# StanfordASL/pmpc

Hardware: AMD Instinct MI355X
Metric: SCP iterations/sec (M particles x N horizon) (higher is better)
Workload: dtype f64; 1 GPU; quadrotor x12 u4 M=4096 N=50 Nc=1 box-u, full SCP iteration (on-device linearise + c_lqp_solve-equivalent + residual), BASELINE config D; timed window = SCP iterations 6..2477 from the cold start X_prev = x0, U_prev = U_ref (the active-set round count falls as the SCP loop converges, so the rate depends on the window); particles_per_gpu=4096, parallelism=particle-shard x1, scp_loop=library (pmpc_scp_loop_device), ipm_warm_start=True

## Files before the change

include/pmpc_abi.h:

```cpp
#ifndef PMPC_ABI_H
#define PMPC_ABI_H

#include <stddef.h>

#ifdef __cplusplus
extern "C" {
#endif


void c_lqp_solve(double *X_out, double *U_out, size_t xdim, size_t udim, size_t N, size_t M, long long Nc,
                 double *x0, double *f, double *fx, double *fu, double *X_prev, double *U_prev, double *Q,
                 double *R, double *X_ref, double *U_ref, double *lx, double *ux, double *lu, double *uu,
                 double reg_x, double reg_u, double *slew_reg, double *slew_reg0, double *slew_um1,
                 long long verbose);

void c_lcone_solve(double *X_out, double *U_out, size_t xdim, size_t udim, size_t N, size_t M, long long Nc,
                   double *x0, double *f, double *fx, double *fu, double *X_prev, double *U_prev, double *Q,
                   double *R, double *X_ref, double *U_ref, double *lx, double *ux, double *lu, double *uu,
                   double reg_x, double reg_u, double *slew_reg, double *slew_reg0, double *slew_um1,
                   long long verbose, double smooth_alpha, char *solver);

void pmpc_lqp_solve_host(double *X_out, double *U_out, size_t xdim, size_t udim, size_t N, size_t M, long long Nc,
                         double *x0, double *f, double *fx, double *fu, double *X_prev, double *U_prev, double *Q,
                         double *R, double *X_ref, double *U_ref, double *lx, double *ux, double *lu, double *uu,
// ... 24 lines not shown
#define PMPC_CONE_OBJECTIVE 1024u
#define PMPC_F32_MATRICES 512u

typedef struct pmpc_problem {
  size_t xdim, udim, N, M;
  long long Nc;
  unsigned flags;
  double reg_x, reg_u;
  const double *x0, *f, *fx, *fu, *X_prev, *U_prev, *Q, *R, *X_ref, *U_ref;
  const double *lx, *ux, *lu, *uu;
  const double *slew_reg, *slew_reg0, *slew_um1;
  double *X_out, *U_out;
  const double *weights;
  double barrier_mu;
  size_t soc_q;
  const double *soc_W, *soc_w0, *soc_v;
  double soc_v0;
  const double *soc_u_interior;
  size_t cone_count;
  const int *cone_sizes;
  const double *cone_A, *cone_c;
  int cone_per_stage;
  long long cone_k;
  int smooth_cstr;
  double smooth_beta;
} pmpc_problem;

typedef struct pmpc_info {
  int status;
  int ipm_iters;
  int structured_solves;
  int fast_path;
  double mu;
  double slack_res;
  double max_violation;
  int outer_solves;
  int active_set_rounds;
} pmpc_info;

typedef struct pmpc_ctx pmpc_ctx;

int pmpc_create(pmpc_ctx **ctx, int device);
void pmpc_destroy(pmpc_ctx *ctx);
int pmpc_set_option(pmpc_ctx *ctx, const char *key, double value);
int pmpc_get_option(pmpc_ctx *ctx, const char *key, double *value);
void *pmpc_stream(pmpc_ctx *ctx);
void pmpc_sync(pmpc_ctx *ctx);

int pmpc_lqp_solve_device(pmpc_ctx *ctx, const pmpc_problem *prob, pmpc_info *info, int verbose);

int pmpc_lcone_solve_device(pmpc_ctx *ctx, const pmpc_problem *prob, double smooth_alpha, pmpc_info *info, int verbose);

int pmpc_lsoc_solve_device(pmpc_ctx *ctx, const pmpc_problem *prob, pmpc_info *info, int verbose);

int pmpc_particle_costs_device(pmpc_ctx *ctx, const pmpc_problem *prob, const double *X, const double *U, double *J_out);

int pmpc_comm_unique_id(void *unique_id_128);
int pmpc_comm_init(pmpc_ctx *ctx, int rank, int world, const void *unique_id_128);
int pmpc_comm_init_mock(pmpc_ctx *ctx, int rank, int world, int group);
int pmpc_comm_rank(pmpc_ctx *ctx);
int pmpc_comm_world(pmpc_ctx *ctx);

int pmpc_linearize_device(pmpc_ctx *ctx, int model, size_t N, size_t M, const double *x0, const double *X_prev,
                          const double *U_prev, const double *params, double *f, double *fx, double *fu);

int pmpc_linearize_device_f32(pmpc_ctx *ctx, int model, size_t N, size_t M, const double *x0, const double *X_prev,
                              const double *U_prev, const double *params, double *f, float *fx, float *fu);

int pmpc_rollout_device(pmpc_ctx *ctx, int model, size_t N, size_t M, const double *x0, const double *U, const double *params, double *X);

int pmpc_shift_plan_device(pmpc_ctx *ctx, int model, size_t N, size_t M, size_t s, const double *X, const double *U,
                           const double *params, const double *U_tail, double *X_new, double *U_new, double *um1_new);

int pmpc_linearize_compact_device(pmpc_ctx *ctx, int model, size_t N, size_t M, const double *x0, const double *X_prev,
                                  const double *U_prev, const double *params, double *f, double *jc);
int pmpc_expand_jac_device(pmpc_ctx *ctx, int model, size_t N, size_t M, const double *jc, double *fx, double *fu, int orient);
long long pmpc_jac_compact_doubles(int model, size_t N, size_t M);
int pmpc_jac_live_mask(int model, unsigned char *fx_mask, unsigned char *fu_mask);

int pmpc_as_sweep_variant(int sweep, int xdim, int udim, int M, int Nc, unsigned flags, const int *knobs, int *out);

int pmpc_as_sweep_launches(int sweep, unsigned long long *out, int n, int reset);
void pmpc_as_sweep_knobs(int *out);

int pmpc_scp_residual_device(pmpc_ctx *ctx, size_t xdim, size_t udim, size_t N, size_t M, const double *X, const double *X_prev,
                             const double *U, const double *U_prev, double *out);

int pmpc_scp_loop_device(pmpc_ctx *ctx, int model, const double *params, const pmpc_problem *p, double *f2, double *fx2, double *fu2,
                         int steps, int first_cold, double *res, pmpc_info *infos, int *last_in_out);

int pmpc_ref_shift_device(pmpc_ctx *ctx, size_t dim, size_t rows, const double *A, const double *c, const double *ref, double *out);
long long pmpc_ref_shift_bad_pivots(pmpc_ctx *ctx, int reset);

typedef struct pmpc_scp_cost {
  int kind;
  int K, pos_dim;
  int pos_idx[3];
  int per_stage;
  const double *centres, *sigma, *w;
} pmpc_scp_cost;
size_t pmpc_abi_scp_cost_size(void);

int pmpc_obstacle_cost_grad_device(pmpc_ctx *ctx, const pmpc_scp_cost *cost, size_t xdim, size_t N, size_t M, const double *X_prev,
                                   double *cx);
int pmpc_obstacle_ref_shift_device(pmpc_ctx *ctx, const pmpc_scp_cost *cost, size_t xdim, size_t N, size_t M, const double *X_prev,
                                   const double *Q, const double *X_ref, double *out);

int pmpc_scp_loop_device_cost(pmpc_ctx *ctx, int model, const double *params, const pmpc_problem *p, double *f2, double *fx2,
                              double *fu2, int steps, int first_cold, double *res, pmpc_info *infos, int *last_in_out,
                              const pmpc_scp_cost *cost);

typedef struct pmpc_scp_cstr {
  int kind;
  int K, pos_dim;
  int pos_idx[3];
  long long centre_stride_particle, centre_stride_stage;
  const double *centres, *radius;
} pmpc_scp_cstr;
size_t pmpc_abi_scp_cstr_size(void);

int pmpc_keepout_augment_device(pmpc_ctx *ctx, const pmpc_scp_cstr *cstr, size_t xdim, size_t udim, size_t N, size_t M,
                                const double *X_prev, const double *f, const double *fx, const double *fu, const double *X_ref,
                                double *f_aug, double *fx_aug, double *fu_aug, double *X_prev_aug, double *X_ref_aug, double *xu_aug);

void pmpc_profile_enable(pmpc_ctx *ctx, int level);
void pmpc_profile_read(pmpc_ctx *ctx, double *ms4, long long *n4);
void pmpc_profile_read_partial(pmpc_ctx *ctx, double *ms, long long *n);
void pmpc_profile_read_all(pmpc_ctx *ctx, double *ms, long long *launches, int count);

void pmpc_restart_stats(pmpc_ctx *ctx, unsigned long long *out4, int reset);

const char *pmpc_version(void);
void pmpc_abi_struct_sizes(size_t *problem, size_t *info);

#ifdef __cplusplus
}
#endif
#endif
```

pmpc_amd/_lib.py:

```python
from __future__ import annotations

import ctypes
import os
from pathlib import Path

import numpy as np

_HERE = Path(__file__).resolve().parent
LIB_PATH = Path(os.environ["PMPC_HIP_LIB"]) if os.environ.get("PMPC_HIP_LIB") else _HERE / "libpmpc_hip.so"
_lib = None

c_dp = ctypes.POINTER(ctypes.c_double)

HAS_XBOUNDS, HAS_UBOUNDS, HAS_SLEW, HAS_SLEW0, FORCE_GENERIC, SYMMETRIC_COST, COLD_START, STATIC_CONS_BOUNDS, PREV_IS_LAST_SOLUTION, F32_MATRICES, CONE_OBJECTIVE = 1, 2, 4, 8, 16, 32, 64, 128, 256, 512, 1024

ABI_SYMBOLS = [
    "c_lqp_solve", "c_lcone_solve", "pmpc_lqp_solve_host", "pmpc_lcone_solve_host", "pmpc_create", "pmpc_destroy", "pmpc_stream", "pmpc_sync", "pmpc_lqp_solve_device",
    "pmpc_comm_unique_id", "pmpc_comm_init", "pmpc_comm_rank", "pmpc_comm_world", "pmpc_linearize_device",
    "pmpc_profile_enable", "pmpc_profile_read", "pmpc_version", "pmpc_lcone_solve_device", "pmpc_particle_costs_device", "pmpc_lsoc_solve_device", "pmpc_comm_init_mock",
    "pmpc_scp_residual_device", "pmpc_profile_read_partial", "pmpc_profile_read_all", "pmpc_scp_loop_device", "pmpc_linearize_device_f32",
    "pmpc_set_option", "pmpc_get_option", "pmpc_abi_struct_sizes", "pmpc_lcone_solve_host_ex", "pmpc_restart_stats",
    "pmpc_linearize_compact_device", "pmpc_expand_jac_device", "pmpc_jac_compact_doubles", "pmpc_jac_live_mask",
    "pmpc_as_sweep_variant", "pmpc_as_sweep_launches", "pmpc_as_sweep_knobs",
    "pmpc_ref_shift_device", "pmpc_ref_shift_bad_pivots", "pmpc_obstacle_cost_grad_device", "pmpc_obstacle_ref_shift_device",
    "pmpc_scp_loop_device_cost", "pmpc_abi_scp_cost_size",
    "pmpc_rollout_device", "pmpc_shift_plan_device",
    "pmpc_keepout_augment_device", "pmpc_abi_scp_cstr_size",
]


class PmpcProblem(ctypes.Structure):
    _fields_ = (
        [(k, ctypes.c_size_t) for k in ("xdim", "udim", "N", "M")]
        + [("Nc", ctypes.c_longlong), ("flags", ctypes.c_uint), ("reg_x", ctypes.c_double), ("reg_u", ctypes.c_double)]
        + [(k, ctypes.c_void_p) for k in ("x0", "f", "fx", "fu", "X_prev", "U_prev", "Q", "R", "X_ref", "U_ref",
                                          "lx", "ux", "lu", "uu", "slew_reg", "slew_reg0", "slew_um1", "X_out", "U_out", "weights")]
        + [("barrier_mu", ctypes.c_double), ("soc_q", ctypes.c_size_t), ("soc_W", ctypes.c_void_p), ("soc_w0", ctypes.c_void_p),
           ("soc_v", ctypes.c_void_p), ("soc_v0", ctypes.c_double), ("soc_u_interior", ctypes.c_void_p),
           ("cone_count", ctypes.c_size_t), ("cone_sizes", ctypes.POINTER(ctypes.c_int)), ("cone_A", ctypes.c_void_p), ("cone_c", ctypes.c_void_p),
           ("cone_per_stage", ctypes.c_int), ("cone_k", ctypes.c_longlong), ("smooth_cstr", ctypes.c_int), ("smooth_beta", ctypes.c_double)]
    )


class PmpcInfo(ctypes.Structure):
    _fields_ = [("status", ctypes.c_int), ("ipm_iters", ctypes.c_int), ("structured_solves", ctypes.c_int),
                ("fast_path", ctypes.c_int), ("mu", ctypes.c_double), ("slack_res", ctypes.c_double),
                ("max_violation", ctypes.c_double), ("outer_solves", ctypes.c_int), ("active_set_rounds", ctypes.c_int)]


class PmpcScpCost(ctypes.Structure):
    _fields_ = [("kind", ctypes.c_int), ("K", ctypes.c_int), ("pos_dim", ctypes.c_int), ("pos_idx", ctypes.c_int * 3), ("per_stage", ctypes.c_int),
                ("centres", ctypes.c_void_p), ("sigma", ctypes.c_void_p), ("w", ctypes.c_void_p)]


class PmpcScpCstr(ctypes.Structure):
    _fields_ = [("kind", ctypes.c_int), ("K", ctypes.c_int), ("pos_dim", ctypes.c_int), ("pos_idx", ctypes.c_int * 3),
                ("centre_stride_particle", ctypes.c_longlong), ("centre_stride_stage", ctypes.c_longlong),
                ("centres", ctypes.c_void_p), ("radius", ctypes.c_void_p)]


def load():
    global _lib
    if _lib is not None:
        return _lib
    if not LIB_PATH.exists():
        raise ImportError(
            f"{LIB_PATH} is missing: build the HIP extension first (python -c 'import __graft_entry__ as g; g.build()' "
            "or make -C pmpc_amd/csrc). pmpc_amd has no CPU fallback.")
    lib = ctypes.CDLL(str(LIB_PATH), mode=ctypes.RTLD_GLOBAL)
    sz, ll, dbl, vp = ctypes.c_size_t, ctypes.c_longlong, ctypes.c_double, ctypes.c_void_p
    common = [c_dp, c_dp, sz, sz, sz, sz, ll] + [c_dp] * 14 + [dbl, dbl] + [c_dp] * 3 + [ll]
    lib.c_lqp_solve.argtypes = common
    lib.c_lqp_solve.restype = None
    lib.c_lcone_solve.argtypes = common + [dbl, ctypes.c_char_p]
    lib.c_lcone_solve.restype = None
    lib.pmpc_lqp_solve_host.argtypes = common + [ctypes.c_uint]
    lib.pmpc_lqp_solve_host.restype = None
    lib.pmpc_lcone_solve_host.argtypes = common + [dbl, ctypes.c_uint, ll]
    lib.pmpc_lcone_solve_host.restype = None
    lib.pmpc_lcone_solve_host_ex.argtypes = common + [dbl, ctypes.c_uint, ll, ctypes.c_int, dbl]
    lib.pmpc_lcone_solve_host_ex.restype = None
    lib.pmpc_create.argtypes = [ctypes.POINTER(vp), ctypes.c_int]
    lib.pmpc_create.restype = ctypes.c_int
    lib.pmpc_destroy.argtypes = [vp]
    lib.pmpc_destroy.restype = None
    lib.pmpc_set_option.argtypes = [vp, ctypes.c_char_p, ctypes.c_double]
    lib.pmpc_set_option.restype = ctypes.c_int
    lib.pmpc_get_option.argtypes = [vp, ctypes.c_char_p, c_dp]
    lib.pmpc_get_option.restype = ctypes.c_int
    lib.pmpc_stream.argtypes = [vp]
    lib.pmpc_stream.restype = vp
    lib.pmpc_sync.argtypes = [vp]
    lib.pmpc_sync.restype = None
    lib.pmpc_lqp_solve_device.argtypes = [vp, ctypes.POINTER(PmpcProblem), ctypes.POINTER(PmpcInfo), ctypes.c_int]
    lib.pmpc_lqp_solve_device.restype = ctypes.c_int
    lib.pmpc_lcone_solve_device.argtypes = [vp, ctypes.POINTER(PmpcProblem), dbl, ctypes.POINTER(PmpcInfo), ctypes.c_int]
    lib.pmpc_lcone_solve_device.restype = ctypes.c_int
    lib.pmpc_lsoc_solve_device.argtypes = [vp, ctypes.POINTER(PmpcProblem), ctypes.POINTER(PmpcInfo), ctypes.c_int]
    lib.pmpc_lsoc_solve_device.restype = ctypes.c_int
    lib.pmpc_particle_costs_device.argtypes = [vp, ctypes.POINTER(PmpcProblem), vp, vp, vp]
    lib.pmpc_particle_costs_device.restype = ctypes.c_int
    lib.pmpc_comm_unique_id.argtypes = [vp]
    lib.pmpc_comm_unique_id.restype = ctypes.c_int
    lib.pmpc_comm_init.argtypes = [vp, ctypes.c_int, ctypes.c_int, vp]
    lib.pmpc_comm_init.restype = ctypes.c_int
    lib.pmpc_comm_init_mock.argtypes = [vp, ctypes.c_int, ctypes.c_int, ctypes.c_int]
    lib.pmpc_comm_init_mock.restype = ctypes.c_int
    lib.pmpc_comm_rank.argtypes = [vp]
    lib.pmpc_comm_rank.restype = ctypes.c_int
    lib.pmpc_comm_world.argtypes = [vp]
    lib.pmpc_comm_world.restype = ctypes.c_int
    lib.pmpc_linearize_device.argtypes = [vp, ctypes.c_int, sz, sz] + [vp] * 7
    lib.pmpc_linearize_device.restype = ctypes.c_int
    lib.pmpc_linearize_device_f32.argtypes = [vp, ctypes.c_int, sz, sz] + [vp] * 7
    lib.pmpc_linearize_device_f32.restype = ctypes.c_int
    if hasattr(lib, "pmpc_jac_live_mask"):
        lib.pmpc_linearize_compact_device.argtypes = [vp, ctypes.c_int, sz, sz] + [vp] * 6
        lib.pmpc_linearize_compact_device.restype = ctypes.c_int
        lib.pmpc_expand_jac_device.argtypes = [vp, ctypes.c_int, sz, sz, vp, vp, vp, ctypes.c_int]
        lib.pmpc_expand_jac_device.restype = ctypes.c_int
        lib.pmpc_jac_compact_doubles.argtypes = [ctypes.c_int, sz, sz]
        lib.pmpc_jac_compact_doubles.restype = ctypes.c_longlong
        lib.pmpc_jac_live_mask.argtypes = [ctypes.c_int, vp, vp]
        lib.pmpc_jac_live_mask.restype = ctypes.c_int
    if hasattr(lib, "pmpc_as_sweep_variant"):
        lib.pmpc_as_sweep_variant.argtypes = [ctypes.c_int] * 5 + [ctypes.c_uint, ctypes.POINTER(ctypes.c_int), ctypes.POINTER(ctypes.c_int)]
        lib.pmpc_as_sweep_variant.restype = ctypes.c_int
    if hasattr(lib, "pmpc_as_sweep_launches"):
        lib.pmpc_as_sweep_launches.argtypes = [ctypes.c_int, ctypes.POINTER(ctypes.c_ulonglong), ctypes.c_int, ctypes.c_int]
        lib.pmpc_as_sweep_launches.restype = ctypes.c_int
        lib.pmpc_as_sweep_knobs.argtypes = [ctypes.POINTER(ctypes.c_int)]
        lib.pmpc_as_sweep_knobs.restype = None
    lib.pmpc_scp_residual_device.argtypes = [vp, sz, sz, sz, sz] + [vp] * 5
    lib.pmpc_scp_residual_device.restype = ctypes.c_int
    lib.pmpc_profile_enable.argtypes = [vp, ctypes.c_int]
    lib.pmpc_profile_enable.restype = None
    lib.pmpc_profile_read.argtypes = [vp, c_dp, ctypes.POINTER(ctypes.c_longlong)]
    lib.pmpc_profile_read.restype = None
    lib.pmpc_profile_read_partial.argtypes = [vp, ctypes.POINTER(ctypes.c_double), ctypes.POINTER(ctypes.c_longlong)]
    lib.pmpc_profile_read_partial.restype = None
    lib.pmpc_restart_stats.argtypes = [vp, ctypes.POINTER(ctypes.c_ulonglong), ctypes.c_int]
    lib.pmpc_restart_stats.restype = None
    lib.pmpc_profile_read_all.argtypes = [vp, c_dp, ctypes.POINTER(ctypes.c_longlong), ctypes.c_int]
    lib.pmpc_profile_read_all.restype = None
    lib.pmpc_scp_loop_device.argtypes = [vp, ctypes.c_int, vp, ctypes.POINTER(PmpcProblem), vp, vp, vp, ctypes.c_int, ctypes.c_int, vp,
                                         ctypes.POINTER(PmpcInfo), ctypes.POINTER(ctypes.c_int)]
    lib.pmpc_scp_loop_device.restype = ctypes.c_int
    if hasattr(lib, "pmpc_scp_loop_device_cost"):
        lib.pmpc_ref_shift_device.argtypes = [vp, sz, sz, vp, vp, vp, vp]
        lib.pmpc_ref_shift_device.restype = ctypes.c_int
        lib.pmpc_ref_shift_bad_pivots.argtypes = [vp, ctypes.c_int]
        lib.pmpc_ref_shift_bad_pivots.restype = ctypes.c_longlong
        lib.pmpc_obstacle_cost_grad_device.argtypes = [vp, ctypes.POINTER(PmpcScpCost), sz, sz, sz, vp, vp]
        lib.pmpc_obstacle_cost_grad_device.restype = ctypes.c_int
        lib.pmpc_obstacle_ref_shift_device.argtypes = [vp, ctypes.POINTER(PmpcScpCost), sz, sz, sz, vp, vp, vp, vp]
        lib.pmpc_obstacle_ref_shift_device.restype = ctypes.c_int
        lib.pmpc_scp_loop_device_cost.argtypes = lib.pmpc_scp_loop_device.argtypes + [ctypes.POINTER(PmpcScpCost)]
        lib.pmpc_scp_loop_device_cost.restype = ctypes.c_int
        lib.pmpc_abi_scp_cost_size.argtypes = []
        lib.pmpc_abi_scp_cost_size.restype = sz
        if lib.pmpc_abi_scp_cost_size() != ctypes.sizeof(PmpcScpCost):
            raise ImportError(f"{LIB_PATH} and pmpc_amd/_lib.py disagree on pmpc_scp_cost: library {lib.pmpc_abi_scp_cost_size()} bytes, "
                              f"binding {ctypes.sizeof(PmpcScpCost)}: rebuild the library")
    if hasattr(lib, "pmpc_shift_plan_device"):
        lib.pmpc_rollout_device.argtypes = [vp, ctypes.c_int, sz, sz, vp, vp, vp, vp]
        lib.pmpc_rollout_device.restype = ctypes.c_int
        lib.pmpc_shift_plan_device.argtypes = [vp, ctypes.c_int, sz, sz, sz] + [vp] * 7
        lib.pmpc_shift_plan_device.restype = ctypes.c_int
    if hasattr(lib, "pmpc_keepout_augment_device"):
        lib.pmpc_keepout_augment_device.argtypes = [vp, ctypes.POINTER(PmpcScpCstr), sz, sz, sz, sz] + [vp] * 11
        lib.pmpc_keepout_augment_device.restype = ctypes.c_int
        lib.pmpc_abi_scp_cstr_size.argtypes = []
        lib.pmpc_abi_scp_cstr_size.restype = sz
        if lib.pmpc_abi_scp_cstr_size() != ctypes.sizeof(PmpcScpCstr):
            raise ImportError(f"{LIB_PATH} and pmpc_amd/_lib.py disagree on pmpc_scp_cstr: library {lib.pmpc_abi_scp_cstr_size()} bytes, "
                              f"binding {ctypes.sizeof(PmpcScpCstr)}: rebuild the library")
    lib.pmpc_version.argtypes = []
    lib.pmpc_version.restype = ctypes.c_char_p
    if not hasattr(lib, "pmpc_abi_struct_sizes"):
        raise ImportError(f"{LIB_PATH} predates this binding (no pmpc_abi_struct_sizes): rebuild it (make -C pmpc_amd/csrc)")
    lib.pmpc_abi_struct_sizes.argtypes = [ctypes.POINTER(sz), ctypes.POINTER(sz)]
    lib.pmpc_abi_struct_sizes.restype = None
    sp, si = sz(0), sz(0)
    lib.pmpc_abi_struct_sizes(ctypes.byref(sp), ctypes.byref(si))
    if (sp.value, si.value) != (ctypes.sizeof(PmpcProblem), ctypes.sizeof(PmpcInfo)):
        raise ImportError(f"{LIB_PATH} ({lib.pmpc_version().decode()}) and pmpc_amd/_lib.py disagree on the ABI structs: library "
                          f"{sp.value}/{si.value} bytes, binding {ctypes.sizeof(PmpcProblem)}/{ctypes.sizeof(PmpcInfo)}: rebuild the library")
    _lib = lib
    return lib


def jac_live_mask(model: int, x: int, u: int):
    lib = load()
    mx, mu = np.zeros(x * x, dtype=np.uint8), np.zeros(x * u, dtype=np.uint8)
    got = lib.pmpc_jac_live_mask(int(model), mx.ctypes.data, mu.ctypes.data)
    if got < 0:
        raise ValueError(f"model {model} is not a built-in model")
    if got != 100 * x + u:
        raise ValueError(f"model {model}: compact records are for dims {got // 100} x {got % 100}, not {x} x {u}")
    return mx.reshape(x, x).T.astype(bool), mu.reshape(u, x).T.astype(bool)


AS_SWEEP_FLAGS = ("defect", "as_settled_in", "mat32", "cone_H", "xb_D", "as_uraw", "as_T")


def as_sweep_variant(sweep: str, x: int, u: int, M: int, Nc: int, flags: int, knobs=None):
    lib = load()
    out = (ctypes.c_int * 8)()
    kn = (ctypes.c_int * 3)(*knobs) if knobs is not None else None
    got = lib.pmpc_as_sweep_variant({"bwd": 0, "fwd": 1}[sweep], x, u, M, Nc, flags, kn, out)
    if got < 0:
        raise ValueError(f"({x}, {u}) is not a compiled pair of the active-set sweeps")
    return tuple(out[:5]), bool(got), tuple(bool(v) for v in out[5:8])


def as_sweep_code(sweep: str, variant) -> int:
    a, b, c, d, e = (int(v) for v in variant)
    if sweep == "bwd":
        return a + 3 * (b + 2 * (c + 2 * (d + 3 * e)))
    return a + 2 * b + 4 * c + 8 * d + 16 * e


def as_sweep_launches(sweep: str, reset: bool = False):
    lib = load()
    sw = {"bwd": 0, "fwd": 1}[sweep]
    n = lib.pmpc_as_sweep_launches(sw, None, 0, 0)
    out = (ctypes.c_ulonglong * n)()
    lib.pmpc_as_sweep_launches(sw, out, n, int(reset))
    return [int(v) for v in out]


def as_sweep_knobs():
    out = (ctypes.c_int * 3)()
    load().pmpc_as_sweep_knobs(out)
    return tuple(out)


def dptr(a: np.ndarray):
    assert a.dtype == np.float64 and a.flags["C_CONTIGUOUS"]
    return a.ctypes.data_as(c_dp)
```

pmpc_amd/csrc/as_ctl_dev.h:

```cpp
#pragma once
#include "pmpc_dev.h"

namespace {

__device__ inline void as_ctl_block(AsCtl *ctl, const int *cnt_part, int M, const int *fail, int reduce, int decide, int last_of_batch,
                                                 AsCtl *mirror, unsigned long long *mirror_seq, unsigned long long seq, double *tail, const double *viol,
                                                 const int *open_part = nullptr) {
  __shared__ int sh[4][1024];
  __shared__ double shv[1024];
  if (ctl->done) {
    if (threadIdx.x == 0 && decide && last_of_batch && mirror) {
      *mirror = *ctl;
      __threadfence_system();
      *(volatile unsigned long long *)mirror_seq = seq;
    }
    return;
  }
  if (reduce) {
    int r = 0, d = 0, b = 0, op = 0;
    double vw = 0.0;
    for (int i = threadIdx.x; i < M; i += 1024) {
      r += cnt_part[3 * i]; d += cnt_part[3 * i + 1]; b |= cnt_part[3 * i + 2];
      if (viol) vw = fmax(vw, viol[i]);
      if (open_part) op += open_part[i];
    }
    sh[0][threadIdx.x] = r; sh[1][threadIdx.x] = d; sh[2][threadIdx.x] = b; sh[3][threadIdx.x] = op; shv[threadIdx.x] = vw;
    __syncthreads();
    for (int o = 512; o > 0; o >>= 1) {
      if (threadIdx.x < o) {
        sh[0][threadIdx.x] += sh[0][threadIdx.x + o];
        sh[1][threadIdx.x] += sh[1][threadIdx.x + o];
        sh[2][threadIdx.x] |= sh[2][threadIdx.x + o];
        sh[3][threadIdx.x] += sh[3][threadIdx.x + o];
        shv[threadIdx.x] = fmax(shv[threadIdx.x], shv[threadIdx.x + o]);
      }
      __syncthreads();
    }
    if (threadIdx.x == 0 && viol && ctl->round < 16) ctl->worst[ctl->round] = shv[0];
    if (threadIdx.x == 0) {
      if (tail) { tail[0] = sh[0][0]; tail[1] = sh[1][0]; tail[2] = sh[2][0]; tail[3] = *fail; tail[4] = sh[3][0]; }
      else { ctl->cnt[0] = sh[0][0]; ctl->cnt[1] = sh[1][0]; ctl->cnt[2] = sh[2][0]; ctl->cnt[3] = *fail; ctl->open = sh[3][0]; }
    }
  }
  if (threadIdx.x == 0 && decide) {
    if (tail) {
      for (int k = 0; k < 4; k++) ctl->cnt[k] = (int)(tail[k] < 2e9 ? tail[k] : 2e9);
      ctl->open = (int)(tail[4] < 2e9 ? tail[4] : 2e9);
    }
    const int rel = ctl->cnt[0], add = ctl->cnt[1], bad = ctl->cnt[2], fl = ctl->cnt[3];
    const int round = ctl->round;
    if (round < 16) { ctl->hist[round][0] = rel; ctl->hist[round][1] = add; }
    const int changes = rel + add;
    int done = 0, status = 1;
    if (bad || fl) { done = 1; status = 2; }
    else if (changes == 0 && ctl->open == 0) { done = 1; status = 0; }
    else if (changes == 0) {
      if (round + 1 >= ctl->max_rounds) done = 1;
    } else {
      if (changes * 2 > ctl->last_changes && ++ctl->stalls >= ctl->stall_limit) done = 1;
      ctl->last_changes = changes;
      if (round + 1 >= ctl->max_rounds) done = 1;
    }
    ctl->round = round + 1;
    ctl->status = status;
    const int e = ctl->round - 3 > 0 ? ctl->round - 3 : 0;
    double tl = 1e-11;
    for (int k = 0; k < e && tl < 1e-8; k++) tl *= 10.0;
    ctl->tol_l = ctl->dual_scale * (tl < 1e-8 ? tl : 1e-8);
    __threadfence();
    ctl->done = done;
    if ((done || last_of_batch) && mirror) {
      *mirror = *ctl;
      __threadfence_system();
      *(volatile unsigned long long *)mirror_seq = seq;
    }
  }
}

__device__ inline void as_perm_block(const int *settled, int M, int *perm) {
  __shared__ int cnt[1024];
  const int t = threadIdx.x, per = (M + 1023) / 1024, lo = t * per, hi = min(M, lo + per);
  int n = 0;
  for (int i = lo; i < hi; i++) n += settled[i] ? 0 : 1;
  cnt[t] = n;
  __syncthreads();
  for (int o = 1; o < 1024; o <<= 1) {
    const int v = t >= o ? cnt[t - o] : 0;
    __syncthreads();
    cnt[t] += v;
    __syncthreads();
  }
  const int total = cnt[1023];
  int pu = cnt[t] - n, ps = total + lo - pu;
  for (int i = lo; i < hi; i++) {
    if (settled[i]) perm[ps++] = i;
    else perm[pu++] = i;
  }
}

}
```

pmpc_amd/csrc/dynamics.hip:

```cpp
#include "pmpc_dev.h"
#include "jac_compact.h"
#include <cstring>
#include <cstdlib>

namespace {

struct Unicycle {
  static constexpr int X = 4, U = 2, P = 3, UNITS = 64;
  typedef jacc::UnicycleSpec Spec;
  static __device__ __forceinline__ void step(const double *xs, const double *us, const double *p, double *fo);
  static __device__ __forceinline__ void eval(long long idx, int N, const double *x0, const double *X_prev, const double *U_prev,
                                              const double *params, double *fo, double *A, double *B);
};
struct Quadrotor {
  static constexpr int X = 12, U = 4, P = 4, UNITS = 32;
  typedef jacc::QuadrotorSpec Spec;
  static __device__ __forceinline__ void step(const double *xs, const double *us, const double *p, double *fo);
  static __device__ __forceinline__ void eval(long long idx, int N, const double *x0, const double *X_prev, const double *U_prev,
                                              const double *params, double *fo, double *A, double *B);
};

struct Bicycle {
  static constexpr int X = 4, U = 2, P = 2, UNITS = 64;
  typedef jacc::BicycleSpec Spec;
  static __device__ __forceinline__ void step(const double *xs, const double *us, const double *p, double *fo);
  static __device__ __forceinline__ void eval(long long idx, int N, const double *x0, const double *X_prev, const double *U_prev,
                                              const double *params, double *fo, double *A, double *B);
};

template <class F>
void with_model(int model, F &&fn) {
  if (model == 0) fn(Unicycle{});
  else if (model == 1) fn(Quadrotor{});
  else if (model == 2) fn(Bicycle{});
  else throw PmpcHipError{(int)hipErrorInvalidValue, "unknown built-in model", __FILE__, __LINE__};
}

__device__ __forceinline__ void Unicycle::step(const double *xs, const double *us, const double *p, double *fo) {
  const double vs = p[0], ws = p[1], T = p[2], eps = 1e-6;
  double u1 = vs * us[0], u2 = -ws * us[1];
  u1 += (u1 >= 0.0 ? eps : -eps);
  u2 += (u2 >= 0.0 ? eps : -eps);
  const double px = xs[0], py = xs[1], v0 = xs[2], th0 = xs[3];
  const double a = T * u2 + th0;
  double sa, ca, s0, c0;
  sincos(a, &sa, &ca);
  sincos(th0, &s0, &c0);
  const double iu2 = 1.0 / u2, iu22 = iu2 * iu2;
  const double n1 = u2 * sa * v0 + T * u1 * u2 * sa + u1 * ca - s0 * u2 * v0 - c0 * u1;
  const double n2 = -(u2 * ca * v0 - u1 * sa + T * u1 * u2 * ca) + c0 * u2 * v0 - s0 * u1;
  fo[0] = px + n1 * iu22; fo[1] = py + n2 * iu22; fo[2] = v0 + T * u1; fo[3] = a;
}
__device__ __forceinline__ void Unicycle::eval(long long idx, int N, const double *x0, const double *X_prev, const double *U_prev,
                                               const double *params, double *fo, double *A, double *B) {
  const int i = (int)(idx / N), j = (int)(idx % N);
  const double *xs = j == 0 ? x0 + 4 * (size_t)i : X_prev + (idx - 1) * 4;
  const double *us = U_prev + idx * 2, *p = params + 3 * (size_t)i;
  const double vs = p[0], ws = p[1], T = p[2], eps = 1e-6;
  double u1 = vs * us[0], u2 = -ws * us[1];
  u1 += (u1 >= 0.0 ? eps : -eps);
  u2 += (u2 >= 0.0 ? eps : -eps);
  const double px = xs[0], py = xs[1], v0 = xs[2], th0 = xs[3];
  const double a = T * u2 + th0;
  double sa, ca, s0, c0;
  sincos(a, &sa, &ca);
  sincos(th0, &s0, &c0);
  const double iu2 = 1.0 / u2, iu22 = iu2 * iu2;
  const double n1 = u2 * sa * v0 + T * u1 * u2 * sa + u1 * ca - s0 * u2 * v0 - c0 * u1;
  const double n2 = -(u2 * ca * v0 - u1 * sa + T * u1 * u2 * ca) + c0 * u2 * v0 - s0 * u1;
  fo[0] = px + n1 * iu22; fo[1] = py + n2 * iu22; fo[2] = v0 + T * u1; fo[3] = a;
  A[0 + 4 * 0] = 1.0; A[1 + 4 * 1] = 1.0; A[2 + 4 * 2] = 1.0; A[3 + 4 * 3] = 1.0;
  A[0 + 4 * 2] = (u2 * sa - s0 * u2) * iu22;
  A[0 + 4 * 3] = (u2 * ca * v0 + T * u1 * u2 * ca - u1 * sa - c0 * u2 * v0 + s0 * u1) * iu22;
  A[1 + 4 * 2] = (-u2 * ca + c0 * u2) * iu22;
  A[1 + 4 * 3] = (-(-u2 * sa * v0 - u1 * ca - T * u1 * u2 * sa) - s0 * u2 * v0 - c0 * u1) * iu22;
  const double dn1_du1 = T * u2 * sa + ca - c0, dn2_du1 = sa - T * u2 * ca - s0;
  const double dn1_du2 = sa * v0 + u2 * ca * T * v0 + T * u1 * sa + T * u1 * u2 * ca * T - u1 * sa * T - s0 * v0;
  const double dn2_du2 = -(ca * v0 - u2 * sa * T * v0 - u1 * ca * T + T * u1 * ca - T * T * u1 * u2 * sa) + c0 * v0;
  B[0 + 4 * 0] = dn1_du1 * iu22 * vs;
  B[1 + 4 * 0] = dn2_du1 * iu22 * vs;
  B[2 + 4 * 0] = T * vs;
  B[0 + 4 * 1] = (dn1_du2 * iu22 - 2.0 * n1 * iu22 * iu2) * (-ws);
  B[1 + 4 * 1] = (dn2_du2 * iu22 - 2.0 * n2 * iu22 * iu2) * (-ws);
  B[3 + 4 * 1] = T * (-ws);
// ... 46 lines not shown
  fo[8] = ps + dt * (sph * icth * wy + cph * icth * wz);
  fo[9] = wx + dt * (tx - (Jz - Jy) * wy * wz) / Jx;
  fo[10] = wy + dt * (ty - (Jx - Jz) * wz * wx) / Jy;
  fo[11] = wz + dt * (tz - (Jy - Jx) * wx * wy) / Jz;
}
__device__ __forceinline__ void Quadrotor::eval(long long idx, int N, const double *x0, const double *X_prev, const double *U_prev,
                                                const double *params, double *fo, double *A, double *B) {
  const int i = (int)(idx / N), j = (int)(idx % N);
  const double *xs = j == 0 ? x0 + 12 * (size_t)i : X_prev + (idx - 1) * 12;
  const double *us = U_prev + idx * 4, *p = params + 4 * (size_t)i;
  const double m = p[0], Jx = p[1], Jy = p[2], Jz = p[3], dt = 0.05, g = 9.81;
  const double ph = xs[6], th = xs[7], ps = xs[8], wx = xs[9], wy = xs[10], wz = xs[11];
  const double T = us[0], tx = us[1], ty = us[2], tz = us[3];
  double sph, cph, sth, cth, sps, cps;
  sincos(ph, &sph, &cph);
  sincos(th, &sth, &cth);
  sincos(ps, &sps, &cps);
  const double icth = 1.0 / cth, tth = sth * icth, sec2 = icth * icth;
  const double bx = cps * sth * cph + sps * sph, by = sps * sth * cph - cps * sph, bz = cth * cph;
  const double a = T / m;
  fo[0] = xs[0] + dt * xs[3]; fo[1] = xs[1] + dt * xs[4]; fo[2] = xs[2] + dt * xs[5];
  fo[3] = xs[3] + dt * a * bx; fo[4] = xs[4] + dt * a * by; fo[5] = xs[5] + dt * (a * bz - g);
  fo[6] = ph + dt * (wx + sph * tth * wy + cph * tth * wz);
  fo[7] = th + dt * (cph * wy - sph * wz);
  fo[8] = ps + dt * (sph * icth * wy + cph * icth * wz);
  fo[9] = wx + dt * (tx - (Jz - Jy) * wy * wz) / Jx;
  fo[10] = wy + dt * (ty - (Jx - Jz) * wz * wx) / Jy;
  fo[11] = wz + dt * (tz - (Jy - Jx) * wx * wy) / Jz;
#define AE(r, t) A[(r) + 12 * (t)]
#define BE(r, t) B[(r) + 12 * (t)]
  for (int k = 0; k < 12; k++) AE(k, k) = 1.0;
  for (int k = 0; k < 3; k++) AE(k, 3 + k) = dt;
  AE(3, 6) = dt * a * (-cps * sth * sph + sps * cph); AE(3, 7) = dt * a * (cps * cth * cph); AE(3, 8) = dt * a * (-sps * sth * cph + cps * sph);
  AE(4, 6) = dt * a * (-sps * sth * sph - cps * cph); AE(4, 7) = dt * a * (sps * cth * cph); AE(4, 8) = dt * a * (cps * sth * cph + sps * sph);
  AE(5, 6) = dt * a * (-cth * sph); AE(5, 7) = dt * a * (-sth * cph);
  AE(6, 6) += dt * (cph * tth * wy - sph * tth * wz);
  AE(6, 7) = dt * (sph * sec2 * wy + cph * sec2 * wz);
  AE(6, 9) = dt; AE(6, 10) = dt * sph * tth; AE(6, 11) = dt * cph * tth;
  AE(7, 6) = dt * (-sph * wy - cph * wz);
  AE(7, 10) = dt * cph; AE(7, 11) = -dt * sph;
  AE(8, 6) = dt * (cph * icth * wy - sph * icth * wz);
  AE(8, 7) = dt * (sph * wy + cph * wz) * sth * sec2;
  AE(8, 10) = dt * sph * icth; AE(8, 11) = dt * cph * icth;
  AE(9, 10) = -dt * (Jz - Jy) * wz / Jx; AE(9, 11) = -dt * (Jz - Jy) * wy / Jx;
  AE(10, 9) = -dt * (Jx - Jz) * wz / Jy; AE(10, 11) = -dt * (Jx - Jz) * wx / Jy;
  AE(11, 9) = -dt * (Jy - Jx) * wy / Jz; AE(11, 10) = -dt * (Jy - Jx) * wx / Jz;
  BE(3, 0) = dt * bx / m; BE(4, 0) = dt * by / m; BE(5, 0) = dt * bz / m;
  BE(9, 1) = dt / Jx; BE(10, 2) = dt / Jy; BE(11, 3) = dt / Jz;
#undef AE
#undef BE
}

__device__ __forceinline__ void residual_block(int bid, int nblk, const double *X, const double *Xp, long long rows_x, int x, const double *U,
                                               const double *Up, long long rows_u, int u, unsigned long long *out_bits) {
  __shared__ double sh[256];
  const int sub = threadIdx.x & 3;
  const long long grp = (bid * 256LL + threadIdx.x) >> 2, ngrp = ((long long)nblk * 256) >> 2;
  const int qx = (x + 3) / 4, qu = (u + 3) / 4;
  double m = 0.0;
  for (long long r = grp; r < rows_x + rows_u; r += ngrp) {
    const bool isx = r < rows_x;
    const long long rr = isx ? r : r - rows_x;
    const int d = isx ? x : u, q = isx ? qx : qu;
    const double *a = (isx ? X : U) + rr * d, *b = (isx ? Xp : Up) + rr * d;
    const int k1 = min(d, (sub + 1) * q);
    double acc = 0.0;
    for (int k = sub * q; k < k1; k++) { const double t = a[k] - b[k]; acc = fma(t, t, acc); }
    acc += __shfl_xor(acc, 1, 64);
    acc += __shfl_xor(acc, 2, 64);
    m = (acc == acc) ? fmax(m, acc) : INFINITY;
  }
  sh[threadIdx.x] = sqrt(m);
  __syncthreads();
  for (int o = 128; o > 0; o >>= 1) {
    if (threadIdx.x < o) sh[threadIdx.x] = fmax(sh[threadIdx.x], sh[threadIdx.x + o]);
    __syncthreads();
  }
  if (threadIdx.x == 0) atomicMax(out_bits, (unsigned long long)__double_as_longlong(sh[0]));
}
struct ResArgs {
  const double *X, *Xp, *U, *Up;
  long long rows;
  int x, u, nblk;
  unsigned long long *out_bits;
};
#ifndef PMPC_LIN_THREADS
#define PMPC_LIN_THREADS 256
#endif
template <class Model, class JT>
__global__ void __launch_bounds__(PMPC_LIN_THREADS) k_linearize(int N, long long tot, const double *x0, const double *X_prev, const double *U_prev,
                                                  const double *params, double *f, JT *fx, JT *fu, ResArgs res) {
  constexpr int X = Model::X, U = Model::U, UNITS = Model::UNITS;
  {
    const int glin = (int)gridDim.x - res.nblk;
    if ((int)blockIdx.x >= glin) {
      residual_block((int)blockIdx.x - glin, res.nblk, res.X, res.Xp, res.rows, res.x, res.U, res.Up, res.rows, res.u, res.out_bits);
      return;
    }
  }
  constexpr int REC = X + X * X + X * U, LD = REC | 1;
  extern __shared__ double rec[];
  const int t = threadIdx.x;
  const long long first = (long long)blockIdx.x * UNITS;
  for (int e = t; e < UNITS * LD; e += PMPC_LIN_THREADS) rec[e] = 0.0;
  __syncthreads();
  if (t < UNITS && first + t < tot) {
    double *mine = rec + t * LD;
    Model::eval(first + t, N, x0, X_prev, U_prev, params, mine, mine + X, mine + X + X * X);
  }
  __syncthreads();
  const int n = (int)((tot - first) < UNITS ? (tot - first) : UNITS);
  for (int e = t; e < n * X; e += PMPC_LIN_THREADS) f[first * X + e] = rec[(e / X) * LD + e % X];
  for (int e = t; e < n * X * X; e += PMPC_LIN_THREADS) fx[first * (X * X) + e] = (JT)rec[(e / (X * X)) * LD + X + e % (X * X)];
  for (int e = t; e < n * X * U; e += PMPC_LIN_THREADS) fu[first * (X * U) + e] = (JT)rec[(e / (X * U)) * LD + X + X * X + e % (X * U)];
}

template <class Model>
void launch_model(int N, int M, const double *x0, const double *X_prev, const double *U_prev, const double *params, double *f,
                  double *fx, double *fu, const ResArgs &res, hipStream_t s, int jac32) {
  const long long tot = (long long)M * N;
  constexpr int REC = Model::X + Model::X * Model::X + Model::X * Model::U, LD = REC | 1;
  const unsigned grid = (unsigned)((tot + Model::UNITS - 1) / Model::UNITS);
  if (jac32)
    hipLaunchKernelGGL((k_linearize<Model, float>), dim3(grid + (unsigned)res.nblk), dim3(PMPC_LIN_THREADS), Model::UNITS * LD * sizeof(double), s, N, tot, x0,
                       X_prev, U_prev, params, f, (float *)fx, (float *)fu, res);
  else
    hipLaunchKernelGGL((k_linearize<Model, double>), dim3(grid + (unsigned)res.nblk), dim3(PMPC_LIN_THREADS), Model::UNITS * LD * sizeof(double), s, N, tot, x0,
                       X_prev, U_prev, params, f, fx, fu, res);
}
constexpr int LIN_CUNITS = 64;
template <class Model>
__global__ void __launch_bounds__(PMPC_LIN_THREADS) k_linearize_compact(int N, long long tot, const double *x0, const double *X_prev, const double *U_prev,
                                                                         const double *params, double *f, double *jc, ResArgs res) {
  typedef jacc::Compact<typename Model::Spec> C;
  constexpr int X = Model::X, U = Model::U, UNITS = LIN_CUNITS, REC = C::REC, POOL = C::POOL;
  {
    const int glin = (int)gridDim.x - res.nblk;
    if ((int)blockIdx.x >= glin) {
      residual_block((int)blockIdx.x - glin, res.nblk, res.X, res.Xp, res.rows, res.x, res.U, res.Up, res.rows, res.u, res.out_bits);
      return;
    }
  }
  constexpr int LD = (X + REC) | 1;
  extern __shared__ double rec[];
  const int t = threadIdx.x;
  const long long first = (long long)blockIdx.x * UNITS;
  if (t < UNITS && first + t < tot) {
    double J[X * X + X * U] = {};
    double *mine = rec + t * LD;
    Model::eval(first + t, N, x0, X_prev, U_prev, params, mine, J, J + X * X);
#pragma unroll
    for (int k = 0; k < REC; k++) mine[X + k] = J[C::tab.rec_src[k]];
    if ((first + t) % N == 0) {
      double *pool = jc + tot * REC + ((first + t) / N) * POOL;
#pragma unroll
      for (int k = 0; k < POOL; k++) pool[k] = C::tab.pool_src[k] < 0 ? 0.0 : J[C::tab.pool_src[k] < 0 ? 0 : C::tab.pool_src[k]];
    }
  }
  __syncthreads();
  const int n = (int)((tot - first) < UNITS ? (tot - first) : UNITS);
  for (int e = t; e < n * X; e += PMPC_LIN_THREADS) f[first * X + e] = rec[(e / X) * LD + e % X];
  for (int e = t; e < n * REC; e += PMPC_LIN_THREADS) jc[first * REC + e] = rec[(e / REC) * LD + X + e % REC];
}

template <class Model>
__global__ void __launch_bounds__(256) k_expand_jac(int N, long long tot, const double *jc, double *fx, double *fu, int orient) {
  typedef jacc::Compact<typename Model::Spec> C;
  constexpr int X = Model::X, U = Model::U, XX = X * X, XU = X * U, D = XX + XU;
  const long long n = tot * D;
  for (long long k = (long long)blockIdx.x * 256 + threadIdx.x; k < n; k += (long long)gridDim.x * 256) {
    const long long unit = k / D;
    const int e = (int)(k % D);
    const int m = C::tab.expand[orient ? 1 : 0][e];
    const double v = m >= 0 ? jc[unit * C::REC + m] : jc[tot * C::REC + (unit / N) * C::POOL + (-1 - m)];
    if (e < XX) fx[unit * XX + e] = v;
    else fu[unit * XU + (e - XX)] = v;
  }
}

template <class Model>
void launch_model_compact(int N, int M, const double *x0, const double *X_prev, const double *U_prev, const double *params, double *f,
                          double *jc, const ResArgs &res, hipStream_t s) {
  typedef jacc::Compact<typename Model::Spec> C;
  const long long tot = (long long)M * N;
  constexpr int LD = (Model::X + C::REC) | 1;
  const unsigned grid = (unsigned)((tot + LIN_CUNITS - 1) / LIN_CUNITS);
  hipLaunchKernelGGL((k_linearize_compact<Model>), dim3(grid + (unsigned)res.nblk), dim3(PMPC_LIN_THREADS), LIN_CUNITS * LD * sizeof(double), s, N, tot,
                     x0, X_prev, U_prev, params, f, jc, res);
}
__global__ void __launch_bounds__(256) k_widen_f32(const float *src, double *dst, long long n) {
  for (long long k = (long long)blockIdx.x * 256 + threadIdx.x; k < n; k += (long long)gridDim.x * 256) dst[k] = (double)src[k];
}


constexpr int ROLL_LANES = 64;
template <class Model>
__global__ void __launch_bounds__(ROLL_LANES) k_rollout(int N, int M, const double *x0, const double *U, const double *params, double *X) {
  constexpr int XD = Model::X, UD = Model::U, PD = Model::P;
  const int i = (int)blockIdx.x * ROLL_LANES + (int)threadIdx.x;
  if (i >= M) return;
  double x[XD], xn[XD], u[UD], p[PD];
#pragma unroll
  for (int k = 0; k < PD; k++) p[k] = params[(size_t)i * PD + k];
#pragma unroll
  for (int k = 0; k < XD; k++) x[k] = x0[(size_t)i * XD + k];
  const double *Ui = U + (size_t)i * N * UD;
  double *Xi = X + (size_t)i * N * XD;
  for (int j = 0; j < N; j++) {
#pragma unroll
    for (int k = 0; k < UD; k++) u[k] = Ui[(size_t)j * UD + k];
    Model::step(x, u, p, xn);
#pragma unroll
    for (int k = 0; k < XD; k++) Xi[(size_t)j * XD + k] = x[k] = xn[k];
  }
}

template <class Model>
__global__ void __launch_bounds__(ROLL_LANES) k_shift_plan(int N, int M, int s, int tail_blocks, const double *X, const double *U, const double *params,
                                                           const double *U_tail, double *Xn, double *Un, double *um1n) {
  constexpr int XD = Model::X, UD = Model::U, PD = Model::P;
  const int keep = N - s;
  if ((int)blockIdx.x < tail_blocks) {
    const int i = (int)blockIdx.x * ROLL_LANES + (int)threadIdx.x;
    if (i >= M) return;
    double x[XD], xn[XD], u[UD], p[PD];
#pragma unroll
    for (int k = 0; k < PD; k++) p[k] = params[(size_t)i * PD + k];
#pragma unroll
    for (int k = 0; k < XD; k++) x[k] = X[((size_t)i * N + (N - 1)) * XD + k];
    for (int t = 0; t < s; t++) {
      const double *us = U_tail ? U_tail + ((size_t)i * s + t) * UD : U + ((size_t)i * N + (N - 1)) * UD;
#pragma unroll
      for (int k = 0; k < UD; k++) u[k] = us[k];
      Model::step(x, u, p, xn);
#pragma unroll
      for (int k = 0; k < XD; k++) x[k] = xn[k];
      const size_t row = (size_t)i * N + keep + t;
#pragma unroll
      for (int k = 0; k < UD; k++) Un[row * UD + k] = u[k];
#pragma unroll
      for (int k = 0; k < XD; k++) Xn[row * XD + k] = x[k];
    }
    return;
  }
  const long long nx = (long long)M * keep * XD, nu = (long long)M * keep * UD, nm = um1n ? (long long)M * UD : 0;
  const long long stride = (long long)((int)gridDim.x - tail_blocks) * ROLL_LANES;
  for (long long e = (long long)((int)blockIdx.x - tail_blocks) * ROLL_LANES + threadIdx.x; e < nx + nu + nm; e += stride) {
    if (e < nx) {
      const long long i = e / (keep * XD), r = e % (keep * XD);
      Xn[i * N * XD + r] = X[i * N * XD + (long long)s * XD + r];
    } else if (e < nx + nu) {
      const long long q = e - nx, i = q / (keep * UD), r = q % (keep * UD);
      Un[i * N * UD + r] = U[i * N * UD + (long long)s * UD + r];
    } else {
      const long long q = e - nx - nu, i = q / UD, k = q % UD;
      um1n[q] = U[(i * N + (s - 1)) * UD + k];
    }
  }
}

}

static long long residual_blocks(long long rows) {
  long long nb = (2 * rows * 4 + 255) / 256;
  const long long cap = rows >= 200000 ? 1024 : 256;
  return nb > cap ? cap : nb;
}

void launch_linearize(int model, int N, int M, const double *x0, const double *X_prev, const double *U_prev,
                      const double *params, double *f, double *fx, double *fu, hipStream_t s, int jac32) {
  ResArgs none;
  memset(&none, 0, sizeof(none));
  with_model(model, [&](auto m) { launch_model<decltype(m)>(N, M, x0, X_prev, U_prev, params, f, fx, fu, none, s, jac32); });
}
void launch_linearize_compact(int model, int N, int M, const double *x0, const double *X_prev, const double *U_prev, const double *params,
                              double *f, double *jc, const double *Xr, const double *Xrp, const double *Ur, const double *Urp, int x, int u,
                              double *res_out, hipStream_t s) {
  ResArgs r;
  memset(&r, 0, sizeof(r));
  if (res_out) {
    r.X = Xr; r.Xp = Xrp; r.U = Ur; r.Up = Urp; r.rows = (long long)M * N; r.x = x; r.u = u;
    r.nblk = (int)residual_blocks(r.rows);
    r.out_bits = (unsigned long long *)res_out;
  }
  with_model(model, [&](auto m) { launch_model_compact<decltype(m)>(N, M, x0, X_prev, U_prev, params, f, jc, r, s); });
}
void launch_rollout(int model, int N, int M, const double *x0, const double *U, const double *params, double *X, hipStream_t s) {
  const unsigned grid = (unsigned)((M + ROLL_LANES - 1) / ROLL_LANES);
  with_model(model, [&](auto m) { hipLaunchKernelGGL((k_rollout<decltype(m)>), dim3(grid), dim3(ROLL_LANES), 0, s, N, M, x0, U, params, X); });
}
void launch_shift_plan(int model, int N, int M, int sh, const double *X, const double *U, const double *params, const double *U_tail, double *Xn,
                       double *Un, double *um1n, hipStream_t s) {
  const int tail_blocks = (M + ROLL_LANES - 1) / ROLL_LANES;
  with_model(model, [&](auto m) {
    typedef decltype(m) Model;
    const long long n = (long long)M * (N - sh) * (Model::X + Model::U) + (long long)M * Model::U;
    long long cb = (n + 4 * ROLL_LANES - 1) / (4 * ROLL_LANES);
    if (cb > 8192) cb = 8192;
    hipLaunchKernelGGL((k_shift_plan<Model>), dim3((unsigned)(tail_blocks + cb)), dim3(ROLL_LANES), 0, s, N, M, sh, tail_blocks, X, U, params, U_tail,
                       Xn, Un, um1n);
  });
}
bool model_known(int model) { return model >= 0 && model <= 2; }
bool jac_compact_dims(int model, int x, int u) {
  bool ok = false;
  if (model_known(model)) with_model(model, [&](auto m) { ok = x == decltype(m)::X && u == decltype(m)::U; });
  return ok;
}
long long jac_compact_doubles(int model, int N, int M) {
  const long long tot = (long long)M * N;
  long long n = -1;
  if (model_known(model))
    with_model(model, [&](auto m) {
      typedef jacc::Compact<typename decltype(m)::Spec> C;
      n = tot * C::REC + (long long)M * C::POOL;
    });
  return n;
}
void launch_expand_jac(int model, int N, int M, const double *jc, double *fx, double *fu, int orient, hipStream_t s) {
  const long long tot = (long long)M * N;
  with_model(model, [&](auto m) {
    typedef decltype(m) Model;
    long long b = (tot * (Model::X * Model::X + Model::X * Model::U) + 255) / 256;
    if (b > 8192) b = 8192;
    hipLaunchKernelGGL((k_expand_jac<Model>), dim3((unsigned)b), dim3(256), 0, s, N, tot, jc, fx, fu, orient);
  });
}
int jac_live_mask(int model, unsigned char *fx_mask, unsigned char *fu_mask) {
  auto fill = [&](auto spec) {
    typedef jacc::Compact<decltype(spec)> C;
    for (int c = 0; c < C::X + C::U; c++)
      for (int r = 0; r < C::X; r++) (c < C::X ? fx_mask[r + C::X * c] : fu_mask[r + C::X * (c - C::X)]) = C::cls(r, c) == -1;
    return C::X * 100 + C::U;
  };
  int dims = -1;
  if (model_known(model)) with_model(model, [&](auto m) { dims = fill(typename decltype(m)::Spec{}); });
  return dims;
}
void launch_widen_f32(const float *src, double *dst, long long n, hipStream_t s) {
  long long b = (n + 255) / 256;
  if (b > 4096) b = 4096;
  hipLaunchKernelGGL(k_widen_f32, dim3((unsigned)b), dim3(256), 0, s, src, dst, n);
}

void launch_linearize_with_residual(int model, int N, int M, const double *x0, const double *X_prev, const double *U_prev,
                                    const double *params, double *f, double *fx, double *fu, const double *Xr, const double *Xrp,
                                    const double *Ur, const double *Urp, int x, int u, double *res_out, hipStream_t s, int jac32) {
  ResArgs r;
  r.X = Xr; r.Xp = Xrp; r.U = Ur; r.Up = Urp; r.rows = (long long)M * N; r.x = x; r.u = u;
  r.nblk = (int)residual_blocks(r.rows);
  r.out_bits = (unsigned long long *)res_out;
  with_model(model, [&](auto m) { launch_model<decltype(m)>(N, M, x0, X_prev, U_prev, params, f, fx, fu, r, s, jac32); });
}

namespace {
__global__ void __launch_bounds__(256) k_scp_residual(const double *X, const double *Xp, long long rows_x, int x, const double *U,
                                                      const double *Up, long long rows_u, int u, unsigned long long *out_bits) {
  residual_block((int)blockIdx.x, (int)gridDim.x, X, Xp, rows_x, x, U, Up, rows_u, u, out_bits);
}
}

void launch_scp_residual(const double *X, const double *Xp, const double *U, const double *Up, long long rows, int x, int u,
                         double *out, hipStream_t s, bool zero_out) {
  if (zero_out) HIP_CHECK(hipMemsetAsync(out, 0, sizeof(double), s));
  const long long nb = residual_blocks(rows);
  hipLaunchKernelGGL(k_scp_residual, dim3((unsigned)nb), dim3(256), 0, s, X, Xp, rows, x, U, Up, rows, u, (unsigned long long *)out);
}
```

pmpc_amd/csrc/kernels_as.hip:

```cpp
#include <atomic>
#include <type_traits>

#include "fast_common.h"
#include "as_ctl_dev.h"
#include "as_variant.h"
#include "../../include/pmpc_abi.h"
#include "jac_compact.h"

#ifdef PMPC_STAGE_TIMELINE
#define PMPC_TL_STAMPS 10
__device__ unsigned long long pmpc_tl[3][128][PMPC_TL_STAMPS];
#define TL_DECL(kind) unsigned long long tl_[PMPC_TL_STAMPS] = {}; const int tl_kind = (kind); const bool tl_on = blockIdx.x == gridDim.x / 2
#define TL(k) do { __builtin_amdgcn_sched_barrier(0); tl_[k] = __builtin_amdgcn_s_memtime(); __builtin_amdgcn_sched_barrier(0); } while (0)
#define TL_FLUSH(j) do { if (tl_on && threadIdx.x == 0 && (j) < 128) { for (int k_ = 0; k_ < PMPC_TL_STAMPS; k_++) pmpc_tl[tl_kind][j][k_] = tl_[k_]; } } while (0)
#else
#define TL_DECL(kind)
#define TL(k)
#define TL_FLUSH(j)
#endif

#ifndef PMPC_AS_LEAN_WAVES
#define PMPC_AS_LEAN_WAVES 4
#endif
#ifndef PMPC_AS_DEEP_WAVES
#define PMPC_AS_DEEP_WAVES 3
#endif
#ifndef PMPC_AS_DEEP2_MAXM
#define PMPC_AS_DEEP2_MAXM 1024
#endif

namespace {

template <int XD, int UD, int MODE, bool SKIP, bool DEFECT, int EX = 0, class MT = double>
__global__ void __launch_bounds__(64, MODE == 2 ? 2 : (MODE == 1 ? PMPC_AS_DEEP_WAVES : PMPC_AS_LEAN_WAVES)) k_bwd_as(LQArgs a) {
  constexpr bool CONE = EX == 1, XBOX = EX == 2;
  typedef Lane<XD, UD> LT;
  constexpr int KS = LT::KS, XP = LT::XP;
  constexpr bool PADX = (XD != XP);
  constexpr long long D8 = sizeof(double);
  constexpr bool DEEP = MODE != 0, SCHOL = !DEEP;
  constexpr long long MB = sizeof(MT);
  if (a.done && *a.done) return;
  const int lane = threadIdx.x;
  const int N = a.N, Nc = a.Nc, i = a.as_perm ? __builtin_amdgcn_readfirstlane(a.as_perm[blockIdx.x]) : (int)blockIdx.x;
  if (SKIP && a.as_settled_in[i]) {
    const int nc = Nc * UD;
    if (lane < nc) {
      const double *H = a.Hc_part + (size_t)i * nc * nc;
      double acc = 0.0;
      for (int cc = 0; cc < nc; cc++) acc = fma(H[(lane < cc ? lane : cc) + nc * (lane < cc ? cc : lane)], a.as_delta[cc], acc);
      a.gc_part[(size_t)i * nc + lane] += acc;
    }
    return;
  }
  const LT L(lane);
  const int g = L.g, c = L.c;
  const size_t pbase = (size_t)i * N;
  const bool own0 = (i == 0 && a.owner);
  const bool gu = g < UD;
  const double *Z = a.zeros;
  const double pwt = a.pw ? a.pw[i] : 1.0;
  const double regx = pwt * a.reg_x, regu = pwt * a.reg_u;
  const double *Xb = DEFECT ? a.X_prev : a.Xb, *Ub = DEFECT ? a.U_prev : a.Ub;
  constexpr int CKS = 64 * KS + 32;
  int jtop = N - 1, ck_k = 0;
  if (SKIP && a.as_ck) {
    const int jh = a.as_jhi[i];
    const int lo = jh > Nc ? jh : (Nc > 1 ? Nc : 1);
    const int k = lo <= PMPC_AS_CK_FIRST ? 0 : 32 - __builtin_clz((unsigned)(lo - 1) >> PMPC_AS_CK_LOG);
    if (k < a.ck_slots) { ck_k = __builtin_amdgcn_readfirstlane(k + 1); jtop = PMPC_AS_CK_FIRST << (ck_k - 1); }
    if (lane == 0 && a.ck_stat) {
      atomicAdd(a.ck_stat + (ck_k ? 0 : 2), 1ull);
      atomicAdd(a.ck_stat + (ck_k ? 1 : 3), (unsigned long long)(jtop + 1));
    }
  }
  const double *ck_ = a.as_ck ? ubase(a.as_ck, (long long)i * a.ck_slots * (long long)(CKS * sizeof(double))) : nullptr;

  const bool fF = L.cxv || L.cu;
  const MT *pF = L.cxv ? (const MT *)a.fx + (pbase + jtop) * (XD * XD) + XD * L.oc + L.row0
                       : (L.cu ? (const MT *)a.fu + (pbase + jtop) * (XD * UD) + XD * L.cb + L.row0 : (const MT *)Z);
  int sF = fF ? -(int)MB * (L.cxv ? XD * XD : XD * UD) : 0;
  typedef typename jacc::SpecFor<XD, UD>::list JSpecs;
  if constexpr (JSpecs::COUNT > 0 && std::is_same<MT, double>::value) {
    if (a.jac_compact) {
      const jacc::LaneSel js = jacc::select(JSpecs{}, a.jac_compact, lane);
      const int m = js.bwd;
      if (m != jacc::NONE) {
        pF = m >= 0 ? (const MT *)a.fx + (pbase + jtop) * js.rec + m : (const MT *)a.fx + (size_t)a.M * N * js.rec + (size_t)i * js.pool + (-1 - m);
        sF = m >= 0 ? -(int)MB * js.rec : 0;
      }
    }
  }
  const unsigned lQ = (unsigned)((L.cxv ? XD * L.oc + L.row0 : 0) * MB);
  const double pwt_x = L.cxv ? pwt : 0.0;
  const bool fR = L.cu && gu;
  const unsigned lR = (unsigned)((fR ? g + UD * L.cb : 0) * MB), lRd = (unsigned)((fR ? g + UD * L.cb : 0) * D8);
  const unsigned lxr = (unsigned)(L.row0 * D8), lxc = (unsigned)((L.cxv ? L.oc : 0) * D8);
  const unsigned lug = (unsigned)((gu ? g : 0) * D8);
  const double regx_c = L.cxv ? regx : 0.0;
  const bool umask = L.cu && g == L.cb;
  const double umask_d = umask ? 1.0 : 0.0;
  const bool diag_x = L.cxv && ((c & 3) == g);
  bool dmask[KS];
#pragma unroll
  for (int r = 0; r < KS; r++) dmask[r] = diag_x && (c >> 2) == r;
  const long long px = (long long)(pbase * XD) * D8, pu = (long long)(pbase * UD) * D8;
  const double *Xb_ = ubase(Xb, px), *Xr_ = ubase(a.X_ref, px), *Xp_ = ubase(a.X_prev, px), *f_ = ubase(a.f, px);
  const double *kff_ = ubase(a.kff, pu);
  const void *Q_ = ubase_v(a.Q, (long long)(pbase * (XD * XD)) * MB), *R_ = ubase_v(a.R, (long long)(pbase * (UD * UD)) * MB);
  const void *K_ = ubase_v(a.K, (long long)(pbase * 64) * MB);
  auto xoff = [&](int jj) { return (long long)(jj * (int)(XD * D8)); };
  auto uoff = [&](int jj) { return (long long)(jj * (int)(UD * D8)); };
  auto ld_Q = [&](int jj, double *dst) {
    const void *q = ubase_v(Q_, (long long)(jj * (int)(XD * XD * MB)));
#pragma unroll
    for (int r = 0; r < KS; r++) {
      const bool rv = !PADX || (L.row0 + r < XD);
      const double v = ldom<MT>(q, rv ? lQ + r * (unsigned)MB : 0u);
      dst[r] = rv ? v : 0.0;
    }
  };
  auto ld_xm = [&](int jj, double *dst) {
    const double *xb = ubase(Xb_, xoff(jj)), *xr = ubase(Xr_, xoff(jj));
#pragma unroll
    for (int r = 0; r < KS; r++) {
      const bool rv = !PADX || (L.row0 + r < XD);
      const unsigned o = rv ? lxr + r * 8u : 0u;
      const double v = pwt * (ldo(xb, o) - ldo(xr, o));
      dst[r] = rv ? v : 0.0;
    }
  };
  auto ld_gx = [&](int jj) -> double {
    if (DEFECT) return 0.0;
    return regx_c * (ldo(ubase(Xb_, xoff(jj)), lxc) - ldo(ubase(Xp_, xoff(jj)), lxc));
  };
  const char *pC = (const char *)Z;
  int sC = 0;
  if (gu && c == XP) { pC = (const char *)(Ub + (pbase + jtop) * UD + g); sC = -UD * (int)D8; }
  else if (gu && c == XP + 1) { pC = (const char *)(a.U_ref + (pbase + jtop) * UD + g); sC = -UD * (int)D8; }
  else if (gu && c == XP + 2) { pC = (const char *)(a.as_act + (pbase + jtop) * UD + g); sC = -UD * (int)sizeof(int); }
  else if (CONE && gu && c == XP + 3) { pC = (const char *)(a.cone_g + (pbase + jtop) * UD + g); sC = -UD * (int)D8; }
  else if (!DEFECT && g < 2 && 15 - XP - c >= 0 && 15 - XP - c < UD) {
    pC = (const char *)((g == 0 ? Ub : a.U_prev) + (pbase + jtop) * UD + (15 - XP - c));
    sC = -UD * (int)D8;
  }
  const double regu_s = (L.cu && g < 2) ? (g == 0 ? regu : -regu) : 0.0;
  auto ld_R = [&](int jj) -> double {
    const double v = ldom<MT>(ubase_v(R_, (long long)(jj * (int)(UD * UD * MB))), lR);
    return fR ? v : 0.0;
  };
  const double *CH_ = CONE ? ubase(a.cone_H, (long long)(pbase * (UD * UD)) * D8) : Z;
  auto ld_CH = [&](int jj) -> double {
    const double v = ldo(ubase(CH_, (long long)(jj * (int)(UD * UD * D8))), lRd);
    return fR ? v : 0.0;
  };
  const bool frec = (L.cxv || L.cu) && gu;
// ... 593 lines not shown
      swap32_d(vworst, p01, p23);
      const double m = fmax(p01, p23);
      swap16_d(m, q0, q1);
      if (lane == 0) a.as_viol[i] = fmax(q0, q1);
    }
    if (a.as_jhi) {
      int m = jh;
#pragma unroll
      for (int k = 1; k < 4; k++) { const int o = __builtin_amdgcn_readlane(jh, 16 * k); m = o > m ? o : m; }
      if (lane == 0) a.as_jhi[i] = m;
    }
    if (lane == 0) {
      a.as_cnt[3 * i + 0] = (int)r;
      a.as_cnt[3 * i + 1] = (int)d;
      a.as_cnt[3 * i + 2] = b > 0.0 ? 1 : 0;
      if (a.as_settled_out) a.as_settled_out[i] = (r == 0.0 && d == 0.0 && !(b > 0.0)) ? 1 : 0;
      if (CONE) a.as_open[i] = 0;
    }
  };

  const int jmin = Nc > 1 ? Nc : 1;
  auto clampN = [&](int jj) { return jj < N ? jj : N - 1; };
  int j = 0;
  if constexpr (SENS && !DEFECT) if (elem) {
    Pipe P;
    fetch(0, P);
    stage(std::false_type{}, 0, P);
    settled_update(1);
    finish();
    return;
  }
  if (PF2) {
    Pipe P0, P1, P2;
    fetch(0, P0);
    fetch(clampN(1), P1);
    for (; j < jmin && j < N; j++) {
      fetch(clampN(j + 2), P2);
      stage(std::false_type{}, j, P0);
      P0 = P1;
      P1 = P2;
    }
    for (; j + 2 < N; j += 3) {
      fetch(clampN(j + 2), P2);
      stage(std::true_type{}, j, P0);
      fetch(clampN(j + 3), P0);
      stage(std::true_type{}, j + 1, P1);
      fetch(clampN(j + 4), P1);
      stage(std::true_type{}, j + 2, P2);
    }
    if (j < N) { stage(std::true_type{}, j, P0); j++; }
    if (j < N) { stage(std::true_type{}, j, P1); j++; }
  } else {
    Pipe A, B;
    fetch(0, A);
    for (; j < jmin && j < N; j++) {
      fetch(clampN(j + 1), B);
      stage(std::false_type{}, j, A);
      A = B;
    }
    for (; j < N; j++) {
      fetch(clampN(j + 1), B);
      stage(std::true_type{}, j, A);
      A = B;
    }
  }
  finish();
}

__global__ void k_as_begin(AsCtl *ctl, int *fail, int max_rounds, double dual_scale, int stall_limit) {
  if (threadIdx.x == 0) {
    *fail = 0;
    AsCtl h = {};
    h.max_rounds = max_rounds;
    h.stall_limit = stall_limit;
    h.last_changes = 0x7fffffff;
    h.dual_scale = dual_scale;
    h.tol_l = dual_scale * 1e-11;
    *ctl = h;
  }
}

__global__ void __launch_bounds__(1024) k_as_ctl(AsCtl *ctl, const int *cnt_part, int M, const int *fail, int reduce, int decide, int last_of_batch,
                                                 AsCtl *mirror, unsigned long long *mirror_seq, unsigned long long seq, double *tail, const double *viol,
                                                 const int *open_part) {
  as_ctl_block(ctl, cnt_part, M, fail, reduce, decide, last_of_batch, mirror, mirror_seq, seq, tail, viol, open_part);
}

__global__ void __launch_bounds__(1024) k_as_perm(const int *settled, int M, int *perm, const int *done) {
  if (done && *done) return;
  as_perm_block(settled, M, perm);
}

template <class F>
void lift(bool v, F &&f) {
  if (v) f(std::true_type{}); else f(std::false_type{});
}
template <class F>
void lift3(int v, F &&f) {
  if (v == 0) f(std::integral_constant<int, 0>{}); else if (v == 1) f(std::integral_constant<int, 1>{}); else f(std::integral_constant<int, 2>{});
}
[[noreturn]] void no_such_variant(const char *sweep, int x, int u) {
  fprintf(stderr, "pmpc_hip: %s: the selected variant is not compiled for xdim %d, udim %d (as_variant.h)\n", sweep, x, u);
  throw PmpcHipError{-1, sweep, __FILE__, __LINE__};
}
const AsSweepKnobs &as_sweep_knobs() {
  static const AsSweepKnobs k = {getenv("PMPC_AS_DEEP2_MAXM") ? atoi(getenv("PMPC_AS_DEEP2_MAXM")) : PMPC_AS_DEEP2_MAXM,
                                 getenv("PMPC_AS_DEEP_MAXM") ? atoi(getenv("PMPC_AS_DEEP_MAXM")) : PMPC_AS_DEEP_WAVES * 1024,
                                 getenv("PMPC_AS_FWD_PF2_MAXM") ? atoi(getenv("PMPC_AS_FWD_PF2_MAXM")) : (1 << 30)};
  return k;
}
std::atomic<unsigned long long> as_bwd_launches[AS_BWD_CODES], as_fwd_launches[AS_FWD_CODES];

template <int XD, int UD>
void launch_bwd_as_t(const LQArgs &a, hipStream_t s) {
  const BwdAsVariant v = select_bwd_as(a.M, a.defect, a.as_settled_in, a.mat32, a.cone_H, a.xb_D, as_sweep_knobs());
  bool launched = false;
  lift3(v.mode, [&](auto MODE) { lift(v.skip, [&](auto SKIP) { lift(v.defect, [&](auto DEFECT) { lift3(v.ex, [&](auto EX) { lift(v.f32, [&](auto F32) {
    if constexpr (bwd_as_compiled(BwdAsVariant{MODE, SKIP, DEFECT, EX, F32}, XD, UD)) {
      hipLaunchKernelGGL((k_bwd_as<XD, UD, MODE, SKIP, DEFECT, EX, std::conditional_t<F32, float, double>>), dim3(a.M), dim3(64), 0, s, a);
      as_bwd_launches[bwd_as_code(v)].fetch_add(1, std::memory_order_relaxed);
      launched = true;
    }
  }); }); }); }); });
  if (!launched) no_such_variant("factor sweep of an active-set round", XD, UD);
}
template <int XD, int UD>
void launch_fwd_as_t(const LQArgs &a, hipStream_t s) {
  const FwdAsVariant v = select_fwd_as(a.M, a.Nc, a.defect, a.mat32, a.as_uraw, a.as_T, as_sweep_knobs());
  bool launched = false;
  lift(v.defect, [&](auto DEFECT) { lift(v.pf2, [&](auto PF2) { lift(v.cone, [&](auto CONE) { lift(v.f32, [&](auto F32) { lift(v.sens, [&](auto SENS) {
    if constexpr (fwd_as_compiled(FwdAsVariant{DEFECT, PF2, CONE, F32, SENS}, XD, UD)) {
      hipLaunchKernelGGL((k_fwd_as<XD, UD, DEFECT, PF2, CONE, std::conditional_t<F32, float, double>, SENS>), dim3(a.M), dim3(64), 0, s, a);
      as_fwd_launches[fwd_as_code(v)].fetch_add(1, std::memory_order_relaxed);
      launched = true;
    }
  }); }); }); }); });
  if (!launched) no_such_variant("forward sweep of an active-set round", XD, UD);
}

}

#ifdef PMPC_STAGE_TIMELINE
extern "C" int pmpc_debug_timeline_read(unsigned long long *out) {
  return (int)hipMemcpyFromSymbol(out, HIP_SYMBOL(pmpc_tl), sizeof(unsigned long long) * 3 * 128 * PMPC_TL_STAMPS);
}
#endif
static bool as_dims_compiled(int x, int u) {
#define X(xd, ud) if (x == xd && u == ud) return true;
  PMPC_FAST_DIMS(X)
#undef X
  return false;
}
bool f32_as_dims_supported(int x, int u) { return as_dims_compiled(x, u) && as_f32_dims(x, u); }
bool xbox_as_dims_supported(int x, int u) { return as_dims_compiled(x, u) && as_xbox_dims(x, u); }
bool cone_as_dims_supported(int x, int u) { return as_dims_compiled(x, u) && as_cone_dims(x, u); }
int pmpc_as_sweep_variant(int sweep, int xdim, int udim, int M, int Nc, unsigned flags, const int *knobs, int *out) {
  if ((sweep != 0 && sweep != 1) || !as_dims_compiled(xdim, udim) || !out) return -1;
  const AsSweepKnobs k = knobs ? AsSweepKnobs{knobs[0], knobs[1], knobs[2]} : AsSweepKnobs{PMPC_AS_DEEP2_MAXM, PMPC_AS_DEEP_WAVES * 1024, 1 << 30};
  const bool defect = flags & 1, settled_in = flags & 2, mat32 = flags & 4, cone_H = flags & 8, xb_D = flags & 16, as_uraw = flags & 32, as_T = flags & 64;
  out[5] = f32_as_dims_supported(xdim, udim); out[6] = cone_as_dims_supported(xdim, udim); out[7] = xbox_as_dims_supported(xdim, udim);
  if (sweep == 0) {
    const BwdAsVariant v = select_bwd_as(M, defect, settled_in, mat32, cone_H, xb_D, k);
    out[0] = v.mode; out[1] = v.skip; out[2] = v.defect; out[3] = v.ex; out[4] = v.f32;
    return bwd_as_compiled(v, xdim, udim);
  }
  const FwdAsVariant v = select_fwd_as(M, Nc, defect, mat32, as_uraw, as_T, k);
  out[0] = v.defect; out[1] = v.pf2; out[2] = v.cone; out[3] = v.f32; out[4] = v.sens;
  return fwd_as_compiled(v, xdim, udim);
}
int pmpc_as_sweep_launches(int sweep, unsigned long long *out, int n, int reset) {
  if (sweep != 0 && sweep != 1) return -1;
  std::atomic<unsigned long long> *t = sweep == 0 ? as_bwd_launches : as_fwd_launches;
  const int codes = sweep == 0 ? AS_BWD_CODES : AS_FWD_CODES;
  for (int c = 0; c < codes; c++) {
    const unsigned long long v = reset ? t[c].exchange(0, std::memory_order_relaxed) : t[c].load(std::memory_order_relaxed);
    if (out && c < n) out[c] = v;
  }
  return codes;
}
void pmpc_as_sweep_knobs(int *out) {
  const AsSweepKnobs &k = as_sweep_knobs();
  out[0] = k.deep2_maxm; out[1] = k.deep_maxm; out[2] = k.fwd_pf2_maxm;
}
void launch_bwd_as(const LQArgs &a, hipStream_t s) {
#define X(xd, ud) if (a.x == xd && a.u == ud) { launch_bwd_as_t<xd, ud>(a, s); return; }
  PMPC_FAST_DIMS(X)
#undef X
  no_such_variant("factor sweep of an active-set round", a.x, a.u);
}
void launch_fwd_as(const LQArgs &a, hipStream_t s) {
#define X(xd, ud) if (a.x == xd && a.u == ud) { launch_fwd_as_t<xd, ud>(a, s); return; }
  PMPC_FAST_DIMS(X)
#undef X
  no_such_variant("forward sweep of an active-set round", a.x, a.u);
}
void launch_as_ctl(AsCtl *ctl, const int *cnt_part, int M, const int *fail, int reduce, int decide, int last_of_batch, AsCtl *mirror,
                   unsigned long long *mirror_seq, unsigned long long seq, hipStream_t s, double *tail, const double *viol, const int *open_part) {
  hipLaunchKernelGGL(k_as_ctl, dim3(1), dim3(1024), 0, s, ctl, cnt_part, M, fail, reduce, decide, last_of_batch, mirror, mirror_seq, seq, tail, viol,
                     open_part);
}
void launch_as_perm(const int *settled, int M, int *perm, const int *done, hipStream_t s) {
  hipLaunchKernelGGL(k_as_perm, dim3(1), dim3(1024), 0, s, settled, M, perm, done);
}
void launch_as_begin(AsCtl *ctl, int *fail, int max_rounds, double dual_scale, hipStream_t s, int stall_limit) {
  hipLaunchKernelGGL(k_as_begin, dim3(1), dim3(64), 0, s, ctl, fail, max_rounds, dual_scale, stall_limit);
}
```

pmpc_amd/csrc/kernels_generic.hip:

```cpp
#include "pmpc_dev.h"
#include <cstdlib>
#include "as_ctl_dev.h"

namespace {

constexpr int WV = 64;

__device__ __forceinline__ size_t vofs(int i, int j, int N, int d) { return ((size_t)i * N + j) * (size_t)d; }
__device__ __forceinline__ size_t mofs(int i, int j, int N, int r, int c) {
  return ((size_t)i * N + j) * (size_t)r * (size_t)c;
}
__device__ __forceinline__ double slew_diag(double s0, double s, int j, int N) {
  return j == 0 ? s0 + s : (j == N - 1 ? s : 2.0 * s);
}
__device__ __forceinline__ double symu(const double *B, int d, int r, int t) {
  return r <= t ? B[r + d * t] : B[t + d * r];
}

struct LdsMap {
  double *S, *F, *G, *H, *Lc, *Kt, *Hi, *sv, *hv, *tv, *Qr, *Rr, *gxs;
};
__host__ __device__ inline size_t lds_doubles(int x, int u, int n) {
  int nt = n + u;
  return (size_t)n * n + 2 * (size_t)n * nt + (size_t)nt * nt + 2 * (size_t)u * u + (size_t)u * n + n + 2 * nt +
// ... 802 lines not shown
    for (int q = 0; q < MAXQ; q++)
      if (bJ[q] == p) {
        const int I = launder_s(bI[q]);
#pragma unroll
        for (int r = 0; r < 4; r++) Praw[(16 * I + g + 4 * r) * LD + c] = blk[q][r];
      }
    __syncthreads();
    if (tid < 64) cons_diag_block(Praw + kb * LD, Dg, Di + p * 272, bs, fail);
    __syncthreads();
#pragma unroll
    for (int q = 0; q < MAXQ; q++)
      if (bJ[q] == p) {
        const int I = launder_s(bI[q]);
        cv4d acc = {0.0, 0.0, 0.0, 0.0};
#pragma unroll
        for (int kk = 0; kk < 4; kk++)
          acc = __builtin_amdgcn_mfma_f64_16x16x4f64(Praw[(16 * I + c) * LD + 4 * kk + g], Di[p * 272 + c * 17 + 4 * kk + g], acc, 0, 0, 0);
        const int rr = nc - 16 * I;
#pragma unroll
        for (int r = 0; r < 4; r++) {
          if (I == p && g + 4 * r < bs) acc[r] = (c <= g + 4 * r) ? Dg[c * 16 + g * 4 + r] : 0.0;
          P[(16 * I + g + 4 * r) * LD + c] = acc[r];
          if (g + 4 * r == rr && c < bs) zs[kb + c] = acc[r];
        }
        blk[q] = acc;
        __builtin_amdgcn_sched_barrier(0);
      }
    __syncthreads();
#pragma unroll
    for (int q = 0; q < MAXQ; q++)
      if (bJ[q] > p) {
        const int I = launder_s(bI[q]), J = launder_s(bJ[q]);
#pragma unroll
        for (int kk = 0; kk < 4; kk++)
          blk[q] = __builtin_amdgcn_mfma_f64_16x16x4f64(-P[(16 * I + c) * LD + 4 * kk + g], P[(16 * J + c) * LD + 4 * kk + g], blk[q], 0, 0, 0);
        __builtin_amdgcn_sched_barrier(0);
      }
  }
#pragma unroll
  for (int q = 0; q < MAXQ; q++)
    if (bI[q] >= 0) {
#pragma unroll
      for (int r = 0; r < 4; r++) {
        const int R = 16 * bI[q] + g + 4 * r, C = 16 * bJ[q] + c;
        if (R < nc && C <= R) Lc[R + (size_t)nc * C] = blk[q][r];
      }
    }
  for (int e = tid; e < npan * 272; e += NTH) Lc[(size_t)nc * nc + e] = Di[e];
  for (int p = npan - 1; p >= 0; p--) {
    const int kb = 16 * p, bs = min(16, nc - kb);
    double v = 0.0;
    if (tid < bs) {
#pragma unroll
      for (int k = 0; k < 16; k++)
        if (k >= tid && k < bs) v = fma(Di[p * 272 + k * 17 + tid], zs[kb + k], v);
    }
    __syncthreads();
    if (tid < bs) zs[kb + tid] = v;
    __syncthreads();
    if (kb > 0) {
#pragma unroll
      for (int q = 0; q < MAXQ; q++)
        if (bI[q] == p && bJ[q] < p) {
          double s_ = 0.0;
#pragma unroll
          for (int r = 0; r < 4; r++) s_ = fma(blk[q][r], zs[kb + g + 4 * r], s_);
          part[g * NCP + 16 * launder_s(bJ[q]) + c] = s_;
        }
      __syncthreads();
      for (int e = tid; e < kb; e += NTH) zs[e] -= (part[e] + part[NCP + e]) + (part[2 * NCP + e] + part[3 * NCP + e]);
      __syncthreads();
    }
  }
  for (int e = tid; e < nc; e += NTH) duc[e] = zs[e];
}

__global__ void __launch_bounds__(1024) k_cons_small(const double *Hc_part, const double *gc_part, int M, int nc, int with_H,
                                                     double *outH, double *outg, int solve_now, double *Lc, double *duc,
                                                     int *fail, AsCtlCall pend) {
  __shared__ double red[32][33];
  __shared__ double y[8];
  const int nblk = pend.ctl ? (int)gridDim.x - 1 : (int)gridDim.x;
  if (pend.ctl && (int)blockIdx.x == nblk) {
    as_ctl_block(pend.ctl, pend.cnt_part, pend.M, pend.fail, 1, 1, 0, pend.mirror, pend.mirror_seq, pend.seq, nullptr, pend.viol, pend.open_part);
    if (pend.perm) {
      __syncthreads();
      as_perm_block(pend.settled, pend.M, pend.perm);
    }
    return;
  }
  const int tid = threadIdx.x, e = tid & 31, pl = tid >> 5;
  const int nH = nc * nc, E = with_H ? nH + nc : nc;
  const int per = (M + nblk - 1) / nblk, i0 = blockIdx.x * per, i1 = min(M, i0 + per);
  const bool isH = with_H && e < nH;
  double acc = 0.0;
  if (e < E) {
    const double *src = isH ? Hc_part + e : gc_part + (with_H ? e - nH : e);
    const int stride = isH ? nH : nc;
    double a0 = 0.0, a1 = 0.0, a2 = 0.0, a3 = 0.0;
    int i = i0 + pl;
    for (; i + 96 < i1; i += 128) {
      a0 += src[(size_t)i * stride];
      a1 += src[(size_t)(i + 32) * stride];
      a2 += src[(size_t)(i + 64) * stride];
      a3 += src[(size_t)(i + 96) * stride];
    }
    for (; i < i1; i += 32) a0 += src[(size_t)i * stride];
    acc = (a0 + a1) + (a2 + a3);
  }
  red[pl][e] = acc;
  __syncthreads();
  if (pl == 0 && e < E) {
    double t = 0.0;
    for (int k = 0; k < 32; k++) t += red[k][e];
    if (isH) outH[(size_t)blockIdx.x * nH + e] = t;
    else outg[(size_t)blockIdx.x * nc + (with_H ? e - nH : e)] = t;
  }
  __syncthreads();
  if (solve_now && tid == 0) {
    const double *H = outH, *g = outg;
    if (with_H) {
      for (int q = 0; q < nc; q++) {
        double d = H[q + nc * q];
        for (int k = 0; k < q; k++) d -= Lc[q + nc * k] * Lc[q + nc * k];
        if (!(d > 0.0)) { *fail = 2; d = 1.0; }
        d = sqrt(d);
        Lc[q + nc * q] = d;
        for (int p = q + 1; p < nc; p++) {
          double v = H[q + nc * p];
          for (int k = 0; k < q; k++) v -= Lc[p + nc * k] * Lc[q + nc * k];
          Lc[p + nc * q] = v / d;
        }
      }
    }
    for (int p = 0; p < nc; p++) {
      double v = -g[p];
      for (int k = 0; k < p; k++) v -= Lc[p + nc * k] * y[k];
      y[p] = v / Lc[p + nc * p];
    }
    for (int p = nc - 1; p >= 0; p--) {
      double v = y[p];
      for (int k = p + 1; k < nc; k++) v -= Lc[k + nc * p] * y[k];
      y[p] = v / Lc[p + nc * p];
    }
    for (int p = 0; p < nc; p++) duc[p] = y[p];
  }
}

}

void launch_cons_small(const double *Hc_part, const double *gc_part, int M, int nc, bool with_H, double *Hg, double *tmp,
                       bool solve_now, double *Lc, double *duc, int *fail, hipStream_t s) {
  const int nH = nc * nc;
  int G = (M + 127) / 128;
  if (G > 64) G = 64;
  if (M <= 512) G = 1;
  double *Hc = Hg, *gc = Hg + nH;
  if (G <= 1) {
    hipLaunchKernelGGL(k_cons_small, dim3(1), dim3(1024), 0, s, Hc_part, gc_part, M, nc, with_H ? 1 : 0, Hc, gc, solve_now ? 1 : 0,
                       Lc, duc, fail, AsCtlCall{});
    return;
  }
  double *tH = tmp, *tg = tmp + (size_t)64 * nH;
  hipLaunchKernelGGL(k_cons_small, dim3(G), dim3(1024), 0, s, Hc_part, gc_part, M, nc, with_H ? 1 : 0, tH, tg, 0, Lc, duc, fail, AsCtlCall{});
  hipLaunchKernelGGL(k_cons_small, dim3(1), dim3(1024), 0, s, (const double *)tH, (const double *)tg, G, nc, with_H ? 1 : 0, Hc, gc,
                     solve_now ? 1 : 0, Lc, duc, fail, AsCtlCall{});
}

int launch_cons_partials(const double *Hc_part, const double *gc_part, int M, int nc, double *tmp, const AsCtlCall &pend, hipStream_t s) {
  const int nH = nc * nc;
  static const int per = getenv("PMPC_CONS_PER_PARTIAL") ? atoi(getenv("PMPC_CONS_PER_PARTIAL")) : 256;
  int G = (M + per - 1) / per;
  if (G > 64) G = 64;
  hipLaunchKernelGGL(k_cons_small, dim3(G + (pend.ctl ? 1 : 0)), dim3(1024), 0, s, Hc_part, gc_part, M, nc, 1, tmp, tmp + (size_t)64 * nH, 0,
                     nullptr, nullptr, nullptr, pend);
  return G;
}

__global__ void __launch_bounds__(256) k_cons_scale(const double *Hc_part, const double *gc_part, const double *w, int M, int nc, int with_H,
                                                    double *outH, double *outg, const int *as_act, double as_big, const double *Du,
                                                    const double *wu, int u, int owner) {
  const int nH = nc * nc, E = with_H ? nH + nc : nc;
  const long long tot = (long long)M * E;
  for (long long k = blockIdx.x * 256ll + threadIdx.x; k < tot; k += (long long)gridDim.x * 256) {
    const int i = (int)(k / E), e = (int)(k % E);
    const bool isH = with_H && e < nH;
    const int r = isH ? e % nc : (with_H ? e - nH : e), cc = isH ? e / nc : -1;
    const double v = isH ? Hc_part[(size_t)i * nH + e] : gc_part[(size_t)i * nc + r];
    double keep = 0.0;
    if (i == 0 && owner) {
      if (isH && cc == r) keep = as_act ? (as_act[r] ? as_big : 0.0) : (Du ? Du[r] : 0.0);
      if (!isH && !as_act && wu) keep = wu[r];
    }
    const double o = fma(w[i], v - keep, keep);
    if (isH) outH[(size_t)i * nH + e] = o;
    else outg[(size_t)i * nc + r] = o;
  }
}
void launch_cons_scale(const double *Hc_part, const double *gc_part, const double *w, int M, int nc, bool with_H, double *outH, double *outg,
                       const int *as_act, double as_big, const double *Du, const double *wu, int u, int owner, hipStream_t s) {
  const long long tot = (long long)M * (with_H ? nc * nc + nc : nc);
  const long long blocks = (tot + 255) / 256;
  hipLaunchKernelGGL(k_cons_scale, dim3((unsigned)(blocks < 2048 ? (blocks > 0 ? blocks : 1) : 2048)), dim3(256), 0, s, Hc_part, gc_part, w, M, nc,
                     with_H ? 1 : 0, outH, outg, as_act, as_big, Du, wu, u, owner);
}

__global__ void __launch_bounds__(1024) k_epi_check(const double *lam, const double *J, const double *user, int M, double cap, double *out,
                                                   double *mirror, unsigned long long *mirror_seq, unsigned long long seq) {
  __shared__ double rs[1024], rmin[1024], rmax[1024];
  __shared__ int rn[1024];
  __shared__ double tsh;
  const int t = threadIdx.x;
  double s = 0.0, jmin = 1e300, jmax = -1e300;
  int n = 0;
  for (int i = t; i < M; i += 1024) {
    const double l = lam[i], j = J[i] * (user ? user[i] : 1.0);
    if (l > 1e-12 && l < cap - 1e-12) { s += j; n++; }
    else if (l >= cap - 1e-12) jmin = fmin(jmin, j);
    else jmax = fmax(jmax, j);
  }
  rs[t] = s; rn[t] = n; rmin[t] = jmin; rmax[t] = jmax;
  __syncthreads();
  for (int w = 512; w > 0; w >>= 1) {
    if (t < w) { rs[t] += rs[t + w]; rn[t] += rn[t + w]; rmin[t] = fmin(rmin[t], rmin[t + w]); rmax[t] = fmax(rmax[t], rmax[t + w]); }
    __syncthreads();
  }
  if (t == 0) {
    const double a = rmin[0], b = rmax[0];
    tsh = rn[0] ? rs[0] / (double)rn[0] : ((a < 1e300 && b > -1e300) ? 0.5 * (a + b) : (a < 1e300 ? a : b));
  }
  __syncthreads();
  const double th = tsh;
  double v = 0.0;
  bool bad = false;
  for (int i = t; i < M; i += 1024) {
    const double l = lam[i], j = J[i] * (user ? user[i] : 1.0);
    bad |= !(j == j);
    if (l > 1e-12 && l < cap - 1e-12) v = fmax(v, fabs(j - th));
    else if (l >= cap - 1e-12) v = fmax(v, th - j);
    else v = fmax(v, j - th);
  }
  const int nin = rn[0];
  __syncthreads();
  rs[t] = bad ? 1e300 : v;
  __syncthreads();
  for (int w = 512; w > 0; w >>= 1) {
    if (t < w) rs[t] = fmax(rs[t], rs[t + w]);
    __syncthreads();
  }
  if (t == 0) {
    out[0] = rs[0]; out[1] = th; out[2] = (double)nin; out[3] = 0.0;
    if (mirror) {
      mirror[0] = rs[0]; mirror[1] = th; mirror[2] = (double)nin; mirror[3] = 0.0;
      __threadfence_system();
      *(volatile unsigned long long *)mirror_seq = seq;
    }
  }
}
// ... 89 lines not shown
```

pmpc_amd/csrc/pmpc_dev.h:

```cpp
#pragma once
#include <hip/hip_runtime.h>
#include <cstdint>
#include <cstdio>
#include <cstdlib>

struct PmpcHipError {
  int code;
  const char *what, *file;
  int line;
};
#define HIP_CHECK(expr)                                                                       \
  do {                                                                                        \
    hipError_t _e = (expr);                                                                   \
    if (_e != hipSuccess) {                                                                   \
      fprintf(stderr, "pmpc_hip: HIP error %s at %s:%d (%s)\n", hipGetErrorString(_e), __FILE__, \
              __LINE__, #expr);                                                               \
      throw PmpcHipError{(int)_e, #expr, __FILE__, __LINE__};                                 \
    }                                                                                         \
  } while (0)
#define HIP_WARN(expr)                                                                        \
  do {                                                                                        \
    hipError_t _e = (expr);                                                                   \
    if (_e != hipSuccess)                                                                     \
      fprintf(stderr, "pmpc_hip: HIP error %s at %s:%d (%s)\n", hipGetErrorString(_e), __FILE__, __LINE__, #expr); \
// ... 54 lines not shown
  int *as_jhi;
  int ck_slots;
  unsigned long long *ck_stat;
  double as_big, as_tol_p, as_tol_l;
  double as_freeze_tol;
  const double *Xb, *Ub;
  double *Xo, *Uo;
  double *as_delta;
  const AsCtl *as_ctl;
  const int *done;
  int as_merge;
  const double *cons_tH, *cons_tg;
  int cons_G;
  const double *cone_H, *cone_g;
  double *as_uraw;
  int *as_open;
  double *as_T;
  const double *xb_D, *xb_g;
  int mat32;
  int jac_compact;
  int owner;
  int any_slew;
  int sym_cost;
  int *fail;
};

struct Slab {
  long long count;
  int d, N, Nc;
  int is_u;
  int owner;
  const double *lo, *hi;
  double *z, *dz;
  const double *dz2;
  double *tl, *tu, *ll, *lu, *cl, *cu, *D, *w;
};

struct SlabEx {
  Slab s;
  int bounded;
  const double *ref, *prev;
  double *gm, *gd;
  double reg;
  const double *pw;
  long long per;
};

struct IpmScal {
  double comp_sum;
  double cnt;
  double muaff_sum;
  double pad0;
  double res_max;
  double viol_max;
  unsigned long long amin_bits;
  unsigned long long pad1;
  double mu, sigma, sigmu, alpha_aff, alpha, nu;
  int iter, status;
  double mu_target;
  double dev_max;
  double *part_dev;
};

#define PMPC_RED_BLOCKS 1024

size_t lq_generic_lds_bytes(const LQArgs &a);
void launch_rollout(const LQArgs &a, const double *U, double *X, hipStream_t s);
void launch_bwd_generic(const LQArgs &a, bool factor, hipStream_t s);
void launch_fwd_generic(const LQArgs &a, hipStream_t s);
void launch_reduce_particles_hg(const double *Hc_part, const double *gc_part, double *tmp, double *Hg, int M, int nc, hipStream_t s, int MH = -1);
void launch_reduce_particles(const double *src, double *tmp, double *dst, int M, int E, hipStream_t s);
struct AsCtlCall {
  AsCtl *ctl;
  const int *cnt_part;
  int M;
  const int *fail;
  AsCtl *mirror;
  unsigned long long *mirror_seq;
  unsigned long long seq;
  const double *viol;
  const int *open_part;
  const int *settled;
  int *perm;
};
int launch_cons_partials(const double *Hc_part, const double *gc_part, int M, int nc, double *tmp, const AsCtlCall &pend,
                         hipStream_t s);
void launch_cons_small(const double *Hc_part, const double *gc_part, int M, int nc, bool with_H, double *Hg, double *tmp, bool solve_now,
                       double *Lc, double *duc, int *fail, hipStream_t s);
void launch_cons_solve(double *Hc, double *Lc, const double *gc, double *duc, int nc, bool factor, int *fail,
                       hipStream_t s);
void launch_epi_check(const double *lam, const double *J, const double *user, int M, double cap, double *out, hipStream_t s, double *mirror = nullptr,
                      unsigned long long *mirror_seq = nullptr, unsigned long long seq = 0);
void launch_cons_scale(const double *Hc_part, const double *gc_part, const double *w, int M, int nc, bool with_H, double *outH, double *outg,
                       const int *as_act, double as_big, const double *Du, const double *wu, int u, int owner, hipStream_t s);

bool lq_fast_supported(const LQArgs &a);
void launch_bwd_fast(const LQArgs &a, bool factor, hipStream_t s);
void launch_fwd_fast(const LQArgs &a, hipStream_t s);
int cond_fast_groups(int M);
void launch_cond_fast(const LQArgs &a, hipStream_t s);
void launch_rollout_fast(const LQArgs &a, const double *U, double *X, hipStream_t s);
void launch_grad_prep(const LQArgs &a, hipStream_t s);
void launch_as_publish(int *counters, const int *fail, int *mirror_cnt, unsigned long long *mirror_seq, unsigned long long seq, hipStream_t s);
void launch_particle_cost(const LQArgs &a, const double *X, const double *U, double *J, hipStream_t s);

void launch_bwd_as(const LQArgs &a, hipStream_t s);
void launch_fwd_as(const LQArgs &a, hipStream_t s);
void launch_as_perm(const int *settled, int M, int *perm, const int *done, hipStream_t s);
void launch_as_begin(AsCtl *ctl, int *fail, int max_rounds, double dual_scale, hipStream_t s, int stall_limit = 2);
void launch_as_ctl(AsCtl *ctl, const int *cnt_part, int M, const int *fail, int reduce, int decide, int last_of_batch, AsCtl *mirror,
                   unsigned long long *mirror_seq, unsigned long long seq, hipStream_t s, double *tail = nullptr, const double *viol = nullptr,
                   const int *open_part = nullptr);

struct ConeArgs {
  int M, N, u, q, Nc, owner;
  const double *U, *Uraw;
  const double *A, *c;
  int ncones, qs[4], rows, per_stage;
  const double *R;
  int r32;
  double reg_u, rho_scale;
  double *z, *rec;
  double *H, *g;
  int *cnt, *settled, *open;
  int *jhi;
  const int *done;
  const AsCtl *ctl;
  int finish;
  double tol_step, tol_phi, dual_scale;
};
#define PMPC_CONE_REC 12
bool cone_as_supported(int u, int q);
bool cone_as_dims_supported(int x, int u);
void launch_cone_step(const ConeArgs &a, hipStream_t s);
void launch_cone_drop_redundant_lo(double *lo, const double *A, const double *c, int q, long long rows, int u, hipStream_t s);

struct XboxArgs {
  int M, N, x;
  const double *X;
  const double *lo, *hi;
  const double *Q, *pw;
  double reg_x, rho_scale;
  double *qmax;
  double *z;
  int *st;
  double *D, *g;
  int *cnt, *settled, *open;
  int *jhi;
  const int *done;
  const AsCtl *ctl;
  int finish;
  double tol, dual_scale;
  double z_tol;
  int keep_on_clamp;
  double act_frac;
  int ctrl_from;
};
bool xbox_as_dims_supported(int x, int u);
void launch_xbox_step(const XboxArgs &a, hipStream_t s);
void launch_xbox_from_ipm(const struct Slab &sx, int *st, double *z, hipStream_t s);

void launch_block_transpose(const double *in, double *out, int rows, int cols, long long n, hipStream_t s);
void launch_host_checks(const double *lx, const double *ux, long long nx, const double *lu, const double *uu, long long nu,
                        const double *Q, long long nq, int x, const double *R, long long nr, int u, int *flags, hipStream_t s);
void launch_axpy(double *y, const double *xv, double alpha, long long n, hipStream_t s);
void launch_fill(double *y, double v, long long n, hipStream_t s);
void launch_cons_bounds(double *lo, double *hi, int M, int N, int u, int Nc, hipStream_t s);
void launch_init_base(double *U, const double *U_prev, int M, int N, int u, int Nc, hipStream_t s);
void launch_violation(const Slab &sl, double *part_max, hipStream_t s);
void launch_violation_sum(const Slab &sl, const double *za, const double *zb, double *part_max, hipStream_t s);
void launch_ipm_clip(const Slab &sl, hipStream_t s);
void launch_as_setup(const Slab &sl, int from_ipm, int keep_base, int *act, double *ztry, double big, hipStream_t s);
void launch_as_check(const Slab &sl, int *act, const double *ztry, double big, double tol_p, double tol_l, int *counters,
                     unsigned long long *worst_bits, hipStream_t s);
void launch_as_accept_all(const Slab &sl, const int *act, const double *ztry, double *Uout, const double *xtry, const double *dx,
                          long long nx, double *Xws, double *Xout, hipStream_t s);
void launch_ipm_init_slack(const Slab &sl, double mu0, hipStream_t s, double thr_frac = 1e-2);
void launch_ipm_prepare(const Slab &sl, int corrector, const IpmScal *sc, double *part_sum, double *part_cnt,
                        double *part_max, hipStream_t s);
void launch_ipm_step(const Slab &sl, int corrector, IpmScal *sc, double *part_s1, double *part_s2, hipStream_t s);
void launch_ipm_advance(const SlabEx &X, const SlabEx &U, int do_update, const IpmScal *sc, double *part_sum, double *part_cnt,
                        double *part_max, hipStream_t s);
void launch_ipm_exchange(int phase, bool pack, bool unpack, IpmScal *sc, const int *fail, double *xch, int rank, int world,
                         const double *part_sum, const double *part_cnt, const double *part_max, int nblocks, hipStream_t s,
                         double mu_target = 0.0, double *part_dev = nullptr,
                         IpmScal *mirror = nullptr, unsigned long long *mirror_seq = nullptr, unsigned long long seq = 0);

struct SocArgs {
  int M, N, u, Nc, q, owner;
  const double *U, *dU, *dU2;
  int corr;
  double *cl, *cu, *cc;
  const double *lo, *hi;
  const double *W, *w0, *v;
  double v0, mu, sigmu;
  double *sl, *su, *sc;
  double *zl, *zu, *zc;
  double *dsl, *dsu, *dsc, *dzl, *dzu, *dzc;
  double *Hadd, *wu;
  int *fail;
};
int launch_soc_prepare(const SocArgs &a, int mode, double *part_sum, double *part_cnt, hipStream_t s);
int launch_soc_step(const SocArgs &a, unsigned long long *amin_bits, double *part_s1, double *part_s2, hipStream_t s);
void launch_soc_update(const SocArgs &a, double alpha, double *X, const double *dX, const double *dX2, double *U, long long nx,
                       long long nu, long long ncz, hipStream_t s);
void launch_soc_fill_u(double *U, const double *u0, long long tot, int u, hipStream_t s);

void launch_bar_prep(const double *X, const double *U, const double *lx, const double *ux, const double *lu, const double *uu, double *Dx, double *wx,
                     double *Du, double *wu, double mu, long long nx, long long nu, int u, int N, int Nc, int owner, double *part_val, double *part_min,
                     double *out2, hipStream_t s, int mode = 0, double beta = 1.0);
void launch_cost_dots(const LQArgs &a, const double *X, const double *U, const double *dX1, const double *dU1, const double *dX2, const double *dU2,
                      double *out, hipStream_t s, const double *bx = nullptr, const double *bu = nullptr);
int launch_epi_newton(const double *Hc_part, const double *gb, const double *ga, const double *dots, const double *sig, int M, int nc, double k_minus_summu,
                      double *coef, double *duc, int *fail, hipStream_t s, int mode = 0, double *xch = nullptr);
void launch_axpy_particle(const double *a_, const double *b_, const double *coef, double *y, long long per, long long tot, hipStream_t s);
void launch_step_to(const double *a_, const double *b_, double alpha, double *y, long long tot, hipStream_t s);
void launch_interior(double *U, const double *lo, const double *hi, long long tot, double frac, hipStream_t s);
void launch_share_cons(double *U, int M, int N, int u, int Nc, hipStream_t s);

struct SlewAug {
  int x, u, N, M, Nc, has_xb, has_ub, has_um1;
  double dx, du;
  const double *f, *fx, *fu, *Xp, *Up, *Q, *R, *Xr, *Ur, *lx, *ux, *lu, *uu, *cons_lo, *cons_hi, *slew, *slew0, *um1;
  double *af, *afx, *afu, *aXp, *aUp, *aQ, *aR, *aXr, *aUr, *alo, *ahi;
};
void launch_slew_augment(const SlewAug &g, hipStream_t s);
void launch_slew_split(const double *Z, const double *W, double *X, double *U, long long rows, int x, int u, int N, int Nc,
                       const double *cons_lo, const double *cons_hi, hipStream_t s);
void launch_linearize(int model, int N, int M, const double *x0, const double *X_prev, const double *U_prev,
                      const double *params, double *f, double *fx, double *fu, hipStream_t s, int jac32 = 0);
void launch_linearize_compact(int model, int N, int M, const double *x0, const double *X_prev, const double *U_prev, const double *params,
                              double *f, double *jc, const double *Xr, const double *Xrp, const double *Ur, const double *Urp, int x, int u,
                              double *res_out, hipStream_t s);
void launch_rollout(int model, int N, int M, const double *x0, const double *U, const double *params, double *X, hipStream_t s);
void launch_shift_plan(int model, int N, int M, int sh, const double *X, const double *U, const double *params, const double *U_tail, double *Xn,
                       double *Un, double *um1n, hipStream_t s);
bool model_known(int model);
bool jac_compact_dims(int model, int x, int u);
long long jac_compact_doubles(int model, int N, int M);
void launch_expand_jac(int model, int N, int M, const double *jc, double *fx, double *fu, int orient, hipStream_t s);
int jac_live_mask(int model, unsigned char *fx_mask, unsigned char *fu_mask);
void launch_linearize_with_residual(int model, int N, int M, const double *x0, const double *X_prev, const double *U_prev,
                                    const double *params, double *f, double *fx, double *fu, const double *Xr, const double *Xrp,
                                    const double *Ur, const double *Urp, int x, int u, double *res_out, hipStream_t s, int jac32 = 0);
void launch_widen_f32(const float *src, double *dst, long long n, hipStream_t s);
bool f32_as_dims_supported(int x, int u);
void launch_scp_residual(const double *X, const double *Xp, const double *U, const double *Up, long long rows, int x, int u,
                         double *out, hipStream_t s, bool zero_out = true);
```

pmpc_amd/csrc/solver.hip:

```cpp
#include <dlfcn.h>

#include "solver_internal.h"
#include "cost_lin.h"

namespace {

struct Rccl {
  void *h = nullptr;
  ncclResult_t (*GetUniqueId)(ncclUniqueId *) = nullptr;
  ncclResult_t (*CommInitRank)(ncclComm_t *, int, ncclUniqueId, int) = nullptr;
  ncclResult_t (*CommDestroy)(ncclComm_t) = nullptr;
  ncclResult_t (*AllReduce)(const void *, void *, size_t, ncclDataType_t, ncclRedOp_t, ncclComm_t, hipStream_t) = nullptr;
  ncclResult_t (*Broadcast)(const void *, void *, size_t, ncclDataType_t, int, ncclComm_t, hipStream_t) = nullptr;
  bool load() {
    if (h) return true;
    const char *names[] = {"librccl.so", "librccl.so.1", "/opt/rocm/lib/librccl.so"};
    for (const char *n : names)
      if ((h = dlopen(n, RTLD_NOW | RTLD_GLOBAL))) break;
    if (!h) return false;
    GetUniqueId = (decltype(GetUniqueId))dlsym(h, "ncclGetUniqueId");
    CommInitRank = (decltype(CommInitRank))dlsym(h, "ncclCommInitRank");
    CommDestroy = (decltype(CommDestroy))dlsym(h, "ncclCommDestroy");
    AllReduce = (decltype(AllReduce))dlsym(h, "ncclAllReduce");
    Broadcast = (decltype(Broadcast))dlsym(h, "ncclBroadcast");
// ... 287 lines not shown
      c->opt[k] = value;
      c->fp_key = -1;
      c->ws.as_key = c->ws.warm_key = c->cone_rw_key = c->cone_lam_key = c->ws.es_key = -1;
      return 0;
    }
  return -1;
}
int pmpc_get_option(pmpc_ctx *c, const char *key, double *value) {
  if (!c || !key || !value) return -1;
  for (int k = 0; k < OPT_COUNT; k++)
    if (!strcmp(key, kPmpcOptions[k].key)) {
      *value = c->opt[k];
      return 0;
    }
  return -1;
}

void pmpc_destroy(pmpc_ctx *c) {
  if (!c) return;
  (void)hipSetDevice(c->device);
  (void)hipStreamSynchronize(c->stream);
  if (c->comm && c->mock_comm) delete (MockRank *)c->comm;
  else if (c->comm && g_rccl.CommDestroy) g_rccl.CommDestroy(c->comm);
  Workspace &w = c->ws;
  DevBuf *all[] = {&w.X, &w.U, &w.dX, &w.dU, &w.dX2, &w.dU2, &w.xm, &w.xd, &w.um, &w.ud, &w.K, &w.Hinv, &w.kff, &w.gc_part, &w.Hc_part, &w.Hc_w, &w.gc_w, &w.cons_w, &w.epi_lam, &w.epi_out, &w.epi_gath, &w.es_Dx, &w.es_wx, &w.es_Du, &w.es_wu, &w.es_xm, &w.es_xd, &w.es_um, &w.es_ud, &w.es_kff2, &w.es_kff3, &w.es_gc2, &w.es_dots, &w.es_coef, &w.es_out2, &w.es_Xt, &w.es_Ut, &w.es_U, &w.es_zero, &w.scratch,
                   &w.red_tmp, &w.Hg, &w.Lc, &w.duc, &w.xch, &w.zeros, &w.zslew, &w.zslew0, &w.zum1, &w.part_sum, &w.part_cnt,
                   &w.part_max, &w.sc, &w.fail, &w.pw, &w.Jc, &w.Jg, &w.part_dev, &w.warmU, &w.lateX, &w.lateU, &w.warm_llu, &w.warm_luu, &w.warm_llx,
                   &w.warm_lux, &w.Hadd, &w.wu_soc, &w.soc_zl, &w.soc_zu, &w.soc_zc, &w.soc_dzl, &w.soc_dzu, &w.soc_dzc, &w.soc_sl, &w.soc_su, &w.soc_sc, &w.soc_dsl,
                   &w.soc_dsu, &w.soc_dsc, &w.soc_cl, &w.soc_cu, &w.soc_cc, &w.soc_wU, &w.soc_wzl, &w.soc_wzu, &w.soc_wzc, &w.as_act, &w.as_cnt, &w.as_cntp, &w.as_settled, &w.cons_lo, &w.cons_hi, &w.as_ctl, &w.as_delta, &w.as_viol, &w.as_ck, &w.as_jhi, &w.ck_stat, &w.Hc_grp, &w.as_T, &w.xb_qmax, &w.as_perm,
                   &w.sa_f, &w.sa_fx, &w.sa_fu, &w.sa_Xp, &w.sa_Up, &w.sa_Q, &w.sa_R, &w.sa_Xr, &w.sa_Ur, &w.sa_lo, &w.sa_hi, &w.sa_Xo, &w.sa_Uo,
                   &w.sa_cl, &w.sa_ch, &w.cone_A, &w.cone_c, &w.cone_z, &w.cone_rec, &w.cone_uraw, &w.as_open, &w.xb_z, &w.xb_st, &w.xb_D, &w.xb_g, &w.m64[0], &w.m64[1], &w.m64[2], &w.m64[3], &w.cost_ref[0], &w.cost_ref[1], &w.cost_bad};
  for (DevBuf *b : all) b->release();
  for (SlabBufs *sb : {&w.sx, &w.su})
    for (DevBuf *b : {&sb->lo, &sb->hi, &sb->tl, &sb->tu, &sb->ll, &sb->lu, &sb->cl, &sb->cu, &sb->D, &sb->w}) b->release();
  for (DevBuf &b : c->stage) b.release();
  (void)hipHostFree(c->mirror);
  if (c->pinned) (void)hipHostFree(c->pinned);
  if (c->sm_pinned) (void)hipHostFree(c->sm_pinned);
  c->host_flags.release();
  free(c->sc_host);
  free(c->fail_host);
  (void)hipStreamDestroy(c->stream);
  delete c;
}

void *pmpc_stream(pmpc_ctx *c) { return (void *)c->stream; }
void pmpc_sync(pmpc_ctx *c) { HIP_WARN(hipStreamSynchronize(c->stream)); }

void pmpc_profile_enable(pmpc_ctx *c, int level) { c->prof = level < 0 ? 0 : level; }

void pmpc_profile_read(pmpc_ctx *c, double *ms4, long long *n4) {
  HIP_WARN(hipStreamSynchronize(c->stream));
  for (int k = 0; k < 8; k++) {
    ProfCat &pc = c->cat[k];
    for (auto &ev : pc.pending) {
      float t = 0.f;
      HIP_WARN(hipEventElapsedTime(&t, ev.first, ev.second));
      pc.ms += t;
      pc.n++;
      pc.pool.push_back(ev);
    }
    pc.pending.clear();
    if (k < 4) { ms4[k] = pc.ms; n4[k] = pc.n; }
    else if (k == 4) { c->partial_ms = pc.ms; c->partial_n = pc.n; }
    c->last_ms[k] = pc.ms;
    c->last_n[k] = pc.n;
    pc.ms = 0.0;
    pc.n = 0;
  }
}

void pmpc_profile_read_all(pmpc_ctx *c, double *ms, long long *n, int count) {
  for (int k = 0; k < count && k < 8; k++) { ms[k] = c->last_ms[k]; n[k] = c->last_n[k]; }
}

void pmpc_profile_read_partial(pmpc_ctx *c, double *ms, long long *n) {
  *ms = c->partial_ms;
  *n = c->partial_n;
}

void pmpc_restart_stats(pmpc_ctx *c, unsigned long long *out4, int reset) {
  for (int k = 0; k < 4; k++) out4[k] = 0;
  if (!c || !c->ws.ck_stat.p) return;
  (void)hipSetDevice(c->device);
  HIP_WARN(hipStreamSynchronize(c->stream));
  HIP_WARN(hipMemcpy(out4, c->ws.ck_stat.p, 4 * sizeof(unsigned long long), hipMemcpyDeviceToHost));
  if (reset) HIP_WARN(hipMemset(c->ws.ck_stat.p, 0, 4 * sizeof(unsigned long long)));
}

int pmpc_comm_unique_id(void *out128) {
  if (!g_rccl.load()) return 1;
  ncclUniqueId id;
  if (g_rccl.GetUniqueId(&id) != ncclSuccess) return 2;
  memcpy(out128, &id, sizeof(id));
  return 0;
}

int pmpc_comm_init(pmpc_ctx *c, int rank, int world, const void *id128) {
  const char *single = getenv("PMPC_RCCL_SINGLE");
  if (world <= 1 && !(single && single[0] == '1')) {
    c->rank = 0;
    c->world = 1;
    return 0;
  }
  if (world <= 1) { world = 1; rank = 0; c->single_rank_comm = true; }
  if (!g_rccl.load()) return 1;
  if (hipSetDevice(c->device) != hipSuccess) return 3;
  ncclUniqueId id;
  memcpy(&id, id128, sizeof(id));
  if (g_rccl.CommInitRank(&c->comm, world, id, rank) != ncclSuccess) return 2;
  c->rank = rank;
  c->world = world;
  return 0;
}
int pmpc_comm_init_mock(pmpc_ctx *c, int rank, int world, int group) {
  std::lock_guard<std::mutex> lk(g_mock_mutex);
  MockGroup *&g = g_mock_groups[group];
  if (!g) {
    g = new MockGroup();
    g->world = world;
    g->slot.resize(world);
  }
  if (g->world != world || rank < 0 || rank >= world) return 1;
  g_rccl.AllReduce = mock_allreduce;
  g_rccl.Broadcast = mock_broadcast;
  c->comm = (ncclComm_t) new MockRank{g, rank};
  c->mock_comm = true;
  c->rank = rank;
  c->world = world;
  return 0;
}
int pmpc_comm_rank(pmpc_ctx *c) { return c->rank; }
int pmpc_comm_world(pmpc_ctx *c) { return c->world; }

int pmpc_scp_residual_device(pmpc_ctx *c, size_t xdim, size_t udim, size_t N, size_t M, const double *X, const double *X_prev,
                             const double *U, const double *U_prev, double *out) {
  try {
    HIP_CHECK(hipSetDevice(c->device));
    ProfScope ps(c, 7);
    launch_scp_residual(X, X_prev, U, U_prev, (long long)M * (long long)N, (int)xdim, (int)udim, out, c->stream);
    HIP_CHECK(hipGetLastError());
  } catch (const PmpcHipError &) {
    return 2;
  }
  return 0;
}

int pmpc_linearize_device_f32(pmpc_ctx *c, int model, size_t N, size_t M, const double *x0, const double *X_prev,
                              const double *U_prev, const double *params, double *f, float *fx, float *fu) {
  try {
    HIP_CHECK(hipSetDevice(c->device));
    if (!model_known(model)) return 2;
    ProfScope ps(c, 6);
    launch_linearize(model, (int)N, (int)M, x0, X_prev, U_prev, params, f, (double *)fx, (double *)fu, c->stream, 1);
    HIP_CHECK(hipGetLastError());
  } catch (const PmpcHipError &) {
    return 2;
  }
  return 0;
}

int pmpc_linearize_device(pmpc_ctx *c, int model, size_t N, size_t M, const double *x0, const double *X_prev,
                          const double *U_prev, const double *params, double *f, double *fx, double *fu) {
  try {
    HIP_CHECK(hipSetDevice(c->device));
    if (!model_known(model)) return 2;
    ProfScope ps(c, 6);
    launch_linearize(model, (int)N, (int)M, x0, X_prev, U_prev, params, f, fx, fu, c->stream);
    HIP_CHECK(hipGetLastError());
  } catch (const PmpcHipError &) {
// ... 185 lines not shown
  g.slew0 = has_slew0 ? p->slew_reg0 : w.zslew0.d();
  g.um1 = has_slew0 ? p->slew_um1 : w.zum1.d();
  if (has_ub && Nc > 0) {
    const size_t nc = (size_t)Nc * u;
    w.sa_cl.ensure(nc * D8); w.sa_ch.ensure(nc * D8);
    HIP_CHECK(hipMemcpyAsync(w.sa_cl.p, p->lu, nc * D8, hipMemcpyDeviceToDevice, s));
    HIP_CHECK(hipMemcpyAsync(w.sa_ch.p, p->uu, nc * D8, hipMemcpyDeviceToDevice, s));
    if (c->multi()) {
      broadcast(c, w.sa_cl.p, nc, ncclFloat64, 0);
      broadcast(c, w.sa_ch.p, nc, ncclFloat64, 0);
    }
    g.cons_lo = w.sa_cl.d(); g.cons_hi = w.sa_ch.d();
  }
  g.af = w.sa_f.d(); g.afx = w.sa_fx.d(); g.afu = w.sa_fu.d(); g.aXp = w.sa_Xp.d(); g.aUp = w.sa_Up.d();
  g.aQ = w.sa_Q.d(); g.aR = w.sa_R.d(); g.aXr = w.sa_Xr.d(); g.aUr = w.sa_Ur.d();
  g.alo = boxes ? w.sa_lo.d() : nullptr; g.ahi = boxes ? w.sa_hi.d() : nullptr;
  launch_slew_augment(g, s);

  q = *p;
  q.xdim = (size_t)n;
  q.flags &= ~(PMPC_HAS_SLEW | PMPC_HAS_SLEW0 | PMPC_HAS_UBOUNDS | PMPC_HAS_XBOUNDS | PMPC_PREV_IS_LAST_SOLUTION | PMPC_STATIC_CONS_BOUNDS);
  if (boxes) q.flags |= PMPC_HAS_XBOUNDS;
  q.reg_x = reg;
  q.reg_u = 0.0;
  q.f = g.af; q.fx = g.afx; q.fu = g.afu; q.X_prev = g.aXp; q.U_prev = g.aUp; q.Q = g.aQ; q.R = g.aR; q.X_ref = g.aXr; q.U_ref = g.aUr;
  q.lx = g.alo; q.ux = g.ahi; q.lu = q.uu = nullptr;
  q.slew_reg = q.slew_reg0 = q.slew_um1 = nullptr;
  q.X_out = w.sa_Xo.d(); q.U_out = w.sa_Uo.d();
}

int solve_slew_increment_form(pmpc_ctx *c, const pmpc_problem *p, pmpc_info *info, int verbose) {
  hipStream_t s = c->stream;
  Workspace &w = c->ws;
  const int x = (int)p->xdim, u = (int)p->udim, N = (int)p->N, M = (int)p->M;
  const int Nc = p->Nc < 0 ? N : (int)p->Nc;
  const size_t rows = (size_t)M * N;
  pmpc_problem q;
  SlewAug g;
  build_slew_increment_problem(c, p, q, g);
  pmpc_info inf;
  memset(&inf, 0, sizeof(inf));
  c->xb_ctrl_from = x;
  int st;
  try {
    st = solve_impl_body(c, &q, &inf, verbose, false);
  } catch (...) {
    c->xb_ctrl_from = -1;
    throw;
  }
  c->xb_ctrl_from = -1;
  if (st == 0) launch_slew_split(w.sa_Xo.d(), w.sa_Uo.d(), p->X_out, p->U_out, (long long)rows, x, u, N, (M > 1 || c->multi()) ? Nc : 0, g.cons_lo, g.cons_hi, s);
  else fill_nan_outputs(c, p);
  if (info) *info = inf;
  return st;
}


int pmpc_scp_loop_device(pmpc_ctx *c, int model, const double *params, const pmpc_problem *p0, double *f2, double *fx2, double *fu2,
                         int steps, int first_cold, double *res, pmpc_info *infos, int *last_in_out) {
  return pmpc_scp_loop_device_cost(c, model, params, p0, f2, fx2, fu2, steps, first_cold, res, infos, last_in_out, nullptr);
}
int pmpc_scp_loop_device_cost(pmpc_ctx *c, int model, const double *params, const pmpc_problem *p0, double *f2, double *fx2, double *fu2,
                              int steps, int first_cold, double *res, pmpc_info *infos, int *last_in_out, const pmpc_scp_cost *cost) {
  pmpc_problem p = *p0;
  const bool with_cost = cost != nullptr && cost->kind != 0;
  double *Xr[2] = {nullptr, nullptr};
  unsigned *cost_bad = nullptr;
  auto shift = [&](int set, const double *X) {
    if (!with_cost) return;
    launch_obstacle_ref_shift(*cost, (int)p0->xdim, (int)p0->N, (int)p0->M, X, p0->Q, p0->X_ref, Xr[set], cost_bad, c->stream);
  };
  double *XA = const_cast<double *>(p0->X_prev), *UA = const_cast<double *>(p0->U_prev), *XB = p0->X_out, *UB = p0->U_out;
  double *F[2][3] = {{const_cast<double *>(p0->f), const_cast<double *>(p0->fx), const_cast<double *>(p0->fu)}, {f2, fx2, fu2}};
  const bool soc = p0->soc_u_interior != nullptr || p0->cone_count > 0;
  const bool cone_obj = (p0->flags & PMPC_CONE_OBJECTIVE) != 0;
  const int jac32 = (p0->flags & PMPC_F32_MATRICES) ? 1 : 0;
  static const bool lin_compact_env = !(getenv("PMPC_LIN_COMPACT") && atoi(getenv("PMPC_LIN_COMPACT")) == 0);
  const bool compact_ok = lin_compact_env && !cone_obj && !jac32 && !c->multi() && p0->Nc >= 0 && p0->Nc <= 1 &&
                          jac_compact_dims(model, (int)p0->xdim, (int)p0->udim) && (p0->flags & PMPC_SYMMETRIC_COST) &&
                          !(p0->flags & (PMPC_HAS_SLEW | PMPC_HAS_SLEW0 | PMPC_FORCE_GENERIC | PMPC_COLD_START)) &&
                          ((p0->flags & PMPC_HAS_UBOUNDS) || soc) && !(p0->barrier_mu > 0.0) && c->opt[OPT_AS_DEFECT] != 0.0 &&
                          c->opt[OPT_AS_WARM] != 0.0 && c->opt[OPT_POLISH_MU] > 0.0;
  bool compact_set[2] = {false, false};
  int done = 0, cur = 0;
  if (!model_known(model) || (with_cost && (jac32 || !obstacle_cost_valid(cost, (int)p0->xdim)))) {
    if (infos && steps > 0) { memset(&infos[0], 0, sizeof(pmpc_info)); infos[0].status = 2; }
    if (last_in_out) *last_in_out = 0;
    return 0;
  }
  bool lin_ready = false;
  try {
    HIP_CHECK(hipSetDevice(c->device));
    HIP_CHECK(hipMemsetAsync(res, 0, (size_t)steps * sizeof(double), c->stream));
    if (with_cost) {
      for (DevBuf &b : c->ws.cost_ref) b.ensure((size_t)p0->M * p0->N * p0->xdim * sizeof(double));
      Xr[0] = c->ws.cost_ref[0].d(); Xr[1] = c->ws.cost_ref[1].d();
      cost_bad = cost_bad_counter(c);
    }
    for (; done < steps; done++) {
      double *Xp = (done & 1) ? XB : XA, *Up = (done & 1) ? UB : UA, *Xo = (done & 1) ? XA : XB, *Uo = (done & 1) ? UA : UB;
      if (!lin_ready) {
        ProfScope ps(c, 6);
        compact_set[cur] = compact_ok && (done > 0 || !first_cold);
        if (compact_set[cur])
          launch_linearize_compact(model, (int)p.N, (int)p.M, p.x0, Xp, Up, params, F[cur][0], F[cur][1], nullptr, nullptr, nullptr, nullptr, 0, 0, nullptr, c->stream);
        else
          launch_linearize(model, (int)p.N, (int)p.M, p.x0, Xp, Up, params, F[cur][0], F[cur][1], F[cur][2], c->stream, jac32);
        shift(cur, Xp);
      }
      p.f = F[cur][0]; p.fx = F[cur][1]; p.fu = F[cur][2];
      if (with_cost) p.X_ref = Xr[cur];
      c->jac_compact_fx = compact_set[cur] ? F[cur][1] : nullptr;
      c->jac_compact_model = model;
      p.X_prev = Xp; p.U_prev = Up; p.X_out = Xo; p.U_out = Uo;
      p.flags = p0->flags | PMPC_STATIC_CONS_BOUNDS;
      if (done > 0 || !first_cold) p.flags |= PMPC_PREV_IS_LAST_SOLUTION;
      else p.flags &= ~(unsigned)PMPC_PREV_IS_LAST_SOLUTION;
      bool res_dirty = false;
      auto follow_up = [&, Xp, Up, Xo, Uo](bool with_next_lin) {
        const bool next = with_next_lin && done + 1 < steps;
        if (next && !res_dirty && !c->multi()) {
          ProfScope ps(c, 6);
          compact_set[cur ^ 1] = compact_ok;
          if (compact_ok)
            launch_linearize_compact(model, (int)p.N, (int)p.M, p.x0, Xo, Uo, params, F[cur ^ 1][0], F[cur ^ 1][1], Xo, Xp, Uo, Up, (int)p.xdim,
                                     (int)p.udim, res + done, c->stream);
          else
            launch_linearize_with_residual(model, (int)p.N, (int)p.M, p.x0, Xo, Uo, params, F[cur ^ 1][0], F[cur ^ 1][1], F[cur ^ 1][2], Xo, Xp, Uo,
                                           Up, (int)p.xdim, (int)p.udim, res + done, c->stream, jac32);
          shift(cur ^ 1, Xo);
          res_dirty = true;
          return;
        }
        {
          ProfScope ps(c, 7);
          launch_scp_residual(Xo, Xp, Uo, Up, (long long)p.M * (long long)p.N, (int)p.xdim, (int)p.udim, res + done, c->stream, res_dirty);
          res_dirty = true;
        }
        if (c->multi()) allreduce(c, res + done, 1, ncclFloat64, ncclMax);
        if (next) {
          ProfScope ps(c, 6);
          compact_set[cur ^ 1] = compact_ok;
          if (compact_ok)
            launch_linearize_compact(model, (int)p.N, (int)p.M, p.x0, Xo, Uo, params, F[cur ^ 1][0], F[cur ^ 1][1], nullptr, nullptr, nullptr, nullptr, 0, 0, nullptr, c->stream);
          else
            launch_linearize(model, (int)p.N, (int)p.M, p.x0, Xo, Uo, params, F[cur ^ 1][0], F[cur ^ 1][1], F[cur ^ 1][2], c->stream, jac32);
          shift(cur ^ 1, Xo);
        }
      };
      c->spec_fired = c->spec_ok = false;
      c->post_batch = [&]() { follow_up(true); };
      pmpc_info inf;
      const int st = cone_obj ? lcone_body(c, &p, p.barrier_mu > 0.0 ? 1.0 / p.barrier_mu : std::numeric_limits<double>::quiet_NaN(), &inf, 0)
                              : solve_impl(c, &p, &inf, 0, soc);
      c->post_batch = nullptr;
      c->jac_compact_fx = nullptr;
      if (infos) infos[done] = inf;
      if (st != 0) break;
      if (c->spec_fired && c->spec_ok) {
        lin_ready = true;
      } else {
        follow_up(false);
        lin_ready = false;
      }
      cur ^= 1;
    }
    HIP_CHECK(hipGetLastError());
  } catch (const PmpcHipError &) {
    c->post_batch = nullptr;
    c->jac_compact_fx = nullptr;
    if (infos && done < steps) { memset(&infos[done], 0, sizeof(pmpc_info)); infos[done].status = 2; }
    fail_after_error(c, nullptr, nullptr);
    try {
      const double nan = std::numeric_limits<double>::quiet_NaN();
      const long long ex = (long long)p.M * p.N * p.xdim, eu = (long long)p.M * p.N * p.udim;
      for (double *b : {XA, XB}) if (b) launch_fill(b, nan, ex, c->stream);
      for (double *b : {UA, UB}) if (b) launch_fill(b, nan, eu, c->stream);
      HIP_WARN(hipStreamSynchronize(c->stream));
    } catch (...) {
    }
  }
  if (last_in_out) *last_in_out = done & 1;
  return done;
}

}
```

pmpc_amd/csrc/solver_internal.h:

```cpp
#pragma once
#include <dlfcn.h>
#include <rccl/rccl.h>

#include <algorithm>
#include <chrono>
#include <cmath>
#include <condition_variable>
#include <cstring>
#include <functional>
#include <map>
#include <atomic>
#include <mutex>
#include <thread>
#include <limits>
#include <vector>

#include "../../include/pmpc_abi.h"
#include "pmpc_dev.h"

namespace pmpc_impl {

struct DevBuf {
  void *p = nullptr;
  size_t bytes = 0;
  bool ensure(size_t b) {
    if (b <= bytes) return false;
    if (p) HIP_WARN(hipFree(p));
    p = nullptr;
    bytes = 0;
    HIP_CHECK(hipMalloc(&p, b ? b : 8));
    bytes = b;
    return true;
  }
  void release() {
    if (p) (void)hipFree(p);
    p = nullptr;
    bytes = 0;
  }
  double *d() const { return (double *)p; }
};

struct SlabBufs {
  DevBuf lo, hi, tl, tu, ll, lu, cl, cu, D, w;
};

struct Workspace {
  DevBuf X, U, dX, dU, dX2, dU2, xm, xd, um, ud, K, Hinv, kff, gc_part, Hc_part, scratch, red_tmp, Hg , Lc, duc;
  DevBuf Hc_w, gc_w, cons_w, epi_lam, epi_out, epi_gath;
  DevBuf Hc_grp;
  DevBuf es_Dx, es_wx, es_Du, es_wu, es_xm, es_xd, es_um, es_ud, es_kff2, es_kff3, es_gc2, es_dots, es_coef, es_out2, es_Xt, es_Ut, es_U, es_zero;
  long long es_key = -1;
  DevBuf xch, zeros, zslew, zslew0, zum1, part_sum, part_cnt, part_max, sc, fail;
  DevBuf pw, Jc, Jg;
  DevBuf soc_zl, soc_zu, soc_zc, soc_dzl, soc_dzu, soc_dzc, soc_sl, soc_su, soc_sc, soc_dsl, soc_dsu, soc_dsc;
  DevBuf soc_cl, soc_cu, soc_cc;
  DevBuf soc_wU, soc_wzl, soc_wzu, soc_wzc;
  long long soc_key = -1;
  DevBuf Hadd, wu_soc;
  DevBuf cone_A, cone_c, cone_z, cone_rec, cone_uraw, as_open;
  DevBuf xb_qmax;
  DevBuf xb_z, xb_st, xb_D, xb_g;
  DevBuf jac_tmp;
  DevBuf cost_ref[2];
  DevBuf cost_bad;
  DevBuf m64[4];
  DevBuf warmU, warm_llu, warm_luu, warm_llx, warm_lux;
  DevBuf lateX, lateU;
  long long warm_key = -1;
  double warm_mu = 0.0;
  DevBuf as_perm;
  int as_perm_m = -1;
  DevBuf as_T;
  DevBuf as_ck, as_jhi, ck_stat;
  DevBuf as_act, as_cnt, as_cntp, as_settled, as_ctl, as_delta, as_viol;
  long long su_key = -1;
  const double *su_src_lo = nullptr, *su_src_hi = nullptr;
  bool as_U_valid = false;
  int as_pred_rounds = 3;
  DevBuf cons_lo, cons_hi;
  long long cons_key = -1;
  long long xb_block_key = -1;
  int xb_warm_backoff = 0, xb_warm_fails = 0;
  long long as_key = -1;
  double as_scale = 1.0;
  DevBuf part_dev;
  DevBuf sa_f, sa_fx, sa_fu, sa_Xp, sa_Up, sa_Q, sa_R, sa_Xr, sa_Ur, sa_lo, sa_hi, sa_Xo, sa_Uo, sa_cl, sa_ch;
  SlabBufs sx, su;
};


enum PmpcOpt {
  OPT_AS_WARM, OPT_AS_SKIP, OPT_AS_DEFECT, OPT_AS_COLD_ROUNDS, OPT_POLISH_MU, OPT_WARM_START, OPT_CONE_AS, OPT_CONE_COLD_ROUNDS, OPT_XBOX_AS,
  OPT_SLEW_INCREMENT_BOXES, OPT_AS_FUSE_CTL, OPT_AS_WAVE_CONS, OPT_HOST_REUSE, OPT_WARN_SLOW_PATH, OPT_CONE_RANK_MEMORY, OPT_CONE_EPIGRAPH, OPT_COND_GROUPED, OPT_AS_FREEZE_TOL, OPT_AS_CKPT, OPT_AS_SENS_MIN_M, OPT_AS_PERM_MIN_M, OPT_CONE_PATH, OPT_COUNT
};
}
using namespace pmpc_impl;

struct ProfCat {
  std::vector<std::pair<hipEvent_t, hipEvent_t>> pending, pool;
  double ms = 0.0;
  long long n = 0;
};

struct pmpc_ctx {
  double opt[OPT_COUNT];
  bool warned_slow_path = false;
  std::vector<double> cone_rw;
  long long cone_rw_key = -1;
  long long fp_key = -1;
  int fp_ok = -1;
  std::vector<double> cone_lam;
  long long cone_lam_key = -1;
  double cone_rho = 0.0;
  std::vector<double> cons_w_host, epi_lam_host;
  const double *cons_w_active = nullptr;
  int xb_ctrl_from = -1;
  AsCtlCall as_pend{};
  int prof = 0;
  double partial_ms = 0.0;
  long long partial_n = 0;
  double last_ms[8] = {0};
  long long last_n[8] = {0};
  ProfCat cat[8];
  int device = 0;
  hipStream_t stream = nullptr;
  Workspace ws;
  IpmScal *sc_host = nullptr;
  int *fail_host = nullptr;
  struct ScMirror { IpmScal sc; unsigned long long seq; int as_cnt[4]; unsigned long long as_seq; AsCtl ctl; double epi[4]; unsigned long long epi_seq; };
  ScMirror *mirror = nullptr, *mirror_dev = nullptr;
  unsigned long long seq = 0, as_seq = 0, epi_seq = 0;
  ncclComm_t comm = nullptr;
  bool mock_comm = false;
  int rank = 0, world = 1;
  bool single_rank_comm = false;
  bool multi() const { return world > 1 || single_rank_comm; }
  DevBuf stage[19], stage_t[4];
  void *pinned = nullptr;
  void *sm_pinned = nullptr;
  size_t sm_pinned_bytes = 0;
  size_t pinned_bytes = 0;
  struct StagedChunk { void *dst; size_t bytes, off; };
  std::vector<StagedChunk> staged;
  DevBuf host_flags;
  std::function<void()> post_batch;
  bool spec_fired = false, spec_ok = false;
  const double *jac_compact_fx = nullptr;
  int jac_compact_model = 0;
};

namespace pmpc_impl {

void allreduce(pmpc_ctx *c, void *buf, size_t n, ncclDataType_t dt, ncclRedOp_t op);
void broadcast(pmpc_ctx *c, void *buf, size_t n, ncclDataType_t dt, int root);

struct ProfScope {
  pmpc_ctx *c;
  int k;
  std::pair<hipEvent_t, hipEvent_t> ev;
  bool on;
  ProfScope(pmpc_ctx *c_, int k_) : c(c_), k(k_), on(c_->prof >= 2 || (c_->prof == 1 && k_ == 0)) {
    if (!on) return;
    ProfCat &pc = c->cat[k];
    if (pc.pool.empty()) {
      HIP_CHECK(hipEventCreate(&ev.first));
      HIP_CHECK(hipEventCreate(&ev.second));
    } else {
      ev = pc.pool.back();
      pc.pool.pop_back();
    }
    HIP_CHECK(hipEventRecord(ev.first, c->stream));
  }
  ~ProfScope() {
    if (!on) return;
    HIP_WARN(hipEventRecord(ev.second, c->stream));
    c->cat[k].pending.push_back(ev);
  }
};

template <class Pred>
bool spin_until(Pred ready, double limit_s = 2.0) {
  const auto t0 = std::chrono::steady_clock::now();
  for (;;) {
    for (int k = 0; k < 1024; k++) {
      if (ready()) return true;
      __builtin_ia32_pause();
    }
    if (std::chrono::duration<double>(std::chrono::steady_clock::now() - t0).count() > limit_s) return ready();
  }
}
void wait_published(pmpc_ctx *c, volatile unsigned long long *seq, unsigned long long want);
void read_scalars(pmpc_ctx *c);
void exchange(pmpc_ctx *c, int phase);
void structured_solve(pmpc_ctx *c, LQArgs &a, bool factor, bool fast, bool prep_done = false);
int fail_after_error(pmpc_ctx *c, const pmpc_problem *p, pmpc_info *info);
void fill_nan_outputs(pmpc_ctx *c, const pmpc_problem *p);

}

constexpr int PMPC_NEEDS_F64 = -7;

extern "C" {
pmpc_problem widened_f32_problem(pmpc_ctx *c, const pmpc_problem *p, bool jacobians = true);
void build_slew_increment_problem(pmpc_ctx *c, const pmpc_problem *p, pmpc_problem &q, SlewAug &g);
int lcone_body(pmpc_ctx *c, const pmpc_problem *p, double smooth_alpha, pmpc_info *info, int verbose);
int solve_impl_body(pmpc_ctx *c, const pmpc_problem *p, pmpc_info *info, int verbose, bool soc);
bool slew_increment_form_applies(const pmpc_ctx *c, const pmpc_problem *p, bool soc);
int solve_slew_increment_form(pmpc_ctx *c, const pmpc_problem *p, pmpc_info *info, int verbose);
}
```

pmpc_amd/csrc/solver_qp.hip:

```cpp
#include "solver_internal.h"

namespace {

constexpr int GO_ON = -1000;

struct AsAttempt {
  double dual_scale;
  int mode, max_rounds;
  LQArgs b;
  ConeArgs ca;
  XboxArgs xa;
  int *act;
  AsCtl *ctl;
  bool cone, xbox;
  bool refused;
  bool use_defect;
  AsCtl h;
  int round;
  int n_batches_at_hook;
};

class QpSolve {
 public:
  QpSolve(pmpc_ctx *c_, const pmpc_problem *p_, pmpc_info *info_, int verbose_, bool soc_)
// ... 469 lines not shown
    fl = measure(nblk, mu_new);
    if (fl) {
      status = (mu <= 1e2 * mu_tol) ? 0 : (fl == 3 ? 3 : 2);
      break;
    }
    if (verbose) printf("pmpc_hip: soc it %3d  mu %9.3e -> %9.3e  alpha_aff %6.4f  sigma %8.2e  alpha %6.4f\n", newton, mu, mu_new, a_aff, sigma, alpha);
    const bool stalled = alpha < 1e-3 && mu <= 1e2 * mu_tol;
    mu = mu_new;
    if (!remembered && !soc_warm_off && mu <= 0.5) {
      for (DevBuf *b : {&w.soc_wU, &w.soc_wzl, &w.soc_wzu}) b->ensure(nu * D8);
      w.soc_wzc.ensure(ncz * D8);
      HIP_CHECK(hipMemcpyAsync(w.soc_wU.p, w.U.p, nu * D8, hipMemcpyDeviceToDevice, s));
      HIP_CHECK(hipMemcpyAsync(w.soc_wzl.p, sa.zl, nu * D8, hipMemcpyDeviceToDevice, s));
      HIP_CHECK(hipMemcpyAsync(w.soc_wzu.p, sa.zu, nu * D8, hipMemcpyDeviceToDevice, s));
      HIP_CHECK(hipMemcpyAsync(w.soc_wzc.p, sa.zc, ncz * D8, hipMemcpyDeviceToDevice, s));
      w.soc_key = skey;
      remembered = true;
    }
    if (mu <= mu_tol || stalled) { status = 0; break; }
  }
  if (status != 0 && warm) {
    if (verbose) printf("pmpc_hip: stage cones: warm-started run failed (status %d), cold start\n", status);
    warm = false; remembered = false; status = 1; newton = 0;
    w.soc_key = -1;
    HIP_CHECK(hipMemsetAsync(w.fail.p, 0, sizeof(int), s));
    goto soc_restart;
  }
  inf.ipm_iters = newton;
  inf.mu = mu;
  if (verbose) printf("pmpc_hip: stage cones: status %d after %d Newton steps\n", status, newton);
  return (finish_now || status != 0) ? finish(status) : 0;
}

int QpSolve::equality_phase() {
  reset_scalars();
  equality_solve();
  if (has_xb) launch_violation(sx, w.part_max.d(), s);
  if (has_ub) launch_violation(su, w.part_max.d() + B, s);
  exchange(c, 1);
  read_scalars(c);
  inf.max_violation = c->sc_host->viol_max;
  if (*c->fail_host || !(c->sc_host->viol_max == c->sc_host->viol_max)) return 2;
  if (verbose) printf("pmpc_hip: equality-only optimum, max bound violation %.3e\n", c->sc_host->viol_max);
  if (!has_xb && !has_ub) return 0;
  if (c->sc_host->viol_max <= 0.0 && mu_target == 0.0) return 0;
  return 1;
}

int QpSolve::active_set_fast(double dual_scale, int mode, int max_rounds, int xb) {
  if (!(mode == 0 && as_defect_on && (p->flags & PMPC_PREV_IS_LAST_SOLUTION) && Nc <= 1)) densify();
  AsAttempt t = as_blocks(dual_scale, mode, max_rounds, xb);
  if (t.refused || !as_start(t)) return 1;
  as_rounds(t);
  return as_accept(t);
}

AsAttempt QpSolve::as_blocks(double dual_scale, int mode, int max_rounds, int xb) {
  AsAttempt t;
  memset(&t, 0, sizeof(t));
  t.dual_scale = dual_scale; t.mode = mode; t.max_rounds = max_rounds;
  LQArgs &b = t.b;
  ConeArgs &ca = t.ca;
  XboxArgs &xa = t.xa;
  const double big = 1e30, tol_p = 1e-13;
  w.as_act.ensure(nu * sizeof(int) + 8); w.as_cntp.ensure((size_t)M * 3 * sizeof(int)); w.as_settled.ensure((size_t)M * sizeof(int));
  w.as_ctl.ensure(sizeof(AsCtl)); w.as_delta.ensure((size_t)std::max(nc, 1) * D8);
  int *act = t.act = (int *)w.as_act.p;
  AsCtl *ctl = t.ctl = (AsCtl *)w.as_ctl.p;
  b = a;
  b.Dx = b.wx = b.Du = b.wu = nullptr; b.du_full = 0;
  b.as_act = act; b.as_lo = su.lo; b.as_hi = su.hi; b.as_cnt = (int *)w.as_cntp.p; b.as_big = big; b.as_tol_p = tol_p;
  b.as_settled_out = (int *)w.as_settled.p; b.as_delta = w.as_delta.d(); b.as_ctl = ctl; b.done = &ctl->done;
  w.as_viol.ensure((size_t)M * D8);
  b.as_viol = w.as_viol.d();
  b.Xb = p->X_out; b.Ub = p->U_out; b.Xo = p->X_out; b.Uo = p->U_out;
  {
    int slots = 0;
    if (c->opt[OPT_AS_CKPT] != 0.0 && as_skip_on && nc <= 32)
      while ((PMPC_AS_CK_FIRST << slots) <= N - 1) slots++;
    if (slots > 0) {
      const int ks = (x + 3) / 4;
      w.as_ck.ensure((size_t)M * slots * (64 * ks + 32) * D8);
      w.as_jhi.ensure((size_t)M * sizeof(int));
      if (w.ck_stat.ensure(4 * sizeof(unsigned long long))) HIP_CHECK(hipMemsetAsync(w.ck_stat.p, 0, 4 * sizeof(unsigned long long), s));
      b.as_ck = w.as_ck.d(); b.as_jhi = (int *)w.as_jhi.p; b.ck_slots = slots; b.ck_stat = (unsigned long long *)w.ck_stat.p;
    }
  }
  w.as_key = -1;
  const bool cone = t.cone = cone_as && (mode == 0 || mode == 3 || mode == 5);
  b.as_freeze_tol = (cone && Nc == 1) ? c->opt[OPT_AS_FREEZE_TOL] : 0.0;
  if (cone) {
    const int q = (int)p->soc_q;
    const size_t rows = (size_t)M * N;
    w.Hadd.ensure(nu * u * D8); w.wu_soc.ensure(nu * D8); w.cone_uraw.ensure(nu * D8); w.as_open.ensure((size_t)M * sizeof(int));
    const bool z_new = w.cone_z.ensure(rows * cone_rows * D8), rec_new = w.cone_rec.ensure(rows * std::max(ncones, 1) * PMPC_CONE_REC * D8);
    if (z_new || rec_new) w.as_key = -1;
    b.cone_H = w.Hadd.d(); b.cone_g = w.wu_soc.d(); b.as_uraw = w.cone_uraw.d(); b.as_open = (int *)w.as_open.p;
    ca.M = M; ca.N = N; ca.u = u; ca.q = q; ca.Nc = Nc; ca.owner = a.owner;
    ca.rows = cone_rows;
    if (ncones > 0) {
      ca.ncones = ncones; ca.per_stage = p->cone_per_stage ? 1 : 0;
      for (int k = 0; k < ncones; k++) ca.qs[k] = p->cone_sizes[k];
      ca.A = p->cone_A; ca.c = p->cone_c;
    } else {
      ca.ncones = 1; ca.qs[0] = q; ca.per_stage = 0;
      ca.A = w.cone_A.d(); ca.c = w.cone_c.d();
    }
    ca.R = p->R; ca.r32 = a.mat32; ca.reg_u = p->reg_u; ca.rho_scale = 1e7;
    ca.z = w.cone_z.d(); ca.rec = w.cone_rec.d(); ca.H = w.Hadd.d(); ca.g = w.wu_soc.d();
    ca.cnt = (int *)w.as_cntp.p; ca.settled = (int *)w.as_settled.p; ca.open = (int *)w.as_open.p; ca.done = &ctl->done; ca.ctl = ctl;
    ca.jhi = b.as_jhi;
    ca.tol_step = 1e-6; ca.tol_phi = 1e-9;
    ca.dual_scale = dual_scale;
  }
  const bool xbox = t.xbox = xbox_as && xb != 0;
  {
    const int min_m = (int)c->opt[OPT_AS_SENS_MIN_M];
    if (min_m > 0 && M >= min_m && as_skip_on && Nc == 1 && (mode != 0 || w.as_pred_rounds >= 2)) {
      w.as_T.ensure((size_t)M * N * 64 * D8);
      b.as_T = w.as_T.d();
    }
  }
  if (xbox) {
    w.as_open.ensure((size_t)M * sizeof(int)); w.xb_D.ensure(nx * D8); w.xb_g.ensure(nx * D8);
    const bool z_new = w.xb_z.ensure(nx * D8), st_new = w.xb_st.ensure(nx * sizeof(int));
    if ((z_new || st_new) && mode == 0) { t.refused = true; return t; }
    if (mode == 2 || xb == 2) {
      HIP_CHECK(hipMemsetAsync(w.xb_z.p, 0, nx * D8, s));
      HIP_CHECK(hipMemsetAsync(w.xb_st.p, 0, nx * sizeof(int), s));
    } else if (mode == 1) {
      launch_xbox_from_ipm(sx, (int *)w.xb_st.p, w.xb_z.d(), s);
    }
    b.xb_D = w.xb_D.d(); b.xb_g = w.xb_g.d(); b.as_open = (int *)w.as_open.p;
    xa.M = M; xa.N = N; xa.x = x; xa.lo = p->lx; xa.hi = p->ux; xa.Q = p->Q; xa.pw = p->weights; xa.reg_x = p->reg_x; xa.rho_scale = 1e7;
    w.xb_qmax.ensure((size_t)M * D8);
    xa.qmax = w.xb_qmax.d();
    xa.z = w.xb_z.d(); xa.st = (int *)w.xb_st.p; xa.D = w.xb_D.d(); xa.g = w.xb_g.d();
    xa.cnt = (int *)w.as_cntp.p; xa.settled = (int *)w.as_settled.p; xa.open = (int *)w.as_open.p; xa.done = &ctl->done; xa.ctl = ctl;
    xa.jhi = b.as_jhi;
    xa.tol = 1e-9; xa.dual_scale = dual_scale;
    xa.z_tol = 1e-3;
    xa.keep_on_clamp = 1;
    xa.act_frac = 0.5;
    xa.ctrl_from = c->xb_ctrl_from >= 0 ? c->xb_ctrl_from : x;
  }
  return t;
}

bool QpSolve::as_start(AsAttempt &t) {
  LQArgs &b = t.b;
  ConeArgs &ca = t.ca;
  XboxArgs &xa = t.xa;
  const int mode = t.mode, max_rounds = t.max_rounds;
  const double dual_scale = t.dual_scale, big = b.as_big;
  const bool cone = t.cone, xbox = t.xbox;
  int *act = t.act;
  AsCtl *ctl = t.ctl;
  launch_as_begin(ctl, (int *)w.fail.p, max_rounds, dual_scale, s, cone ? 8 : (xbox ? (c->xb_ctrl_from >= 0 ? 8 : (mode == 0 ? 6 : 3)) : 2));
  const bool use_defect = t.use_defect = mode == 0 && as_defect_on && (p->flags & PMPC_PREV_IS_LAST_SOLUTION);
  if (a.mat32 && !use_defect) return false;
  if (mode == 3) {
    ProfScope ps(c, 5);
    HIP_CHECK(hipMemsetAsync(act, 0, nu * sizeof(int) + 8, s));
    HIP_CHECK(hipMemsetAsync(w.cone_z.p, 0, (size_t)M * N * cone_rows * D8, s));
    if (p->soc_u_interior) launch_soc_fill_u(p->U_out, p->soc_u_interior, (long long)nu, u, s);
    else launch_init_base(p->U_out, p->U_prev, M, N, u, Nc, s);
    launch_rollout_fast(b, p->U_out, p->X_out, s);
// ... 22 lines not shown
    ca.finish = 0;
    ca.U = use_defect ? p->U_prev : p->U_out;
    launch_cone_step(ca, s);
  }
  return true;
}

void QpSolve::as_rounds(AsAttempt &t) {
  LQArgs &b = t.b;
  ConeArgs &ca = t.ca;
  XboxArgs &xa = t.xa;
  const int mode = t.mode, max_rounds = t.max_rounds;
  const bool cone = t.cone, xbox = t.xbox, use_defect = t.use_defect;
  AsCtl *ctl = t.ctl;
  AsCtl &h = t.h;
  int &round = t.round, &n_batches_at_hook = t.n_batches_at_hook;
  const bool fuse_env = c->opt[OPT_AS_FUSE_CTL] != 0.0 && c->opt[OPT_AS_WAVE_CONS] != 0.0;
  const bool fuse_ctl = fuse_env && !c->multi() && Nc == 1;
  const int *open_part = (cone || xbox) ? (const int *)w.as_open.p : nullptr;
  const int perm_min_m = (int)c->opt[OPT_AS_PERM_MIN_M];
  round = 0;
  int depth = mode == 0 ? std::max(1, std::min(w.as_pred_rounds, max_rounds)) : std::min(3, max_rounds);
  if (verbose > 1 && xbox) depth = 1;
  static const bool duc_trace = getenv("PMPC_DUC_TRACE") != nullptr;
  if (duc_trace) depth = 1;
  n_batches_at_hook = -1000;
  memset(&h, 0, sizeof(h));
  while (true) {
    const int batch = std::min(depth, max_rounds - round);
    for (int k = 0; k < batch; k++) {
      const int r = round + k;
      b.defect = (use_defect && r == 0) ? p->f : nullptr;
      const bool skip = as_skip_on && r > 0 && nc <= 32;
      b.as_settled_in = skip ? (const int *)w.as_settled.p : nullptr;
      b.as_perm = nullptr;
      if (skip && perm_min_m > 0 && M >= perm_min_m && b.as_T) {
        ProfScope pp(c, 5);
        if (w.as_perm.ensure((size_t)M * sizeof(int)) || w.as_perm_m != M) {
          std::vector<int> id(M);
          for (int q_ = 0; q_ < M; q_++) id[q_] = q_;
          HIP_CHECK(hipMemcpyAsync(w.as_perm.p, id.data(), (size_t)M * sizeof(int), hipMemcpyHostToDevice, s));
          HIP_CHECK(hipStreamSynchronize(s));
          w.as_perm_m = M;
        }
        static const bool perm_fused = !(getenv("PMPC_AS_PERM_FUSED") && atoi(getenv("PMPC_AS_PERM_FUSED")) == 0);
        if (c->as_pend.ctl && perm_fused) {
          c->as_pend.settled = (const int *)w.as_settled.p;
          c->as_pend.perm = (int *)w.as_perm.p;
        } else {
          launch_as_perm((const int *)w.as_settled.p, M, (int *)w.as_perm.p, &ctl->done, s);
        }
        b.as_perm = (const int *)w.as_perm.p;
      }
      const bool last = k == batch - 1;
      const bool merge = c->multi() && nc > 0;
      b.as_merge = merge ? (k == 0 ? 1 : 2) : 0;
      c->as_seq++;
      structured_solve(c, b, true, true, true);
      ProfScope ps(c, 5);
      if (cone) {
        ca.finish = 1;
        ca.U = p->U_out; ca.Uraw = w.cone_uraw.d();
        launch_cone_step(ca, s);
      }
      if (xbox) {
        xa.finish = 1;
        xa.X = p->X_out;
        launch_xbox_step(xa, s);
      }
      if (merge) {
        if (last) {
          double *tl = w.Hg.d() + (size_t)nc * nc + nc;
          launch_as_ctl(ctl, (const int *)w.as_cntp.p, M, (const int *)w.fail.p, 1, 0, 0, nullptr, nullptr, 0, s, tl, nullptr, open_part);
          allreduce(c, tl, 5, ncclFloat64, ncclSum);
          launch_as_ctl(ctl, nullptr, M, (const int *)w.fail.p, 0, 1, 1, &c->mirror_dev->ctl, &c->mirror_dev->as_seq, c->as_seq, s, tl);
        }
      } else if (c->multi()) {
        launch_as_ctl(ctl, (const int *)w.as_cntp.p, M, (const int *)w.fail.p, 1, 0, 0, nullptr, nullptr, 0, s, nullptr, nullptr, open_part);
        allreduce(c, &ctl->open, 5, ncclInt32, ncclSum);
        launch_as_ctl(ctl, nullptr, M, (const int *)w.fail.p, 0, 1, last ? 1 : 0, &c->mirror_dev->ctl, &c->mirror_dev->as_seq, c->as_seq, s);
      } else if (!last && fuse_ctl) {
        c->as_pend = AsCtlCall{ctl, (const int *)w.as_cntp.p, M, (const int *)w.fail.p, &c->mirror_dev->ctl, &c->mirror_dev->as_seq, c->as_seq,
                               b.as_viol, open_part, nullptr, nullptr};
      } else {
        launch_as_ctl(ctl, (const int *)w.as_cntp.p, M, (const int *)w.fail.p, 1, 1, last ? 1 : 0, &c->mirror_dev->ctl, &c->mirror_dev->as_seq, c->as_seq, s,
                      nullptr, b.as_viol, open_part);
      }
    }
    if (round == 0 && c->post_batch) {
      std::function<void()> hook;
      hook.swap(c->post_batch);
      c->spec_fired = true;
      n_batches_at_hook = 0;
      hook();
    }
    n_batches_at_hook++;
    {
      const unsigned long long lo_seq = c->as_seq - (unsigned long long)batch + 1, hi_seq = c->as_seq;
      const bool seen = spin_until([&] {
        const unsigned long long v = *(volatile unsigned long long *)&c->mirror->as_seq;
        return v >= lo_seq && v <= hi_seq;
      });
      if (!seen) {
        HIP_CHECK(hipStreamSynchronize(s));
        const unsigned long long v = *(volatile unsigned long long *)&c->mirror->as_seq;
        if (!(v >= lo_seq && v <= hi_seq)) throw PmpcHipError{-1, "active-set control block never published", __FILE__, __LINE__};
      }
      __atomic_thread_fence(__ATOMIC_ACQUIRE);
      memcpy(&h, (const void *)&c->mirror->ctl, sizeof(h));
    }
    if (verbose)
      for (int r = round; r < h.round && r < 16; r++)
        printf("pmpc_hip: active set (%s) round %d: %d released, %d activated (largest violation behind a change %.2e)\n",
               mode == 5 ? "finish" : (mode == 4 ? "state rows" : (mode >= 2 ? "cold" : (mode ? "finish" : "warm"))), r + 1, h.hist[r][0], h.hist[r][1], h.worst[r]);
    if (verbose && cone) printf("pmpc_hip: active set: %d stage cones still open after round %d\n", h.open, h.round);
    if (duc_trace && nc > 0 && !a.cons_G) {
      std::vector<double> hd(nc);
      HIP_CHECK(hipMemcpy(hd.data(), w.as_delta.p, nc * D8, hipMemcpyDeviceToHost));
      double m = 0.0;
      for (double v : hd) m = std::max(m, std::fabs(v));
      int nset = 0;
      { std::vector<int> hs(M); HIP_CHECK(hipMemcpy(hs.data(), w.as_settled.p, M * sizeof(int), hipMemcpyDeviceToHost)); for (int v : hs) nset += v; }
      printf("pmpc_hip: trace: round %d max |du_c| %.3e, %d of %d particles settled\n", h.round, m, nset, M);
      if (b.as_jhi) {
        std::vector<int> hj(M), hs(M), hist(N + 1, 0);
        HIP_CHECK(hipMemcpy(hj.data(), w.as_jhi.p, M * sizeof(int), hipMemcpyDeviceToHost));
        HIP_CHECK(hipMemcpy(hs.data(), w.as_settled.p, M * sizeof(int), hipMemcpyDeviceToHost));
        for (int q = 0; q < M; q++) if (!hs[q]) hist[hj[q] < 0 ? N : hj[q]]++;
        printf("pmpc_hip: trace:   highest changed stage:");
        for (int q = 0; q <= N; q++) if (hist[q]) printf(" %d:%d", q == N ? -1 : q, hist[q]);
        printf("\n");
      }
    }
  if (verbose > 1 && xbox) dump_state_rows(h.round);
  if (verbose > 1 && cone) dump_cone_records();
    inf.structured_solves += h.round - round;
    inf.active_set_rounds += h.round - round;
    round = h.round;
    if (h.done || round >= max_rounds) break;
    depth = 1;
  }
}

void QpSolve::dump_state_rows(int round) {
    HIP_CHECK(hipStreamSynchronize(s));
    std::vector<double> hz(nx), hX(nx), hU(nu);
    std::vector<int> hs(nx), hact(nu);
    HIP_CHECK(hipMemcpy(hz.data(), w.xb_z.p, nx * D8, hipMemcpyDeviceToHost));
    HIP_CHECK(hipMemcpy(hs.data(), w.xb_st.p, nx * sizeof(int), hipMemcpyDeviceToHost));
    HIP_CHECK(hipMemcpy(hX.data(), p->X_out, nx * D8, hipMemcpyDeviceToHost));
    HIP_CHECK(hipMemcpy(hU.data(), p->U_out, nu * D8, hipMemcpyDeviceToHost));
    HIP_CHECK(hipMemcpy(hact.data(), w.as_act.p, nu * sizeof(int), hipMemcpyDeviceToHost));
    int held = 0, uheld = 0, wi = 0;
    double zmax = 0.0, xmax = 0.0;
    for (size_t k = 0; k < nx; k++) {
      held += hs[k] != 0;
      if (hz[k] > zmax) { zmax = hz[k]; wi = (int)(k / ((size_t)N * x)); }
      xmax = std::max(xmax, std::fabs(hX[k]));
    }
    for (size_t k = 0; k < nu; k++) uheld += hact[k] != 0;
    printf("   state rows after round %d: %d held, %d controls held, largest multiplier %.3e (particle %d), largest |x| %.3e\n", round, held, uheld, zmax, wi, xmax);
    if (getenv("PMPC_XB_DUMP")) {
      const int pi = atoi(getenv("PMPC_XB_DUMP"));
      for (int j = 0; j < N; j++) {
        printf("     p%d j%2d st", pi, j);
        for (int r = 0; r < x; r++) printf(" %d", hs[((size_t)pi * N + j) * x + r]);
        printf(" | act");
        for (int r = 0; r < u; r++) printf(" %d", hact[((size_t)pi * N + j) * u + r]);
        printf(" | v");
        for (int r = 3; r < 6 && r < x; r++) printf(" %+.4f", hX[((size_t)pi * N + j) * x + r]);
        printf(" | z");
        for (int r = 3; r < 6 && r < x; r++) printf(" %.3e", hz[((size_t)pi * N + j) * x + r]);
        printf(" | u");
        for (int r = 0; r < u; r++) printf(" %+.4f", hU[((size_t)pi * N + j) * u + r]);
        printf("\n");
      }
    }
// ... 436 lines not shown
```

Baseline: 3011 SCP iterations/s.

## Ride final active-set control block on speculative linearise kernel launch

Defers the last-of-batch active-set control reduction so it runs as an extra leading block inside the speculative next-iteration linearise kernel, which removes one kernel launch per SCP iteration on the host-spin path. It also replaces the shared-memory tree reductions and scan in the control and permutation blocks with wavefront shuffle reductions, and optionally computes the SCP residual inline inside the linearise blocks. Restart statistics move to per-particle slots that are summed on demand. The added coupling makes the control publish depend on linearise block scheduling, and the control block can now run at the same time as linearise work.

```diff
diff --git a/include/pmpc_abi.h b/include/pmpc_abi.h
--- a/include/pmpc_abi.h
+++ b/include/pmpc_abi.h
@@ -130,6 +130,7 @@
 
 int pmpc_as_sweep_launches(int sweep, unsigned long long *out, int n, int reset);
 void pmpc_as_sweep_knobs(int *out);
+int pmpc_as_perm_debug(const int *settled, int M, int *perm, int threads);
 
 int pmpc_scp_residual_device(pmpc_ctx *ctx, size_t xdim, size_t udim, size_t N, size_t M, const double *X, const double *X_prev,
                              const double *U, const double *U_prev, double *out);
diff --git a/pmpc_amd/_lib.py b/pmpc_amd/_lib.py
--- a/pmpc_amd/_lib.py
+++ b/pmpc_amd/_lib.py
@@ -21,7 +21,7 @@
     "pmpc_scp_residual_device", "pmpc_profile_read_partial", "pmpc_profile_read_all", "pmpc_scp_loop_device", "pmpc_linearize_device_f32",
     "pmpc_set_option", "pmpc_get_option", "pmpc_abi_struct_sizes", "pmpc_lcone_solve_host_ex", "pmpc_restart_stats",
     "pmpc_linearize_compact_device", "pmpc_expand_jac_device", "pmpc_jac_compact_doubles", "pmpc_jac_live_mask",
-    "pmpc_as_sweep_variant", "pmpc_as_sweep_launches", "pmpc_as_sweep_knobs",
+    "pmpc_as_sweep_variant", "pmpc_as_sweep_launches", "pmpc_as_sweep_knobs", "pmpc_as_perm_debug",
     "pmpc_ref_shift_device", "pmpc_ref_shift_bad_pivots", "pmpc_obstacle_cost_grad_device", "pmpc_obstacle_ref_shift_device",
     "pmpc_scp_loop_device_cost", "pmpc_abi_scp_cost_size",
     "pmpc_rollout_device", "pmpc_shift_plan_device",
@@ -131,6 +131,9 @@
         lib.pmpc_as_sweep_launches.restype = ctypes.c_int
         lib.pmpc_as_sweep_knobs.argtypes = [ctypes.POINTER(ctypes.c_int)]
         lib.pmpc_as_sweep_knobs.restype = None
+    if hasattr(lib, "pmpc_as_perm_debug"):
+        lib.pmpc_as_perm_debug.argtypes = [ctypes.POINTER(ctypes.c_int), ctypes.c_int, ctypes.POINTER(ctypes.c_int), ctypes.c_int]
+        lib.pmpc_as_perm_debug.restype = ctypes.c_int
     lib.pmpc_scp_residual_device.argtypes = [vp, sz, sz, sz, sz] + [vp] * 5
     lib.pmpc_scp_residual_device.restype = ctypes.c_int
     lib.pmpc_profile_enable.argtypes = [vp, ctypes.c_int]
@@ -236,6 +239,15 @@
     return tuple(out)
 
 
+def as_perm_debug(settled, threads: int = 0):
+    flags = np.ascontiguousarray(settled, dtype=np.int32)
+    perm = np.empty(flags.size, dtype=np.int32)
+    ip = ctypes.POINTER(ctypes.c_int)
+    if load().pmpc_as_perm_debug(flags.ctypes.data_as(ip), int(flags.size), perm.ctypes.data_as(ip), int(threads)) != 0:
+        raise RuntimeError("pmpc_as_perm_debug refused its arguments or hit a HIP error")
+    return perm
+
+
 def dptr(a: np.ndarray):
     assert a.dtype == np.float64 and a.flags["C_CONTIGUOUS"]
     return a.ctypes.data_as(c_dp)
diff --git a/pmpc_amd/csrc/as_ctl_dev.h b/pmpc_amd/csrc/as_ctl_dev.h
--- a/pmpc_amd/csrc/as_ctl_dev.h
+++ b/pmpc_amd/csrc/as_ctl_dev.h
@@ -3,11 +3,40 @@
 
 namespace {
 
+__device__ inline void as_ctl_reduce_tree(int &r, int &d, int &b, int &op, double &vw) {
+  __shared__ int sh[4][1024];
+  __shared__ double shv[1024];
+  sh[0][threadIdx.x] = r; sh[1][threadIdx.x] = d; sh[2][threadIdx.x] = b; sh[3][threadIdx.x] = op; shv[threadIdx.x] = vw;
+  __syncthreads();
+  for (int o = 512; o > 0; o >>= 1) {
+    if (threadIdx.x < o) {
+      sh[0][threadIdx.x] += sh[0][threadIdx.x + o];
+      sh[1][threadIdx.x] += sh[1][threadIdx.x + o];
+      sh[2][threadIdx.x] |= sh[2][threadIdx.x + o];
+      sh[3][threadIdx.x] += sh[3][threadIdx.x + o];
+      shv[threadIdx.x] = fmax(shv[threadIdx.x], shv[threadIdx.x + o]);
+    }
+    __syncthreads();
+  }
+  r = sh[0][0]; d = sh[1][0]; b = sh[2][0]; op = sh[3][0]; vw = shv[0];
+}
+__device__ inline void as_ctl_reduce_waves(int &r, int &d, int &b, int &op, double &vw) {
+  __shared__ int shw[4][16];
+  __shared__ double shvw[16];
+  for (int o = 32; o > 0; o >>= 1) {
+    r += __shfl_xor(r, o, 64); d += __shfl_xor(d, o, 64); b |= __shfl_xor(b, o, 64); op += __shfl_xor(op, o, 64);
+    vw = fmax(vw, __shfl_xor(vw, o, 64));
+  }
+  const int wv = threadIdx.x >> 6, nw = blockDim.x >> 6;
+  if ((threadIdx.x & 63) == 0) { shw[0][wv] = r; shw[1][wv] = d; shw[2][wv] = b; shw[3][wv] = op; shvw[wv] = vw; }
+  __syncthreads();
+  if (threadIdx.x == 0)
+    for (int w = 1; w < nw; w++) { r += shw[0][w]; d += shw[1][w]; b |= shw[2][w]; op += shw[3][w]; vw = fmax(vw, shvw[w]); }
+}
+
 __device__ inline void as_ctl_block(AsCtl *ctl, const int *cnt_part, int M, const int *fail, int reduce, int decide, int last_of_batch,
                                                  AsCtl *mirror, unsigned long long *mirror_seq, unsigned long long seq, double *tail, const double *viol,
-                                                 const int *open_part = nullptr) {
-  __shared__ int sh[4][1024];
-  __shared__ double shv[1024];
+                                                 const int *open_part = nullptr, int tree = 0) {
   if (ctl->done) {
     if (threadIdx.x == 0 && decide && last_of_batch && mirror) {
       *mirror = *ctl;
@@ -19,27 +48,17 @@
   if (reduce) {
     int r = 0, d = 0, b = 0, op = 0;
     double vw = 0.0;
-    for (int i = threadIdx.x; i < M; i += 1024) {
+    for (int i = threadIdx.x; i < M; i += blockDim.x) {
       r += cnt_part[3 * i]; d += cnt_part[3 * i + 1]; b |= cnt_part[3 * i + 2];
       if (viol) vw = fmax(vw, viol[i]);
       if (open_part) op += open_part[i];
     }
-    sh[0][threadIdx.x] = r; sh[1][threadIdx.x] = d; sh[2][threadIdx.x] = b; sh[3][threadIdx.x] = op; shv[threadIdx.x] = vw;
-    __syncthreads();
-    for (int o = 512; o > 0; o >>= 1) {
-      if (threadIdx.x < o) {
-        sh[0][threadIdx.x] += sh[0][threadIdx.x + o];
-        sh[1][threadIdx.x] += sh[1][threadIdx.x + o];
-        sh[2][threadIdx.x] |= sh[2][threadIdx.x + o];
-        sh[3][threadIdx.x] += sh[3][threadIdx.x + o];
-        shv[threadIdx.x] = fmax(shv[threadIdx.x], shv[threadIdx.x + o]);
-      }
-      __syncthreads();
-    }
-    if (threadIdx.x == 0 && viol && ctl->round < 16) ctl->worst[ctl->round] = shv[0];
+    if (tree) as_ctl_reduce_tree(r, d, b, op, vw);
+    else as_ctl_reduce_waves(r, d, b, op, vw);
+    if (threadIdx.x == 0 && viol && ctl->round < 16) ctl->worst[ctl->round] = vw;
     if (threadIdx.x == 0) {
-      if (tail) { tail[0] = sh[0][0]; tail[1] = sh[1][0]; tail[2] = sh[2][0]; tail[3] = *fail; tail[4] = sh[3][0]; }
-      else { ctl->cnt[0] = sh[0][0]; ctl->cnt[1] = sh[1][0]; ctl->cnt[2] = sh[2][0]; ctl->cnt[3] = *fail; ctl->open = sh[3][0]; }
+      if (tail) { tail[0] = r; tail[1] = d; tail[2] = b; tail[3] = *fail; tail[4] = op; }
+      else { ctl->cnt[0] = r; ctl->cnt[1] = d; ctl->cnt[2] = b; ctl->cnt[3] = *fail; ctl->open = op; }
     }
   }
   if (threadIdx.x == 0 && decide) {
@@ -77,21 +96,40 @@
   }
 }
 
-__device__ inline void as_perm_block(const int *settled, int M, int *perm) {
+__device__ inline void as_perm_block(const int *settled, int M, int *perm, int tree = 0) {
   __shared__ int cnt[1024];
-  const int t = threadIdx.x, per = (M + 1023) / 1024, lo = t * per, hi = min(M, lo + per);
+  const int nt = tree ? 1024 : (int)blockDim.x;
+  const int t = threadIdx.x, per = (M + nt - 1) / nt, lo = min(M, t * per), hi = min(M, lo + per);
   int n = 0;
   for (int i = lo; i < hi; i++) n += settled[i] ? 0 : 1;
-  cnt[t] = n;
-  __syncthreads();
-  for (int o = 1; o < 1024; o <<= 1) {
-    const int v = t >= o ? cnt[t - o] : 0;
+  int incl, total;
+  if (tree) {
+    cnt[t] = n;
     __syncthreads();
-    cnt[t] += v;
+    for (int o = 1; o < 1024; o <<= 1) {
+      const int v = t >= o ? cnt[t - o] : 0;
+      __syncthreads();
+      cnt[t] += v;
+      __syncthreads();
+    }
+    incl = cnt[t]; total = cnt[1023];
+  } else {
+    const int lane = t & 63, wv = t >> 6, nw = nt >> 6;
+    incl = n;
+    for (int o = 1; o < 64; o <<= 1) {
+      const int v = __shfl_up(incl, o, 64);
+      if (lane >= o) incl += v;
+    }
+    if (lane == 63) cnt[wv] = incl;
     __syncthreads();
+    total = 0;
+    for (int w = 0; w < nw; w++) {
+      const int c = cnt[w];
+      if (w < wv) incl += c;
+      total += c;
+    }
   }
-  const int total = cnt[1023];
-  int pu = cnt[t] - n, ps = total + lo - pu;
+  int pu = incl - n, ps = total + lo - pu;
   for (int i = lo; i < hi; i++) {
     if (settled[i]) perm[ps++] = i;
     else perm[pu++] = i;
diff --git a/pmpc_amd/csrc/dynamics.hip b/pmpc_amd/csrc/dynamics.hip
--- a/pmpc_amd/csrc/dynamics.hip
+++ b/pmpc_amd/csrc/dynamics.hip
@@ -1,5 +1,6 @@
 #include "pmpc_dev.h"
 #include "jac_compact.h"
+#include "as_ctl_dev.h"
 #include <cstring>
 #include <cstdlib>
 
@@ -212,16 +213,55 @@
   const double *X, *Xp, *U, *Up;
   long long rows;
   int x, u, nblk;
+  int inl;
   unsigned long long *out_bits;
 };
 #ifndef PMPC_LIN_THREADS
 #define PMPC_LIN_THREADS 256
 #endif
+static_assert(PMPC_LIN_THREADS % 64 == 0 && PMPC_LIN_THREADS >= 128 && PMPC_LIN_THREADS <= 1024, "wave 0 evaluates the model, the other waves take the residual rows");
+__device__ __forceinline__ double residual_row_sq(const double *a, const double *b, int d) {
+  const int q = (d + 3) / 4;
+  double s[4];
+#pragma unroll
+  for (int sub = 0; sub < 4; sub++) {
+    const int k1 = min(d, (sub + 1) * q);
+    double acc = 0.0;
+    for (int k = sub * q; k < k1; k++) { const double t = a[k] - b[k]; acc = fma(t, t, acc); }
+    s[sub] = acc;
+  }
+  return (s[0] + s[1]) + (s[2] + s[3]);
+}
+__device__ __forceinline__ void residual_rows_inline(long long first, int n, const ResArgs &res, double *wave_max) {
+  const int t = threadIdx.x;
+  if (t < 64) return;
+  double m = 0.0;
+  for (int r = t - 64; r < 2 * n; r += PMPC_LIN_THREADS - 64) {
+    const bool isx = r < n;
+    const long long row = first + (isx ? r : r - n);
+    const int d = isx ? res.x : res.u;
+    const double acc = residual_row_sq((isx ? res.X : res.U) + row * d, (isx ? res.Xp : res.Up) + row * d, d);
+    m = (acc == acc) ? fmax(m, acc) : INFINITY;
+  }
+  for (int o = 32; o > 0; o >>= 1) m = fmax(m, __shfl_xor(m, o, 64));
+  if ((t & 63) == 0) wave_max[(t >> 6) - 1] = m;
+}
+__device__ __forceinline__ void residual_publish(const double *wave_max, unsigned long long *out_bits) {
+  double m = wave_max[0];
+  for (int w = 1; w < PMPC_LIN_THREADS / 64 - 1; w++) m = fmax(m, wave_max[w]);
+  const unsigned long long bits = (unsigned long long)__double_as_longlong(sqrt(m));
+  if (bits > *(volatile unsigned long long *)out_bits) atomicMax(out_bits, bits);
+}
+__device__ __forceinline__ void last_ctl_block(const AsCtlCall &q) {
+  as_ctl_block(q.ctl, q.cnt_part, q.M, q.fail, 1, 1, 1, q.mirror, q.mirror_seq, q.seq, nullptr, q.viol, q.open_part, 0);
+}
 template <class Model, class JT>
 __global__ void __launch_bounds__(PMPC_LIN_THREADS) k_linearize(int N, long long tot, const double *x0, const double *X_prev, const double *U_prev,
-                                                  const double *params, double *f, JT *fx, JT *fu, ResArgs res) {
+                                                  const double *params, double *f, JT *fx, JT *fu, ResArgs res, AsCtlCall last_ctl) {
   constexpr int X = Model::X, U = Model::U, UNITS = Model::UNITS;
+  const int lead = last_ctl.ctl ? 1 : 0;
   {
+    if (lead && blockIdx.x == 0) { last_ctl_block(last_ctl); return; }
     const int glin = (int)gridDim.x - res.nblk;
     if ((int)blockIdx.x >= glin) {
       residual_block((int)blockIdx.x - glin, res.nblk, res.X, res.Xp, res.rows, res.x, res.U, res.Up, res.rows, res.u, res.out_bits);
@@ -231,15 +271,18 @@
   constexpr int REC = X + X * X + X * U, LD = REC | 1;
   extern __shared__ double rec[];
   const int t = threadIdx.x;
-  const long long first = (long long)blockIdx.x * UNITS;
+  const long long first = (long long)((int)blockIdx.x - lead) * UNITS;
   for (int e = t; e < UNITS * LD; e += PMPC_LIN_THREADS) rec[e] = 0.0;
   __syncthreads();
+  const int n = (int)((tot - first) < UNITS ? (tot - first) : UNITS);
+  __shared__ double res_wave[PMPC_LIN_THREADS / 64];
+  if (res.inl) residual_rows_inline(first, n, res, res_wave);
   if (t < UNITS && first + t < tot) {
     double *mine = rec + t * LD;
     Model::eval(first + t, N, x0, X_prev, U_prev, params, mine, mine + X, mine + X + X * X);
   }
   __syncthreads();
-  const int n = (int)((tot - first) < UNITS ? (tot - first) : UNITS);
+  if (res.inl && t == 0) residual_publish(res_wave, res.out_bits);
   for (int e = t; e < n * X; e += PMPC_LIN_THREADS) f[first * X + e] = rec[(e / X) * LD + e % X];
   for (int e = t; e < n * X * X; e += PMPC_LIN_THREADS) fx[first * (X * X) + e] = (JT)rec[(e / (X * X)) * LD + X + e % (X * X)];
   for (int e = t; e < n * X * U; e += PMPC_LIN_THREADS) fu[first * (X * U) + e] = (JT)rec[(e / (X * U)) * LD + X + X * X + e % (X * U)];
@@ -247,24 +290,26 @@
 
 template <class Model>
 void launch_model(int N, int M, const double *x0, const double *X_prev, const double *U_prev, const double *params, double *f,
-                  double *fx, double *fu, const ResArgs &res, hipStream_t s, int jac32) {
+                  double *fx, double *fu, const ResArgs &res, hipStream_t s, int jac32, const AsCtlCall &last_ctl = AsCtlCall{}) {
   const long long tot = (long long)M * N;
   constexpr int REC = Model::X + Model::X * Model::X + Model::X * Model::U, LD = REC | 1;
-  const unsigned grid = (unsigned)((tot + Model::UNITS - 1) / Model::UNITS);
+  const unsigned grid = (unsigned)((tot + Model::UNITS - 1) / Model::UNITS) + (last_ctl.ctl ? 1u : 0u);
   if (jac32)
     hipLaunchKernelGGL((k_linearize<Model, float>), dim3(grid + (unsigned)res.nblk), dim3(PMPC_LIN_THREADS), Model::UNITS * LD * sizeof(double), s, N, tot, x0,
-                       X_prev, U_prev, params, f, (float *)fx, (float *)fu, res);
+                       X_prev, U_prev, params, f, (float *)fx, (float *)fu, res, last_ctl);
   else
     hipLaunchKernelGGL((k_linearize<Model, double>), dim3(grid + (unsigned)res.nblk), dim3(PMPC_LIN_THREADS), Model::UNITS * LD * sizeof(double), s, N, tot, x0,
-                       X_prev, U_prev, params, f, fx, fu, res);
+                       X_prev, U_prev, params, f, fx, fu, res, last_ctl);
 }
 constexpr int LIN_CUNITS = 64;
 template <class Model>
 __global__ void __launch_bounds__(PMPC_LIN_THREADS) k_linearize_compact(int N, long long tot, const double *x0, const double *X_prev, const double *U_prev,
-                                                                         const double *params, double *f, double *jc, ResArgs res) {
+                                                                         const double *params, double *f, double *jc, ResArgs res, AsCtlCall last_ctl) {
   typedef jacc::Compact<typename Model::Spec> C;
   constexpr int X = Model::X, U = Model::U, UNITS = LIN_CUNITS, REC = C::REC, POOL = C::POOL;
+  const int lead = last_ctl.ctl ? 1 : 0;
   {
+    if (lead && blockIdx.x == 0) { last_ctl_block(last_ctl); return; }
     const int glin = (int)gridDim.x - res.nblk;
     if ((int)blockIdx.x >= glin) {
       residual_block((int)blockIdx.x - glin, res.nblk, res.X, res.Xp, res.rows, res.x, res.U, res.Up, res.rows, res.u, res.out_bits);
@@ -274,7 +319,10 @@
   constexpr int LD = (X + REC) | 1;
   extern __shared__ double rec[];
   const int t = threadIdx.x;
-  const long long first = (long long)blockIdx.x * UNITS;
+  const long long first = (long long)((int)blockIdx.x - lead) * UNITS;
+  const int n = (int)((tot - first) < UNITS ? (tot - first) : UNITS);
+  __shared__ double res_wave[PMPC_LIN_THREADS / 64];
+  if (res.inl) residual_rows_inline(first, n, res, res_wave);
   if (t < UNITS && first + t < tot) {
     double J[X * X + X * U] = {};
     double *mine = rec + t * LD;
@@ -288,7 +336,7 @@
     }
   }
   __syncthreads();
-  const int n = (int)((tot - first) < UNITS ? (tot - first) : UNITS);
+  if (res.inl && t == 0) residual_publish(res_wave, res.out_bits);
   for (int e = t; e < n * X; e += PMPC_LIN_THREADS) f[first * X + e] = rec[(e / X) * LD + e % X];
   for (int e = t; e < n * REC; e += PMPC_LIN_THREADS) jc[first * REC + e] = rec[(e / REC) * LD + X + e % REC];
 }
@@ -310,13 +358,13 @@
 
 template <class Model>
 void launch_model_compact(int N, int M, const double *x0, const double *X_prev, const double *U_prev, const double *params, double *f,
-                          double *jc, const ResArgs &res, hipStream_t s) {
+                          double *jc, const ResArgs &res, hipStream_t s, const AsCtlCall &last_ctl = AsCtlCall{}) {
   typedef jacc::Compact<typename Model::Spec> C;
   const long long tot = (long long)M * N;
   constexpr int LD = (Model::X + C::REC) | 1;
-  const unsigned grid = (unsigned)((tot + LIN_CUNITS - 1) / LIN_CUNITS);
+  const unsigned grid = (unsigned)((tot + LIN_CUNITS - 1) / LIN_CUNITS) + (last_ctl.ctl ? 1u : 0u);
   hipLaunchKernelGGL((k_linearize_compact<Model>), dim3(grid + (unsigned)res.nblk), dim3(PMPC_LIN_THREADS), LIN_CUNITS * LD * sizeof(double), s, N, tot,
-                     x0, X_prev, U_prev, params, f, jc, res);
+                     x0, X_prev, U_prev, params, f, jc, res, last_ctl);
 }
 __global__ void __launch_bounds__(256) k_widen_f32(const float *src, double *dst, long long n) {
   for (long long k = (long long)blockIdx.x * 256 + threadIdx.x; k < n; k += (long long)gridDim.x * 256) dst[k] = (double)src[k];
@@ -396,6 +444,14 @@
   const long long cap = rows >= 200000 ? 1024 : 256;
   return nb > cap ? cap : nb;
 }
+static bool lin_res_inline() {
+  static const bool on = !(getenv("PMPC_LIN_RES_INLINE") && atoi(getenv("PMPC_LIN_RES_INLINE")) == 0);
+  return on;
+}
+static void ride(ResArgs &r) {
+  if (lin_res_inline()) { r.inl = 1; r.nblk = 0; }
+  else { r.inl = 0; r.nblk = (int)residual_blocks(r.rows); }
+}
 
 void launch_linearize(int model, int N, int M, const double *x0, const double *X_prev, const double *U_prev,
                       const double *params, double *f, double *fx, double *fu, hipStream_t s, int jac32) {
@@ -405,15 +461,16 @@
 }
 void launch_linearize_compact(int model, int N, int M, const double *x0, const double *X_prev, const double *U_prev, const double *params,
                               double *f, double *jc, const double *Xr, const double *Xrp, const double *Ur, const double *Urp, int x, int u,
-                              double *res_out, hipStream_t s) {
+                              double *res_out, hipStream_t s, const AsCtlCall *last_ctl) {
   ResArgs r;
   memset(&r, 0, sizeof(r));
   if (res_out) {
     r.X = Xr; r.Xp = Xrp; r.U = Ur; r.Up = Urp; r.rows = (long long)M * N; r.x = x; r.u = u;
-    r.nblk = (int)residual_blocks(r.rows);
+    ride(r);
     r.out_bits = (unsigned long long *)res_out;
   }
-  with_model(model, [&](auto m) { launch_model_compact<decltype(m)>(N, M, x0, X_prev, U_prev, params, f, jc, r, s); });
+  const AsCtlCall lc = (last_ctl && res_out) ? *last_ctl : AsCtlCall{};
+  with_model(model, [&](auto m) { launch_model_compact<decltype(m)>(N, M, x0, X_prev, U_prev, params, f, jc, r, s, lc); });
 }
 void launch_rollout(int model, int N, int M, const double *x0, const double *U, const double *params, double *X, hipStream_t s) {
   const unsigned grid = (unsigned)((M + ROLL_LANES - 1) / ROLL_LANES);
@@ -475,12 +532,14 @@
 
 void launch_linearize_with_residual(int model, int N, int M, const double *x0, const double *X_prev, const double *U_prev,
                                     const double *params, double *f, double *fx, double *fu, const double *Xr, const double *Xrp,
-                                    const double *Ur, const double *Urp, int x, int u, double *res_out, hipStream_t s, int jac32) {
+                                    const double *Ur, const double *Urp, int x, int u, double *res_out, hipStream_t s, int jac32,
+                                    const AsCtlCall *last_ctl) {
   ResArgs r;
   r.X = Xr; r.Xp = Xrp; r.U = Ur; r.Up = Urp; r.rows = (long long)M * N; r.x = x; r.u = u;
-  r.nblk = (int)residual_blocks(r.rows);
+  ride(r);
   r.out_bits = (unsigned long long *)res_out;
-  with_model(model, [&](auto m) { launch_model<decltype(m)>(N, M, x0, X_prev, U_prev, params, f, fx, fu, r, s, jac32); });
+  const AsCtlCall lc = last_ctl ? *last_ctl : AsCtlCall{};
+  with_model(model, [&](auto m) { launch_model<decltype(m)>(N, M, x0, X_prev, U_prev, params, f, fx, fu, r, s, jac32, lc); });
 }
 
 namespace {
diff --git a/pmpc_amd/csrc/kernels_as.hip b/pmpc_amd/csrc/kernels_as.hip
--- a/pmpc_amd/csrc/kernels_as.hip
+++ b/pmpc_amd/csrc/kernels_as.hip
@@ -70,8 +70,9 @@
     const int k = lo <= PMPC_AS_CK_FIRST ? 0 : 32 - __builtin_clz((unsigned)(lo - 1) >> PMPC_AS_CK_LOG);
     if (k < a.ck_slots) { ck_k = __builtin_amdgcn_readfirstlane(k + 1); jtop = PMPC_AS_CK_FIRST << (ck_k - 1); }
     if (lane == 0 && a.ck_stat) {
-      atomicAdd(a.ck_stat + (ck_k ? 0 : 2), 1ull);
-      atomicAdd(a.ck_stat + (ck_k ? 1 : 3), (unsigned long long)(jtop + 1));
+      unsigned long long *st = a.ck_stat + 4 * (size_t)i + (ck_k ? 0 : 2);
+      st[0] += 1ull;
+      st[1] += (unsigned long long)(jtop + 1);
     }
   }
   const double *ck_ = a.as_ck ? ubase(a.as_ck, (long long)i * a.ck_slots * (long long)(CKS * sizeof(double))) : nullptr;
@@ -831,13 +832,30 @@
 
 __global__ void __launch_bounds__(1024) k_as_ctl(AsCtl *ctl, const int *cnt_part, int M, const int *fail, int reduce, int decide, int last_of_batch,
                                                  AsCtl *mirror, unsigned long long *mirror_seq, unsigned long long seq, double *tail, const double *viol,
-                                                 const int *open_part) {
-  as_ctl_block(ctl, cnt_part, M, fail, reduce, decide, last_of_batch, mirror, mirror_seq, seq, tail, viol, open_part);
-}
-
-__global__ void __launch_bounds__(1024) k_as_perm(const int *settled, int M, int *perm, const int *done) {
+                                                 const int *open_part, int tree) {
+  as_ctl_block(ctl, cnt_part, M, fail, reduce, decide, last_of_batch, mirror, mirror_seq, seq, tail, viol, open_part, tree);
+}
+
+__global__ void __launch_bounds__(1024) k_as_perm(const int *settled, int M, int *perm, const int *done, int tree) {
   if (done && *done) return;
-  as_perm_block(settled, M, perm);
+  as_perm_block(settled, M, perm, tree);
+}
+
+__global__ void __launch_bounds__(256) k_ck_stat_sum(unsigned long long *slots, int M, int reset) {
+  __shared__ unsigned long long sh[256];
+  const int t = threadIdx.x, col = t & 3;
+  unsigned long long acc = 0;
+  for (int i = t >> 2; i < M; i += 64) {
+    acc += slots[4 * (size_t)i + col];
+    if (reset) slots[4 * (size_t)i + col] = 0;
+  }
+  sh[t] = acc;
+  __syncthreads();
+  if (t < 4) {
+    unsigned long long tot = 0;
+    for (int k = t; k < 256; k += 4) tot += sh[k];
+    slots[4 * (size_t)M + t] = tot;
+  }
 }
 
 template <class F>
@@ -946,10 +964,39 @@
 void launch_as_ctl(AsCtl *ctl, const int *cnt_part, int M, const int *fail, int reduce, int decide, int last_of_batch, AsCtl *mirror,
                    unsigned long long *mirror_seq, unsigned long long seq, hipStream_t s, double *tail, const double *viol, const int *open_part) {
   hipLaunchKernelGGL(k_as_ctl, dim3(1), dim3(1024), 0, s, ctl, cnt_part, M, fail, reduce, decide, last_of_batch, mirror, mirror_seq, seq, tail, viol,
-                     open_part);
+                     open_part, as_ctl_wave() ? 0 : 1);
 }
 void launch_as_perm(const int *settled, int M, int *perm, const int *done, hipStream_t s) {
-  hipLaunchKernelGGL(k_as_perm, dim3(1), dim3(1024), 0, s, settled, M, perm, done);
+  hipLaunchKernelGGL(k_as_perm, dim3(1), dim3(1024), 0, s, settled, M, perm, done, as_ctl_wave() ? 0 : 1);
+}
+void launch_ck_stat_sum(unsigned long long *slots, int M, int reset, hipStream_t s) {
+  hipLaunchKernelGGL(k_ck_stat_sum, dim3(1), dim3(256), 0, s, slots, M, reset);
+}
+bool as_ctl_wave() {
+  static const bool on = !(getenv("PMPC_AS_CTL_WAVE") && atoi(getenv("PMPC_AS_CTL_WAVE")) == 0);
+  return on;
+}
+int pmpc_as_perm_debug(const int *settled, int M, int *perm, int threads) {
+  if (threads == 0) threads = 1024;
+  if (!settled || !perm || M < 1 || threads < 64 || threads > 1024 || threads % 64) return -1;
+  int *ds = nullptr, *dp = nullptr;
+  try {
+    HIP_CHECK(hipMalloc(&ds, (size_t)M * sizeof(int)));
+    HIP_CHECK(hipMalloc(&dp, (size_t)M * sizeof(int)));
+    HIP_CHECK(hipMemcpy(ds, settled, (size_t)M * sizeof(int), hipMemcpyHostToDevice));
+    HIP_CHECK(hipMemset(dp, 0xff, (size_t)M * sizeof(int)));
+    hipLaunchKernelGGL(k_as_perm, dim3(1), dim3(threads), 0, 0, (const int *)ds, M, dp, (const int *)nullptr, (as_ctl_wave() || threads != 1024) ? 0 : 1);
+    HIP_CHECK(hipGetLastError());
+    HIP_CHECK(hipDeviceSynchronize());
+    HIP_CHECK(hipMemcpy(perm, dp, (size_t)M * sizeof(int), hipMemcpyDeviceToHost));
+  } catch (const PmpcHipError &) {
+    if (ds) (void)hipFree(ds);
+    if (dp) (void)hipFree(dp);
+    return -1;
+  }
+  (void)hipFree(ds);
+  (void)hipFree(dp);
+  return 0;
 }
 void launch_as_begin(AsCtl *ctl, int *fail, int max_rounds, double dual_scale, hipStream_t s, int stall_limit) {
   hipLaunchKernelGGL(k_as_begin, dim3(1), dim3(64), 0, s, ctl, fail, max_rounds, dual_scale, stall_limit);
diff --git a/pmpc_amd/csrc/kernels_generic.hip b/pmpc_amd/csrc/kernels_generic.hip
--- a/pmpc_amd/csrc/kernels_generic.hip
+++ b/pmpc_amd/csrc/kernels_generic.hip
@@ -908,10 +908,10 @@
   __shared__ double y[8];
   const int nblk = pend.ctl ? (int)gridDim.x - 1 : (int)gridDim.x;
   if (pend.ctl && (int)blockIdx.x == nblk) {
-    as_ctl_block(pend.ctl, pend.cnt_part, pend.M, pend.fail, 1, 1, 0, pend.mirror, pend.mirror_seq, pend.seq, nullptr, pend.viol, pend.open_part);
+    as_ctl_block(pend.ctl, pend.cnt_part, pend.M, pend.fail, 1, 1, 0, pend.mirror, pend.mirror_seq, pend.seq, nullptr, pend.viol, pend.open_part, pend.tree);
     if (pend.perm) {
       __syncthreads();
-      as_perm_block(pend.settled, pend.M, pend.perm);
+      as_perm_block(pend.settled, pend.M, pend.perm, pend.tree);
     }
     return;
   }
@@ -998,8 +998,10 @@
   static const int per = getenv("PMPC_CONS_PER_PARTIAL") ? atoi(getenv("PMPC_CONS_PER_PARTIAL")) : 256;
   int G = (M + per - 1) / per;
   if (G > 64) G = 64;
+  AsCtlCall call = pend;
+  call.tree = as_ctl_wave() ? 0 : 1;
   hipLaunchKernelGGL(k_cons_small, dim3(G + (pend.ctl ? 1 : 0)), dim3(1024), 0, s, Hc_part, gc_part, M, nc, 1, tmp, tmp + (size_t)64 * nH, 0,
-                     nullptr, nullptr, nullptr, pend);
+                     nullptr, nullptr, nullptr, call);
   return G;
 }
 
diff --git a/pmpc_amd/csrc/pmpc_dev.h b/pmpc_amd/csrc/pmpc_dev.h
--- a/pmpc_amd/csrc/pmpc_dev.h
+++ b/pmpc_amd/csrc/pmpc_dev.h
@@ -160,7 +160,10 @@
   const int *open_part;
   const int *settled;
   int *perm;
-};
+  int tree;
+};
+void launch_ck_stat_sum(unsigned long long *slots, int M, int reset, hipStream_t s);
+bool as_ctl_wave();
 int launch_cons_partials(const double *Hc_part, const double *gc_part, int M, int nc, double *tmp, const AsCtlCall &pend,
                          hipStream_t s);
 void launch_cons_small(const double *Hc_part, const double *gc_part, int M, int nc, bool with_H, double *Hg, double *tmp, bool solve_now,
@@ -309,7 +312,7 @@
                       const double *params, double *f, double *fx, double *fu, hipStream_t s, int jac32 = 0);
 void launch_linearize_compact(int model, int N, int M, const double *x0, const double *X_prev, const double *U_prev, const double *params,
                               double *f, double *jc, const double *Xr, const double *Xrp, const double *Ur, const double *Urp, int x, int u,
-                              double *res_out, hipStream_t s);
+                              double *res_out, hipStream_t s, const AsCtlCall *last_ctl = nullptr);
 void launch_rollout(int model, int N, int M, const double *x0, const double *U, const double *params, double *X, hipStream_t s);
 void launch_shift_plan(int model, int N, int M, int sh, const double *X, const double *U, const double *params, const double *U_tail, double *Xn,
                        double *Un, double *um1n, hipStream_t s);
@@ -320,7 +323,8 @@
 int jac_live_mask(int model, unsigned char *fx_mask, unsigned char *fu_mask);
 void launch_linearize_with_residual(int model, int N, int M, const double *x0, const double *X_prev, const double *U_prev,
                                     const double *params, double *f, double *fx, double *fu, const double *Xr, const double *Xrp,
-                                    const double *Ur, const double *Urp, int x, int u, double *res_out, hipStream_t s, int jac32 = 0);
+                                    const double *Ur, const double *Urp, int x, int u, double *res_out, hipStream_t s, int jac32 = 0,
+                                    const AsCtlCall *last_ctl = nullptr);
 void launch_widen_f32(const float *src, double *dst, long long n, hipStream_t s);
 bool f32_as_dims_supported(int x, int u);
 void launch_scp_residual(const double *X, const double *Xp, const double *U, const double *Up, long long rows, int x, int u,
diff --git a/pmpc_amd/csrc/solver.hip b/pmpc_amd/csrc/solver.hip
--- a/pmpc_amd/csrc/solver.hip
+++ b/pmpc_amd/csrc/solver.hip
@@ -393,10 +393,16 @@
 void pmpc_restart_stats(pmpc_ctx *c, unsigned long long *out4, int reset) {
   for (int k = 0; k < 4; k++) out4[k] = 0;
   if (!c || !c->ws.ck_stat.p) return;
+  Workspace &w = c->ws;
+  unsigned long long *slots = (unsigned long long *)w.ck_stat.p;
   (void)hipSetDevice(c->device);
+  launch_ck_stat_sum(slots, w.ck_stat_m, reset, c->stream);
   HIP_WARN(hipStreamSynchronize(c->stream));
-  HIP_WARN(hipMemcpy(out4, c->ws.ck_stat.p, 4 * sizeof(unsigned long long), hipMemcpyDeviceToHost));
-  if (reset) HIP_WARN(hipMemset(c->ws.ck_stat.p, 0, 4 * sizeof(unsigned long long)));
+  HIP_WARN(hipMemcpy(out4, slots + 4 * (size_t)w.ck_stat_m, 4 * sizeof(unsigned long long), hipMemcpyDeviceToHost));
+  for (int k = 0; k < 4; k++) {
+    out4[k] += w.ck_carry[k];
+    if (reset) w.ck_carry[k] = 0;
+  }
 }
 
 int pmpc_comm_unique_id(void *out128) {
@@ -748,6 +754,7 @@
                           ((p0->flags & PMPC_HAS_UBOUNDS) || soc) && !(p0->barrier_mu > 0.0) && c->opt[OPT_AS_DEFECT] != 0.0 &&
                           c->opt[OPT_AS_WARM] != 0.0 && c->opt[OPT_POLISH_MU] > 0.0;
   bool compact_set[2] = {false, false};
+  static const bool last_ctl_env = !(getenv("PMPC_AS_LAST_CTL_RIDE") && atoi(getenv("PMPC_AS_LAST_CTL_RIDE")) == 0);
   int done = 0, cur = 0;
   if (!model_known(model) || (with_cost && (jac32 || !obstacle_cost_valid(cost, (int)p0->xdim)))) {
     if (infos && steps > 0) { memset(&infos[0], 0, sizeof(pmpc_info)); infos[0].status = 2; }
@@ -788,12 +795,15 @@
         if (next && !res_dirty && !c->multi()) {
           ProfScope ps(c, 6);
           compact_set[cur ^ 1] = compact_ok;
+          AsCtlCall last_ctl = c->as_last;
+          c->as_last.ctl = nullptr;
+          const AsCtlCall *lc = last_ctl.ctl ? &last_ctl : nullptr;
           if (compact_ok)
             launch_linearize_compact(model, (int)p.N, (int)p.M, p.x0, Xo, Uo, params, F[cur ^ 1][0], F[cur ^ 1][1], Xo, Xp, Uo, Up, (int)p.xdim,
-                                     (int)p.udim, res + done, c->stream);
+                                     (int)p.udim, res + done, c->stream, lc);
           else
             launch_linearize_with_residual(model, (int)p.N, (int)p.M, p.x0, Xo, Uo, params, F[cur ^ 1][0], F[cur ^ 1][1], F[cur ^ 1][2], Xo, Xp, Uo,
-                                           Up, (int)p.xdim, (int)p.udim, res + done, c->stream, jac32);
+                                           Up, (int)p.xdim, (int)p.udim, res + done, c->stream, jac32, lc);
           shift(cur ^ 1, Xo);
           res_dirty = true;
           return;
@@ -816,10 +826,13 @@
       };
       c->spec_fired = c->spec_ok = false;
       c->post_batch = [&]() { follow_up(true); };
+      c->ride_last_ctl = last_ctl_env && !cone_obj && !c->multi() && done + 1 < steps;
+      c->as_last.ctl = nullptr;
       pmpc_info inf;
       const int st = cone_obj ? lcone_body(c, &p, p.barrier_mu > 0.0 ? 1.0 / p.barrier_mu : std::numeric_limits<double>::quiet_NaN(), &inf, 0)
                               : solve_impl(c, &p, &inf, 0, soc);
       c->post_batch = nullptr;
+      c->ride_last_ctl = false;
       c->jac_compact_fx = nullptr;
       if (infos) infos[done] = inf;
       if (st != 0) break;
@@ -834,6 +847,8 @@
     HIP_CHECK(hipGetLastError());
   } catch (const PmpcHipError &) {
     c->post_batch = nullptr;
+    c->ride_last_ctl = false;
+    c->as_last.ctl = nullptr;
     c->jac_compact_fx = nullptr;
     if (infos && done < steps) { memset(&infos[done], 0, sizeof(pmpc_info)); infos[done].status = 2; }
     fail_after_error(c, nullptr, nullptr);
diff --git a/pmpc_amd/csrc/solver_internal.h b/pmpc_amd/csrc/solver_internal.h
--- a/pmpc_amd/csrc/solver_internal.h
+++ b/pmpc_amd/csrc/solver_internal.h
@@ -71,6 +71,8 @@
   DevBuf as_perm;
   int as_perm_m = -1;
   DevBuf as_T;
+  int ck_stat_m = 0;
+  unsigned long long ck_carry[4] = {0, 0, 0, 0};
   DevBuf as_ck, as_jhi, ck_stat;
   DevBuf as_act, as_cnt, as_cntp, as_settled, as_ctl, as_delta, as_viol;
   long long su_key = -1;
@@ -145,6 +147,8 @@
   DevBuf host_flags;
   std::function<void()> post_batch;
   bool spec_fired = false, spec_ok = false;
+  bool ride_last_ctl = false;
+  AsCtlCall as_last{};
   const double *jac_compact_fx = nullptr;
   int jac_compact_model = 0;
 };
diff --git a/pmpc_amd/csrc/solver_qp.hip b/pmpc_amd/csrc/solver_qp.hip
--- a/pmpc_amd/csrc/solver_qp.hip
+++ b/pmpc_amd/csrc/solver_qp.hip
@@ -575,7 +575,14 @@
       const int ks = (x + 3) / 4;
       w.as_ck.ensure((size_t)M * slots * (64 * ks + 32) * D8);
       w.as_jhi.ensure((size_t)M * sizeof(int));
-      if (w.ck_stat.ensure(4 * sizeof(unsigned long long))) HIP_CHECK(hipMemsetAsync(w.ck_stat.p, 0, 4 * sizeof(unsigned long long), s));
+      if (M > w.ck_stat_m) {
+        unsigned long long old[4];
+        pmpc_restart_stats(c, old, 0);
+        for (int k = 0; k < 4; k++) w.ck_carry[k] = old[k];
+        w.ck_stat.ensure((size_t)(M + 1) * 4 * sizeof(unsigned long long));
+        HIP_CHECK(hipMemsetAsync(w.ck_stat.p, 0, (size_t)(M + 1) * 4 * sizeof(unsigned long long), s));
+        w.ck_stat_m = M;
+      }
       b.as_ck = w.as_ck.d(); b.as_jhi = (int *)w.as_jhi.p; b.ck_slots = slots; b.ck_stat = (unsigned long long *)w.ck_stat.p;
     }
   }
@@ -764,6 +771,9 @@
       } else if (!last && fuse_ctl) {
         c->as_pend = AsCtlCall{ctl, (const int *)w.as_cntp.p, M, (const int *)w.fail.p, &c->mirror_dev->ctl, &c->mirror_dev->as_seq, c->as_seq,
                                b.as_viol, open_part, nullptr, nullptr};
+      } else if (last && fuse_ctl && round == 0 && c->post_batch && c->ride_last_ctl) {
+        c->as_last = AsCtlCall{ctl, (const int *)w.as_cntp.p, M, (const int *)w.fail.p, &c->mirror_dev->ctl, &c->mirror_dev->as_seq, c->as_seq,
+                               b.as_viol, open_part, nullptr, nullptr};
       } else {
         launch_as_ctl(ctl, (const int *)w.as_cntp.p, M, (const int *)w.fail.p, 1, 1, last ? 1 : 0, &c->mirror_dev->ctl, &c->mirror_dev->as_seq, c->as_seq, s,
                       nullptr, b.as_viol, open_part);
@@ -775,6 +785,12 @@
       c->spec_fired = true;
       n_batches_at_hook = 0;
       hook();
+      if (c->as_last.ctl) {
+        const AsCtlCall q = c->as_last;
+        c->as_last.ctl = nullptr;
+        ProfScope ps(c, 5);
+        launch_as_ctl(q.ctl, q.cnt_part, q.M, q.fail, 1, 1, 1, q.mirror, q.mirror_seq, q.seq, s, nullptr, q.viol, q.open_part);
+      }
     }
     n_batches_at_hook++;
     {
```

Result: no change. 2997 SCP iterations/s (-0.5%).
